# SDFIdk/malstroem

Measured on AMD Instinct MI355X. Metric: Mcells/s fill->D8->accum->label on 16384^2 f32 DEM, higher is better.
Workload: dtype f32 fill / f64 no-flats+D8+accum / u8 flowdir / i32 labels; 1 GPU; 16384x16384 float32 DEM (spectral fBm beta=2 seed 42 (SURVEY 8d recipe)): fill+depths -> no-flats fill -> D8 -> accumulation -> CCL+label_stats -> watersheds+label_count -> pour points; parallelism=1 GPU, one device context, fill_rounds=8, noflat_rounds=84, fill_tiles=70225, fill_visits=43613, fill_cycles=0, noflat_visits=409001, noflat_cycles=409001, nlabels=4637017, fill_algorithm=1, fill_launches=8, noflat_algorithm=2, pour_algorithm=1

## Files before the change

malstroem_amd/csrc/ccl.hip:

```cpp
#include <cstdlib>
#include <string>
#include <type_traits>
#include <utility>

#include "common.hpp"

namespace mh {
namespace {

constexpr int SCAN_BLOCK = 1024;
constexpr int SCAN_ITEMS = 4;
constexpr int SCAN_TILE = SCAN_BLOCK * SCAN_ITEMS;

template <typename T> __device__ __forceinline__ bool is_fg(T v) { return v != (T)0; }

template <typename T>
__global__ __launch_bounds__(256) void ccl_init_kernel(const T *__restrict__ data, int32_t *__restrict__ parent, int64_t n, int64_t W)
{
    const int64_t i = (int64_t)blockIdx.x * blockDim.x + threadIdx.x;
    const int lane = threadIdx.x & 63;
    const bool fg = i < n && is_fg(data[i]);
    const bool fg_left = __shfl_up((int)fg, 1) != 0;
    const bool start = fg && (lane == 0 || !fg_left || (i % W) == 0);
    const uint64_t brk = __ballot(start);
    if (i >= n) return;
    int32_t p = -1;
    if (fg) {
        const uint64_t below = brk & ((2ull << lane) - 1ull);
        p = (int32_t)(i - (lane - (63 - __builtin_clzll(below))));
    }
    parent[i] = p;
}

__device__ __forceinline__ int32_t find_root(const int32_t *parent, int32_t x)
{
    int32_t p = parent[x];
    while (p != x) {
        x = p;
        p = parent[x];
    }
    return x;
}

__device__ __forceinline__ void unite(int32_t *parent, int32_t a, int32_t b)
{
    for (;;) {
        a = find_root(parent, a);
        b = find_root(parent, b);
        if (a == b) return;
        if (a < b) {
            const int32_t t = a;
            a = b;
            b = t;
        }
        const int32_t old = atomicMin(&parent[a], b);
        if (old == a) return;
        a = old;
    }
}

__global__ __launch_bounds__(256) void ccl_merge_kernel(int32_t *parent, int64_t H, int64_t W)
{
    const int64_t i = (int64_t)blockIdx.x * blockDim.x + threadIdx.x;
    if (i >= H * W) return;
    if (parent[i] < 0) return;
    const int64_t r = i / W, c = i - r * W;
    const bool hasW = c > 0 && parent[i - 1] >= 0;
    if (hasW && (threadIdx.x & 63) == 0) unite(parent, (int32_t)i, (int32_t)(i - 1));
    if (r == 0) return;
    const bool hasN = parent[i - W] >= 0;
    const bool hasNW = c > 0 && parent[i - W - 1] >= 0;
    if (hasN) {
        if (!(hasW && hasNW)) unite(parent, (int32_t)i, (int32_t)(i - W));
        return;
    }
    const bool hasNE = c + 1 < W && parent[i - W + 1] >= 0;
    if (hasNW && !hasW) unite(parent, (int32_t)i, (int32_t)(i - W - 1));
    if (hasNE) unite(parent, (int32_t)i, (int32_t)(i - W + 1));
}

constexpr int CT = 64;
constexpr int MAXROOTS = CT * CT / 4;
constexpr uint32_t LBG = 0xffffffffu;

__device__ __forceinline__ uint32_t find_root_l(const uint32_t *par, uint32_t x)
{
    uint32_t p = par[x];
    while (p != x) {
        x = p;
        p = par[x];
    }
    return x;
}
__device__ __forceinline__ void unite_l(uint32_t *par, uint32_t a, uint32_t b)
{
    for (;;) {
        a = find_root_l(par, a);
        b = find_root_l(par, b);
        if (a == b) return;
        if (a < b) {
            const uint32_t t = a;
            a = b;
            b = t;
        }
        const uint32_t old = atomicMin(&par[a], b);
        if (old == a) return;
        a = old;
    }
}

#ifndef CCL_U2
#define CCL_U2 4
#endif
#ifndef CCL_U3
#define CCL_U3 4
#endif
template <typename T>
__global__ __launch_bounds__(256) void ccl_tile_kernel(const T *__restrict__ data, int32_t *__restrict__ parent, int64_t H, int64_t W, int ntc,
                                                       int32_t *__restrict__ rootlist, int32_t *__restrict__ rootcount, int32_t *__restrict__ colpar)
{
    __shared__ uint32_t par[CT * CT];
    __shared__ int s_nroots;
    if (threadIdx.x == 0) s_nroots = 0;
    const int lane = threadIdx.x & 63, wave = threadIdx.x >> 6;
    const int ti = blockIdx.x / ntc, tj = blockIdx.x - ti * ntc;
    const int64_t r0 = (int64_t)ti * CT, c0 = (int64_t)tj * CT;
    const int64_t cc = c0 + lane;
#pragma unroll
    for (int k = 0; k < CT / 4; ++k) {
        const int r = wave + 4 * k;
        const bool fg = (r0 + r) < H && cc < W && is_fg(data[(r0 + r) * W + cc]);
        const uint64_t m = __ballot(fg);
        const uint64_t starts = m & ~(m << 1);
        const uint64_t below = starts & ((2ull << lane) - 1ull);
        par[r * CT + lane] = fg ? (uint32_t)(r * CT + (63 - __builtin_clzll(below))) : LBG;
    }
    __syncthreads();
#pragma unroll CCL_U2
    for (int k = 0; k < CT / 4; ++k) {
        const int r = wave + 4 * k;
        if (r == 0) continue;
        const uint64_t m = __ballot(par[r * CT + lane] != LBG);
        const uint32_t pn = par[(r - 1) * CT + lane];
        const uint64_t up = __ballot(pn != LBG);
        if (!((m >> lane) & 1ull)) continue;
        const bool hasW = lane > 0 && ((m >> (lane - 1)) & 1ull), hasN = (up >> lane) & 1ull;
        const bool hasNW = lane > 0 && ((up >> (lane - 1)) & 1ull), hasNE = lane < 63 && ((up >> (lane + 1)) & 1ull);
        const uint32_t i = (uint32_t)(r * CT + lane);
        if (hasN) {
            if (!(hasW && hasNW)) unite_l(par, i, i - CT);
        } else {
            if (hasNW && !hasW) unite_l(par, i, i - CT - 1);
            if (hasNE) unite_l(par, i, i - CT + 1);
        }
    }
    __syncthreads();
#pragma unroll CCL_U3
    for (int k = 0; k < CT / 4; ++k) {
        const int r = wave + 4 * k;
        const bool inside = (r0 + r) < H && cc < W;
        const uint32_t p = inside ? par[r * CT + lane] : LBG;
        int32_t out = -1;
        if (lane == 0 || lane == CT - 1) {
            int32_t e = -1;
            if (p != LBG) {
                const uint32_t rt = find_root_l(par, p);
                e = (int32_t)((r0 + (rt >> 6)) * W + c0 + (rt & 63u));
            }
            colpar[((int64_t)blockIdx.x * 2 + (lane ? 1 : 0)) * CT + r] = e;
        }
        if (!inside) continue;
        if (p != LBG) {
            const uint32_t root = find_root_l(par, p);
            out = (int32_t)((r0 + (root >> 6)) * W + c0 + (root & 63u));
            if (root == (uint32_t)(r * CT + lane)) rootlist[(size_t)blockIdx.x * MAXROOTS + atomicAdd(&s_nroots, 1)] = out;
        }
        parent[(r0 + r) * W + cc] = out;
    }
    __syncthreads();
    if (threadIdx.x == 0) rootcount[blockIdx.x] = s_nroots;
}

__global__ __launch_bounds__(256) void ccl_flatten_roots_kernel(int32_t *parent, const int32_t *__restrict__ rootlist, const int32_t *__restrict__ rootcount,
                                                                int64_t ntiles, unsigned long long *rootbits)
{
    const int64_t tile = (int64_t)blockIdx.x * 4 + (threadIdx.x >> 6);
    if (tile >= ntiles) return;
    const int cnt = rootcount[tile];
    for (int j = threadIdx.x & 63; j < cnt; j += 64) {
        const int32_t r = rootlist[(size_t)tile * MAXROOTS + j];
        const int32_t root = find_root(parent, r);
        if (root != r) parent[r] = root;
        else atomicOr(&rootbits[r >> 6], 1ull << (r & 63));
    }
}

constexpr int WB = 1024;
__global__ __launch_bounds__(WB) void ccl_bits_count_kernel(const unsigned long long *__restrict__ rootbits, int64_t nwords, uint32_t *__restrict__ block_counts)
{
    __shared__ uint32_t wsum[WB / 64];
    const int64_t w = (int64_t)blockIdx.x * WB + threadIdx.x;
    uint32_t cnt = w < nwords ? (uint32_t)__popcll(rootbits[w]) : 0u;
#pragma unroll
    for (int o = 32; o > 0; o >>= 1) cnt += __shfl_xor(cnt, o);
    if ((threadIdx.x & 63) == 0) wsum[threadIdx.x >> 6] = cnt;
    __syncthreads();
    if (threadIdx.x == 0) {
        uint32_t t = 0;
        for (int k = 0; k < WB / 64; ++k) t += wsum[k];
        block_counts[blockIdx.x] = t;
    }
}
__global__ __launch_bounds__(WB) void ccl_bits_prefix_kernel(const unsigned long long *__restrict__ rootbits, int64_t nwords,
                                                              const uint32_t *__restrict__ block_offsets, uint32_t *__restrict__ wordprefix)
{
    __shared__ uint32_t wsum[WB / 64];
    const int lane = threadIdx.x & 63, wave = threadIdx.x >> 6;
    const int64_t w = (int64_t)blockIdx.x * WB + threadIdx.x;
    const uint32_t cnt = w < nwords ? (uint32_t)__popcll(rootbits[w]) : 0u;
    uint32_t incl = cnt;
#pragma unroll
    for (int o = 1; o < 64; o <<= 1) {
        const uint32_t v = __shfl_up(incl, o);
        if (lane >= o) incl += v;
    }
    if (lane == 63) wsum[wave] = incl;
    __syncthreads();
    uint32_t woff = 0;
    for (int k = 0; k < wave; ++k) woff += wsum[k];
    if (w < nwords) wordprefix[w] = block_offsets[blockIdx.x] + woff + incl - cnt;
}

__global__ __launch_bounds__(256) void ccl_emit_ranked_kernel(const int32_t *__restrict__ parent, const unsigned long long *__restrict__ rootbits,
                                                              const uint32_t *__restrict__ wordprefix, int32_t *__restrict__ labels, int64_t n)
{
    const int64_t i0 = ((int64_t)blockIdx.x * blockDim.x + threadIdx.x) * 4;
    if (i0 >= n) return;
    auto rank_of = [&](int32_t p) -> int32_t {
        if (p < 0) return 0;
        const int32_t g = parent[p];
        return (int32_t)(wordprefix[g >> 6] + (uint32_t)__popcll(rootbits[g >> 6] & ((1ull << (g & 63)) - 1ull))) + 1;
    };
    if (i0 + 4 <= n) {
        const int4 p = *reinterpret_cast<const int4 *>(parent + i0);
        int4 l;
        l.x = rank_of(p.x);
        l.y = rank_of(p.y);
        l.z = rank_of(p.z);
        l.w = rank_of(p.w);
        *reinterpret_cast<int4 *>(labels + i0) = l;
    } else {
        for (int64_t i = i0; i < n; ++i) labels[i] = rank_of(parent[i]);
    }
}

__global__ __launch_bounds__(256) void ccl_seam_kernel(int32_t *parent, int64_t H, int64_t W, int64_t nh, int64_t total, const int32_t *__restrict__ colpar,
                                                       int64_t ntc)
{
    const int64_t k = (int64_t)blockIdx.x * blockDim.x + threadIdx.x;
    if (k >= total) return;
    if (k < nh) {
        const int64_t r = (k / W + 1) * CT, c = k % W;
        const int64_t i = r * W + c;
        if (parent[i] < 0) return;
        const bool hasW = c > 0 && parent[i - 1] >= 0, hasN = parent[i - W] >= 0, hasNW = c > 0 && parent[i - W - 1] >= 0;
        if (hasN) {
            if (!(hasW && hasNW)) unite(parent, (int32_t)i, (int32_t)(i - W));
            return;
        }
        const bool hasNE = c + 1 < W && parent[i - W + 1] >= 0;
        if (hasNW && !hasW) unite(parent, (int32_t)i, (int32_t)(i - W - 1));
        if (hasNE) unite(parent, (int32_t)i, (int32_t)(i - W + 1));
    } else {
        const int64_t q = k - nh;
        const int64_t r = q % H, sj = q / H;
        const int64_t ti = r / CT, lr = r - ti * CT;
        const int32_t *left = colpar + ((ti * ntc + sj) * 2 + 1) * CT, *right = colpar + ((ti * ntc + sj + 1) * 2 + 0) * CT;
        const int32_t me = right[lr];
        if (me < 0) return;
        const int32_t w = left[lr];
        if (w >= 0) {
            unite(parent, me, w);
            return;
        }
        if (r > 0) {
            const int32_t nw = lr > 0 ? left[lr - 1] : colpar[(((ti - 1) * ntc + sj) * 2 + 1) * CT + CT - 1];
            if (nw >= 0) unite(parent, me, nw);
        }
        if (r + 1 < H) {
            const int32_t sw = lr < CT - 1 ? left[lr + 1] : colpar[(((ti + 1) * ntc + sj) * 2 + 1) * CT];
            if (sw >= 0) unite(parent, me, sw);
        }
    }
}

__global__ __launch_bounds__(256) void ccl_flatten_kernel(int32_t *parent, int64_t n)
{
    const int64_t i = (int64_t)blockIdx.x * blockDim.x + threadIdx.x;
    if (i >= n) return;
    const int32_t p = parent[i];
    if (p < 0 || p == (int32_t)i) return;
    parent[i] = find_root(parent, p);
}

__global__ __launch_bounds__(SCAN_BLOCK) void ccl_count_roots_kernel(const int32_t *__restrict__ parent, int64_t n,
                                                                    uint32_t *__restrict__ block_counts)
{
    __shared__ uint32_t wsum[SCAN_BLOCK / 64];
    const int64_t base = (int64_t)blockIdx.x * SCAN_TILE + (int64_t)threadIdx.x * SCAN_ITEMS;
    uint32_t cnt = 0;
#pragma unroll
    for (int k = 0; k < SCAN_ITEMS; ++k) {
        const int64_t i = base + k;
        if (i < n) cnt += parent[i] == (int32_t)i;
    }
#pragma unroll
    for (int o = 32; o > 0; o >>= 1) cnt += __shfl_xor(cnt, o);
    if ((threadIdx.x & 63) == 0) wsum[threadIdx.x >> 6] = cnt;
    __syncthreads();
    if (threadIdx.x == 0) {
        uint32_t t = 0;
        for (int w = 0; w < SCAN_BLOCK / 64; ++w) t += wsum[w];
        block_counts[blockIdx.x] = t;
    }
}

__global__ __launch_bounds__(1024) void scan_blocks_kernel(uint32_t *block_counts, int64_t nb, unsigned long long *total)
{
    __shared__ unsigned long long part[1024];
    const int64_t per = (nb + 1023) / 1024;
    const int64_t b0 = (int64_t)threadIdx.x * per, b1 = b0 + per < nb ? b0 + per : nb;
    unsigned long long s = 0;
    for (int64_t b = b0; b < b1; ++b) s += block_counts[b];
    part[threadIdx.x] = s;
    __syncthreads();
    if (threadIdx.x == 0) {
        unsigned long long run = 0;
        for (int t = 0; t < 1024; ++t) {
            const unsigned long long v = part[t];
            part[t] = run;
            run += v;
        }
        *total = run;
    }
    __syncthreads();
    unsigned long long run = part[threadIdx.x];
    for (int64_t b = b0; b < b1; ++b) {
        const uint32_t v = block_counts[b];
        block_counts[b] = (uint32_t)run;
        run += v;
    }
}

__global__ __launch_bounds__(SCAN_BLOCK) void ccl_rank_roots_kernel(int32_t *parent, int64_t n,
                                                                   const uint32_t *__restrict__ block_offsets)
{
    __shared__ uint32_t wsum[SCAN_BLOCK / 64];
    const int lane = threadIdx.x & 63, wave = threadIdx.x >> 6;
    const int64_t base = (int64_t)blockIdx.x * SCAN_TILE + (int64_t)threadIdx.x * SCAN_ITEMS;
    bool root[SCAN_ITEMS];
    uint32_t cnt = 0;
#pragma unroll
    for (int k = 0; k < SCAN_ITEMS; ++k) {
        const int64_t i = base + k;
        root[k] = i < n && parent[i] == (int32_t)i;
        cnt += root[k];
    }
    uint32_t incl = cnt;
#pragma unroll
    for (int o = 1; o < 64; o <<= 1) {
        const uint32_t v = __shfl_up(incl, o);
        if (lane >= o) incl += v;
    }
    if (lane == 63) wsum[wave] = incl;
    __syncthreads();
    uint32_t woff = 0;
    for (int w = 0; w < wave; ++w) woff += wsum[w];
    uint32_t rank = block_offsets[blockIdx.x] + woff + incl - cnt;
#pragma unroll
    for (int k = 0; k < SCAN_ITEMS; ++k)
        if (root[k]) {
            ++rank;
            parent[base + k] = -(int32_t)rank - 1;
        }
}

__global__ __launch_bounds__(256) void ccl_emit_kernel(const int32_t *__restrict__ parent, int32_t *__restrict__ labels,
                                                      int64_t n)
{
    const int64_t i = (int64_t)blockIdx.x * blockDim.x + threadIdx.x;
    if (i >= n) return;
    int32_t p = parent[i];
    if (p >= 0) p = parent[p];
    labels[i] = p == -1 ? 0 : -p - 1;
}

template <typename T>
int ccl8_dev(const T *d_data, int32_t *d_labels, int32_t *d_tmp, int64_t H, int64_t W, int64_t *nlabels, hipStream_t s, DevBuf *stats_out = nullptr,
             CclKeep *keep = nullptr)
{
    if (keep) keep->valid = false;
    const int64_t n = H * W;
    if (n >= (int64_t)INT32_MAX - 1) {
        set_error("connected components: %lld cells exceed the int32 index domain", (long long)n);
        return MHIP_ELIMIT;
    }
    const unsigned g256 = (unsigned)cdiv(n, 256);
    const int64_t nb = cdiv(n, SCAN_TILE);
    DevBuf counts, total;
    MH_TRY(counts.alloc(sizeof(uint32_t) * (size_t)nb));
    MH_TRY(total.alloc(sizeof(unsigned long long)));
    int32_t *parent = d_tmp;
    static const bool global_uf = [] { const char *e = dev_env("MHIP_CCL"); return e && std::string(e) == "global"; }();
    if (global_uf) {
        hipLaunchKernelGGL((ccl_init_kernel<T>), dim3(g256), dim3(256), 0, s, d_data, parent, n, W);
        hipLaunchKernelGGL(ccl_merge_kernel, dim3(g256), dim3(256), 0, s, parent, H, W);
        hipLaunchKernelGGL(ccl_flatten_kernel, dim3(g256), dim3(256), 0, s, parent, n);
        hipLaunchKernelGGL(ccl_count_roots_kernel, dim3((unsigned)nb), dim3(SCAN_BLOCK), 0, s, parent, n, counts.as<uint32_t>());
        hipLaunchKernelGGL(scan_blocks_kernel, dim3(1), dim3(1024), 0, s, counts.as<uint32_t>(), nb, total.as<unsigned long long>());
        hipLaunchKernelGGL(ccl_rank_roots_kernel, dim3((unsigned)nb), dim3(SCAN_BLOCK), 0, s, parent, n, counts.as<uint32_t>());
        hipLaunchKernelGGL(ccl_emit_kernel, dim3(g256), dim3(256), 0, s, parent, d_labels, n);
    } else {
        const int64_t ntr = cdiv(H, CT), ntc = cdiv(W, CT), ntiles = ntr * ntc;
        const int64_t nwords = cdiv(n, 64), nwb = cdiv(nwords, WB);
        DevBuf roots, rcount, bits, wprefix, bcounts, colpar;
        MH_TRY(colpar.alloc(4 * 2 * CT * (size_t)ntiles));
        MH_TRY(roots.alloc(4 * (size_t)ntiles * MAXROOTS));
        MH_TRY(rcount.alloc(4 * (size_t)ntiles));
        MH_TRY(bits.alloc(8 * (size_t)nwords));
        MH_TRY(wprefix.alloc(4 * (size_t)nwords));
        MH_TRY(bcounts.alloc(4 * (size_t)nwb));
        MH_HIP(hipMemsetAsync(bits.p, 0, 8 * (size_t)nwords, s));
        hipLaunchKernelGGL((ccl_tile_kernel<T>), dim3((unsigned)ntiles), dim3(256), 0, s, d_data, parent, H, W, (int)ntc, roots.as<int32_t>(),
                           rcount.as<int32_t>(), colpar.as<int32_t>());
        const int64_t nh = (ntr - 1) * W, nv = (ntc - 1) * H;
        if (nh + nv > 0)
            hipLaunchKernelGGL(ccl_seam_kernel, dim3((unsigned)cdiv(nh + nv, 256)), dim3(256), 0, s, parent, H, W, nh, nh + nv, colpar.as<int32_t>(), ntc);
        hipLaunchKernelGGL(ccl_flatten_roots_kernel, dim3((unsigned)cdiv(ntiles, 4)), dim3(256), 0, s, parent, roots.as<int32_t>(),
                           rcount.as<int32_t>(), ntiles, bits.as<unsigned long long>());
        hipLaunchKernelGGL(ccl_bits_count_kernel, dim3((unsigned)nwb), dim3(WB), 0, s, bits.as<unsigned long long>(), nwords, bcounts.as<uint32_t>());
        hipLaunchKernelGGL(scan_blocks_kernel, dim3(1), dim3(1024), 0, s, bcounts.as<uint32_t>(), nwb, total.as<unsigned long long>());
        hipLaunchKernelGGL(ccl_bits_prefix_kernel, dim3((unsigned)nwb), dim3(WB), 0, s, bits.as<unsigned long long>(), nwords, bcounts.as<uint32_t>(),
                           wprefix.as<uint32_t>());
        unsigned long long h_total = 0;
        if constexpr (std::is_same<T, float>::value) {
            if (stats_out) {
                MH_HIP(hipGetLastError());
                MH_HIP(hipMemcpyAsync(&h_total, total.p, sizeof(h_total), hipMemcpyDeviceToHost, s));
                MH_HIP(stream_sync(s));
                *nlabels = (int64_t)h_total;
                MH_TRY(stats_out->alloc(sizeof(mhip_stat_record) * (size_t)(h_total + 1)));
                return label_emit_stats_dev(parent, bits.as<unsigned long long>(), wprefix.as<uint32_t>(), d_data, d_labels, H, W, (int64_t)h_total,
                                            stats_out->as<mhip_stat_record>(), s);
            }
        }
        if (keep) {
            const int64_t top = (H < 4 ? H : 2) * W;
            MH_TRY(ccl_emit_rows_dev(parent, bits.as<unsigned long long>(), wprefix.as<uint32_t>(), d_labels, 0, top, s));
            if (H >= 4) MH_TRY(ccl_emit_rows_dev(parent, bits.as<unsigned long long>(), wprefix.as<uint32_t>(), d_labels, (H - 2) * W, 2 * W, s));
        } else {
            hipLaunchKernelGGL(ccl_emit_ranked_kernel, dim3((unsigned)cdiv(cdiv(n, 4), 256)), dim3(256), 0, s, parent, bits.as<unsigned long long>(), wprefix.as<uint32_t>(), d_labels, n);
        }
        MH_HIP(hipGetLastError());
        MH_HIP(hipMemcpyAsync(&h_total, total.p, sizeof(h_total), hipMemcpyDeviceToHost, s));
        MH_HIP(stream_sync(s));
        *nlabels = (int64_t)h_total;
        if (keep) {
            keep->bits.release();
            keep->wprefix.release();
            std::swap(keep->bits.p, bits.p);
            std::swap(keep->bits.bytes, bits.bytes);
            std::swap(keep->wprefix.p, wprefix.p);
            std::swap(keep->wprefix.bytes, wprefix.bytes);
            keep->H = H;
            keep->W = W;
            keep->nlocal = (int64_t)h_total;
            keep->valid = true;
        }
        return MHIP_OK;
    }
    MH_HIP(hipGetLastError());
    unsigned long long h_total = 0;
    MH_HIP(hipMemcpyAsync(&h_total, total.p, sizeof(h_total), hipMemcpyDeviceToHost, s));
    MH_HIP(stream_sync(s));
    *nlabels = (int64_t)h_total;
    if constexpr (std::is_same<T, float>::value) {
        if (stats_out) {
            MH_TRY(stats_out->alloc(sizeof(mhip_stat_record) * (size_t)(h_total + 1)));
            MH_TRY(label_stats_dev(d_data, d_labels, n, (int64_t)h_total, stats_out->as<mhip_stat_record>(), s, W, true));
        }
    }
    return MHIP_OK;
}

}

int ccl8_f32_dev(const float *d_data, int32_t *d_labels, int32_t *d_tmp, int64_t H, int64_t W, int64_t *nlabels,
                 hipStream_t s, DevBuf *stats_out)
{
    return ccl8_dev<float>(d_data, d_labels, d_tmp, H, W, nlabels, s, stats_out);
}
int ccl8_f32_begin_dev(const float *d_data, int32_t *d_labels, int32_t *d_tmp, int64_t H, int64_t W, int64_t *nlabels, hipStream_t s, CclKeep *keep)
{
    return ccl8_dev<float>(d_data, d_labels, d_tmp, H, W, nlabels, s, nullptr, keep);
}
int ccl8_u8_dev(const uint8_t *d_data, int32_t *d_labels, int32_t *d_tmp, int64_t H, int64_t W, int64_t *nlabels,
                hipStream_t s)
{
    return ccl8_dev<uint8_t>(d_data, d_labels, d_tmp, H, W, nlabels, s);
}

}
```

malstroem_amd/csrc/common.hpp:

```cpp
#pragma once
#include <hip/hip_runtime.h>
#include <cstdint>
#include <cstdio>
#include <cstring>
#include <string>
#include <vector>

#include "../../include/malstroem_hip.h"

struct mhip_polygons;
struct mhip_flowpaths;

namespace mh {

void set_error(const char *fmt, ...);
const char *get_error();
const char *dev_env(const char *name);
hipError_t stream_sync(hipStream_t s);
int require_device();

#define MH_HIP(expr)                                                                             \
    do {                                                                                         \
        hipError_t _e = (expr);                                                                  \
        if (_e != hipSuccess) {                                                                  \
// ... 24 lines not shown
    size_t bytes = 0;
    DevBuf() = default;
    DevBuf(const DevBuf &) = delete;
    DevBuf &operator=(const DevBuf &) = delete;
    ~DevBuf() { release(); }
    int alloc(size_t n)
    {
        if (n == 0) n = 16;
        if (p && bytes >= n && bytes <= 2 * n + 4096) return MHIP_OK;
        release();
        MH_TRY(pool_alloc(&p, n));
        bytes = n;
        return MHIP_OK;
    }
    void release()
    {
        if (p) pool_free(p, bytes);
        p = nullptr;
        bytes = 0;
    }
    template <typename T> T *as() const { return reinterpret_cast<T *>(p); }
};

int upload(DevBuf &b, const void *host, size_t bytes, hipStream_t s);
int download(void *host, const DevBuf &b, size_t bytes, hipStream_t s);
int64_t build_rank_lut(const uint8_t *keep, int64_t nlab, std::vector<int32_t> &lut);
inline bool hyps_res_ok(double res) { return res > 0.0 && res <= 1.7976931348623157e308; }
int trace_on_device(const uint8_t *d_fd, const int32_t *d_lab, int64_t H, int64_t W, const int64_t *cells_rc, int64_t n, int use_bg,
                    int32_t bg, int32_t *out_label, int32_t *out_found, int64_t *out_len, const int64_t *offsets, int64_t *out_cells,
                    hipStream_t s);

__host__ __device__ inline int dir_dr(int k) { return (k == 0 || k == 1 || k == 7) ? -1 : (k >= 3 && k <= 5) ? 1 : 0; }
__host__ __device__ inline int dir_dc(int k) { return (k >= 1 && k <= 3) ? 1 : (k >= 5 && k <= 7) ? -1 : 0; }

__device__ __forceinline__ unsigned d8_code(double z, double u, double ur, double r, double dr, double d, double dl,
                                            double l, double ul)
{
    const double INV_SQRT2 = 0.7071067811865475;
    unsigned i = 8;
    double dzmax = 0.0, dz;
#define MH_D8_STEP(expr, k)          \
    dz = (expr);                     \
    i = dz > dzmax ? (k) : i;        \
    dzmax = fmax(dzmax, dz);
    MH_D8_STEP(__dsub_rn(z, u), 0u)
    MH_D8_STEP(__dmul_rn(__dsub_rn(z, ur), INV_SQRT2), 1u)
    MH_D8_STEP(__dsub_rn(z, r), 2u)
    MH_D8_STEP(__dmul_rn(__dsub_rn(z, dr), INV_SQRT2), 3u)
    MH_D8_STEP(__dsub_rn(z, d), 4u)
    MH_D8_STEP(__dmul_rn(__dsub_rn(z, dl), INV_SQRT2), 5u)
    MH_D8_STEP(__dsub_rn(z, l), 6u)
    MH_D8_STEP(__dmul_rn(__dsub_rn(z, ul), INV_SQRT2), 7u)
#undef MH_D8_STEP
    return i;
}

__device__ __forceinline__ unsigned edge_code(int64_t r, int64_t c, int64_t maxr, int64_t maxc)
{
    unsigned code = 8;
    if (r == 0) code = 0;
    if (r == maxr) code = 4;
    if (c == 0) code = 6;
    if (c == maxc) code = 2;
    if (r == 0 && c == 0) code = 7;
    if (r == 0 && c == maxc) code = 1;
    if (r == maxr && c == 0) code = 5;
    if (r == maxr && c == maxc) code = 3;
    return code;
}

__host__ __device__ inline uint32_t f32_key(float f)
{
    uint32_t u;
    memcpy(&u, &f, 4);
    return (u & 0x80000000u) ? ~u : (u | 0x80000000u);
}
__host__ __device__ inline float key_f32(uint32_t k)
{
    uint32_t u = (k & 0x80000000u) ? (k & 0x7fffffffu) : ~k;
    float f;
    memcpy(&f, &u, 4);
    return f;
}
__device__ __forceinline__ uint32_t dem_key(float v)
{
    if (v != v) return f32_key(__builtin_inff());
    return f32_key(v + 0.0f);
}
__host__ __device__ inline uint64_t f64_key(double f)
{
    uint64_t u;
    memcpy(&u, &f, 8);
    return (u & 0x8000000000000000ull) ? ~u : (u | 0x8000000000000000ull);
}
__host__ __device__ inline double key_f64(uint64_t k)
{
    uint64_t u = (k & 0x8000000000000000ull) ? (k & 0x7fffffffffffffffull) : ~k;
    double f;
    memcpy(&f, &u, 8);
    return f;
}

struct FillStats {
    int32_t rounds = 0;
    int64_t visits = 0;
    int64_t cycles = 0;
    int64_t tiles = 0;
    float hot_ms = 0;
    int32_t hot_launches = 0;
    int32_t algorithm = 0;
    uint32_t overflow = 0;
    bool have_minmax = false, dem_nan = false;
    float dem_min = 0.0f, dem_max = 0.0f;
    int32_t geo_reject = 0;
    int64_t geo_irregular = 0, geo_unreached = 0, geo_mismatch = 0;
};

struct FillRun {
    bool noflat = false;
    const float *dem = nullptr;
    void *out = nullptr;
    int64_t H = 0, W = 0;
    double sh = 0, dg = 0;
    const float *seed = nullptr;
    double seed_add = 0;
    int fixed_top = 0, fixed_bot = 0;
    int rounds_per_batch = 8;
    bool attach_only = false;
    struct Impl;
    Impl *impl;
    FillRun();
    ~FillRun();
    FillRun(const FillRun &) = delete;
    FillRun &operator=(const FillRun &) = delete;
    int begin(hipStream_t s, bool *active);
    int batch(hipStream_t s, bool *active);
    int activate_row(int side, hipStream_t s);
    int attach(hipStream_t s);
    int certify(hipStream_t s, bool *changed);
    int finish(hipStream_t s, FillStats *st);
};
void noflat_seed(FillRun &f, const float *d_filled, double sh, double dg, int64_t ncells_global);
struct PfRun;
struct FillHandover {
    PfRun *run = nullptr;
    const float *dem = nullptr;
    float *filled = nullptr, *depths = nullptr;
    int64_t H = 0, W = 0;
    const uint16_t *bslot = nullptr;
    const uint32_t *tabV = nullptr;
    int ntr = 0, ntc = 0;
    bool pending = false, queued = false, violated = false, repaired = false;
    bool suspect = false;
    FillStats st_repair;
    FillHandover() = default;
    FillHandover(const FillHandover &) = delete;
    FillHandover &operator=(const FillHandover &) = delete;
    ~FillHandover();
    void release();
};
int fill_handover_complete(FillHandover *ho, hipStream_t s);
int fill_handover_repair(FillHandover *ho, hipStream_t s);
int fill_plain_dev(const float *d_dem, float *d_out, int64_t H, int64_t W, hipStream_t s, FillStats *st, float *d_depths = nullptr,
                   bool *depths_done = nullptr, FillHandover *ho = nullptr);
int fill_check_f32_dev(const float *d_dem, const float *d_filled, int64_t H, int64_t W, int fixed_top, int fixed_bot, hipStream_t s,
                       unsigned int *d_flag);
int fill_plain_pflood_dev(const float *d_dem, float *d_out, float *d_depths, int64_t H, int64_t W, hipStream_t s, FillStats *st, bool *violated = nullptr,
                          uint32_t *overflow = nullptr, FillHandover *ho = nullptr);
struct PfRun {
    const float *dem = nullptr;
    float *out = nullptr;
    int64_t H = 0, W = 0;
    int fixed_top = 0, fixed_bot = 0;
    uint32_t overflow = 0;
    struct Impl;
    Impl *impl;
    PfRun();
    ~PfRun();
    PfRun(const PfRun &) = delete;
    PfRun &operator=(const PfRun &) = delete;
    int begin(hipStream_t s);
    int halo_changed(int side, hipStream_t s);
    int batch(hipStream_t s);
    int finish(hipStream_t s, float *d_depths, FillStats *st, bool *violated = nullptr, FillHandover *ho = nullptr);
    int finish_late(hipStream_t s, float *d_depths, bool *violated);
    int proof_flag(hipStream_t s, unsigned int *h_flag);
    int solve(hipStream_t s);
    int pack(hipStream_t s, int row0, int nrows);
    int publish_edges(hipStream_t s);
};
struct StageHook {
    enum Point { FIRST_VISIT = 0, TAIL_ROUNDS = 1, FINISH = 3 };
    void (*fn)(void *, hipStream_t) = nullptr;
    void *arg = nullptr;
    bool fired = false;
    int at = TAIL_ROUNDS;
    void fire(hipStream_t s)
    {
        if (fn && !fired) {
            fired = true;
            fn(arg, s);
        }
    }
    void fire_at(int point, hipStream_t s)
    {
        if (point == at) fire(s);
    }
};

struct GeoRun {
    const float *dem = nullptr, *filled = nullptr;
    double *out = nullptr;
    uint32_t *dist = nullptr;
    int64_t H = 0, W = 0;
    double sh = 0, dg = 0;
    int fixed_top = 0, fixed_bot = 0;
    bool allow_partial = false;
    double seed_add = 0;
    bool partial = false;
    StageHook *tail_hook = nullptr;
    uint8_t *d8_out = nullptr;
    unsigned int *d8_nodir = nullptr;
    bool d8_done = false;
    bool defer_out = false;
    bool out_deferred = false;
    FillHandover *handover = nullptr;
    struct Impl;
    Impl *impl;
    GeoRun();
    ~GeoRun();
    GeoRun(const GeoRun &) = delete;
    GeoRun &operator=(const GeoRun &) = delete;
    int begin(hipStream_t s, bool *applicable, bool *active);
    int batch(hipStream_t s, bool *active);
    int halo_changed(int side, hipStream_t s);
    int end(hipStream_t s, bool *ok, FillStats *st);
    int launch_rounds(hipStream_t s, int nb);
};
struct D8Sink {
    uint8_t *flowdir = nullptr;
    unsigned int *nodir = nullptr;
    bool done = false;
    uint32_t *dist = nullptr;
    bool defer = false, deferred = false;
};
int noflat_assemble_dev(const float *d_filled, const uint32_t *d_dist, double *d_out, int64_t n, double seed_add, hipStream_t s);
int fill_noflat_geodesic_dev(const float *d_dem, const float *d_filled, double *d_out, int64_t H, int64_t W, double sh, double dg, double seed_add,
                             hipStream_t s, FillStats *st, bool *partial, StageHook *tail_hook = nullptr, D8Sink *d8 = nullptr, FillHandover *ho = nullptr);
int noflat_verify_dev(const float *d_dem, const double *d_out, int64_t H, int64_t W, double sh, double dg, hipStream_t s, bool *ok, int fixed_top = 0,
                      int fixed_bot = 0);
int fill_noflat_dev(const float *d_dem, double *d_out, int64_t H, int64_t W, double sh, double dg, hipStream_t s,
                    FillStats *st = nullptr, const float *d_filled = nullptr, StageHook *tail_hook = nullptr, D8Sink *d8 = nullptr,
                    FillHandover *ho = nullptr);
int short_diag_dev(const float *d_dem, int64_t n, double *sh, double *dg, hipStream_t s);
int depths_dev(const float *d_filled, const float *d_dem, float *d_out, int64_t n, hipStream_t s);
int d8_dev(const double *d_z, uint8_t *d_out, int64_t H, int64_t W, int edges_outward, hipStream_t s, int64_t row_off = 0,
           int64_t Hg = 0, unsigned int *d_interior_nodir = nullptr);
void short_diag_from_minmax(float mn, float mx, bool has_nan, double *sh, double *dg);
int minmax_dev(const float *d_x, int64_t n, float *mn, float *mx, int *has_nan, hipStream_t s);
int row_update_dev(void *d_dst, const void *d_src, int64_t nbytes, int *changed, hipStream_t s);
int copy_bandwidth_dev(size_t bytes, int reps, double *gbs, hipStream_t s);
int read_bandwidth_dev(size_t bytes, int reps, double *gbs, hipStream_t s);
int row_update_async(void *d_dst, const void *d_src, int64_t nbytes, int *d_changed, hipStream_t s);
int trace_downstream_dev(const uint8_t *d_fd, const int32_t *d_lab, int64_t H, int64_t W, const int64_t *d_cells, int64_t n, int use_bg,
                         int32_t bg, int32_t *d_label, int32_t *d_found, int64_t *d_len, const int64_t *d_offsets, int64_t *d_out_cells,
                         hipStream_t s);
int comm_unique_id(void *id128);
int comm_available();
int comm_create(void **comm, const void *id128, int rank, int nranks);
void comm_destroy(void *comm);
int comm_exchange_rows(void *comm, int rank, int nranks, const void *first_row, const void *last_row, void *stage, size_t rowbytes,
                       hipStream_t s);
int comm_allreduce_max(void *comm, double *d_value, hipStream_t s);
struct PourCandDev {
    uint16_t *mask0 = nullptr;
    uint2 *list = nullptr;
    uint32_t *tile_cnt = nullptr;
    unsigned long long *tile_key0 = nullptr;
    uint32_t *flags = nullptr;
    int components = 0;
    unsigned long long *key = nullptr;
    uint32_t nlab = 0;
};
constexpr uint32_t POUR_TILE_CAP = 512;
struct PourLink {
    PourCandDev dev;
    hipEvent_t ev = nullptr;
    void (*notify)(void *, int) = nullptr;
    int (*wait)(void *) = nullptr;
    void *arg = nullptr;
    bool consumed = false;
};
struct AccumKeep {
    DevBuf nodes;
    size_t o[9] = {};
    int64_t H = 0, W = 0;
    int fixed_top = 0, fixed_bot = 0;
    bool valid = false;
};
struct AccumPrep {
    DevBuf nodes;
    int64_t H = 0, W = 0;
    hipEvent_t ready = nullptr;
    bool valid = false;
    ~AccumPrep();
};
int accum_prepare_dev(AccumPrep *prep, int64_t H, int64_t W, hipStream_t s, hipEvent_t ready);
int accum_dev(const uint8_t *d_fd, double *d_out, int64_t H, int64_t W, hipStream_t s, int fixed_top = 0, int fixed_bot = 0, int halo_zero = 0,
              int32_t *d_exit_map = nullptr, PourLink *pour = nullptr, AccumKeep *keep = nullptr, AccumPrep *prep = nullptr);
int accum_band_delta_dev(const uint8_t *d_fd, double *d_out, int64_t H, int64_t W, hipStream_t s, int fixed_top, int fixed_bot, AccumKeep *keep, bool *done);
int ccl8_f32_dev(const float *d_data, int32_t *d_labels, int32_t *d_tmp, int64_t H, int64_t W, int64_t *nlabels,
                 hipStream_t s, DevBuf *stats_out = nullptr);
int label_emit_stats_dev(const int32_t *d_parent, const unsigned long long *d_rootbits, const uint32_t *d_wordprefix, const float *d_data,
                         int32_t *d_labels, int64_t H, int64_t W, int64_t nlab, mhip_stat_record *d_rec, hipStream_t s);
int ccl8_u8_dev(const uint8_t *d_data, int32_t *d_labels, int32_t *d_tmp, int64_t H, int64_t W, int64_t *nlabels,
                hipStream_t s);
struct CclKeep {
    DevBuf bits, wprefix;
    int64_t H = 0, W = 0, nlocal = 0;
    bool valid = false;
};
int ccl8_f32_begin_dev(const float *d_data, int32_t *d_labels, int32_t *d_tmp, int64_t H, int64_t W, int64_t *nlabels, hipStream_t s, CclKeep *keep);
int ccl_emit_rows_dev(const int32_t *d_parent, const unsigned long long *d_rootbits, const uint32_t *d_wordprefix, int32_t *d_labels, int64_t base,
                      int64_t count, hipStream_t s);
int label_emit_sparse_dev(const int32_t *d_parent, const unsigned long long *d_rootbits, const uint32_t *d_wordprefix, const float *d_data,
                          int32_t *d_labels, int64_t H, int64_t W, int ht, int64_t H_owned, int64_t nlocal, int32_t offset,
                          const int32_t *d_dropped, const int32_t *d_target, int32_t ndropped, int64_t nlab_global, mhip_stat_record *d_rec,
                          hipStream_t s);
int relabel_lut_dev(int32_t *d_labels, const int32_t *d_lut, int64_t nlab, int64_t n, hipStream_t s);
int relabel_range_dev(int32_t *d_labels, int64_t n, int32_t lo, int32_t hi, const int32_t *d_lut, const int32_t *d_fid, const int32_t *d_fnew, int32_t nf,
                      hipStream_t s);
int band_trace_dev(const uint8_t *d_fd, const int32_t *d_lab, int64_t Hl, int64_t W, int64_t row_lo, int64_t own0, int64_t own1, int64_t Hg,
                   const int64_t *d_cells, const int32_t *d_src, int64_t n, int use_bg, int32_t bg, int32_t *d_label, int32_t *d_status,
                   int32_t *d_src_out, int64_t *d_exit, int64_t *d_len, const int64_t *d_offsets, int64_t *d_out_cells, hipStream_t s);
int relabel_sparse_dev(int32_t *d_labels, int64_t n, int64_t nlocal, int32_t offset, const int32_t *d_dropped, const int32_t *d_target,
                       int32_t ndropped, hipStream_t s);
int keep_mask_dev(const int32_t *d_labels, const uint8_t *d_keep, int64_t nlab, int64_t n, uint8_t *d_mask,
                  hipStream_t s);
int label_stats_dev(const float *d_data, const int32_t *d_labels, int64_t n, int64_t nlab, mhip_stat_record *d_rec,
                    hipStream_t s, int64_t W = 0, bool components = false);
int label_stats64_dev(const double *d_data, const int32_t *d_labels, int64_t n, int64_t nlab, mhip_stat_record *d_rec, hipStream_t s);
int label_stats_zero_sign_dev(const float *d_data, const int32_t *d_labels, int64_t n, int64_t nlab, mhip_stat_record *d_rec, hipStream_t s);
int label_stats_zero_sign_dev(const double *d_data, const int32_t *d_labels, int64_t n, int64_t nlab, mhip_stat_record *d_rec, hipStream_t s);
int label_arg_dev(const double *d_data, const int32_t *d_labels, int64_t H, int64_t W, int64_t nlab, bool is_max,
                  mhip_index_record *d_rec, hipStream_t s, bool components = false);
int label_count_dev(const int32_t *d_labels, int64_t n, int64_t nlab, int64_t *d_counts, hipStream_t s, int64_t W = 0);
int label_max_dev(const int32_t *d_labels, int64_t n, int32_t *out_max, hipStream_t s);
constexpr int64_t HYPS_MAX_BINS = (int64_t)1 << 30;
int hyps_layout_dev(const double *d_dmax, int64_t stride, int64_t nlab, double res, int64_t *d_offsets, int64_t *total, hipStream_t s);
int hyps_table_dev(const float *d_data, const int32_t *d_labels, int64_t n, int64_t W, int64_t nlab, double res, const int64_t *d_offsets,
                   int64_t total, uint32_t *d_counts, double *d_sums, int64_t *lds_spills, hipStream_t s, hipEvent_t ev0 = nullptr,
                   hipEvent_t ev1 = nullptr);
int hyps_levels_dev(int64_t nlab, const int64_t *d_offsets, const uint32_t *d_counts, const double *d_sums, const double *d_dmax, int64_t stride,
                    const double *d_q, mhip_final_record *d_rec, hipStream_t s);
int final_depths_dev(const float *d_data, const int32_t *d_labels, int64_t n, int64_t W, int64_t nlab, mhip_final_record *d_rec, float *d_out,
                     hipStream_t s, hipEvent_t ev0 = nullptr, hipEvent_t ev1 = nullptr);
bool wet_at_events_ok(int64_t K, const float *values);
int wet_at_dev(const float *d_data, const int32_t *d_labels, int64_t n, int64_t W, int64_t nlab, int K, const double *d_drawdown, int64_t stride,
               const float *values, float *d_out, int64_t *d_wet, int64_t wet_stride, hipStream_t s, hipEvent_t ev0 = nullptr,
               hipEvent_t ev1 = nullptr);
bool flow_distance_scale_ok(double scale);
int flow_distance_dev(const uint8_t *d_fd, const int32_t *d_lab, int64_t H, int64_t W, double scale, int64_t nlab, float *d_out, mhip_index_record *d_rec,
                      int64_t *unresolved, hipStream_t s);
int fdist_jumps_dev(uint4 *&cur, uint4 *&nxt, int64_t W, int64_t ntc, int64_t ntiles, unsigned int *d_open, hipStream_t s);
int hand_check(double threshold, double scale);
int hand_dev(const uint8_t *d_fd, const double *d_acc, const float *d_elev, const int32_t *d_lab, int64_t H, int64_t W, double threshold, double scale,
             float nodata, float *d_hand, float *d_dist, int64_t *undrained, hipStream_t s);
int reach_catchments_dev(const uint8_t *d_fd, const double *d_acc, const int32_t *d_lab, int64_t H, int64_t W, double threshold, int32_t *d_catch,
                         mhip_flowpaths *p, int64_t *assigned, hipStream_t s);
int inundate_dev(const float *d_hand, const int32_t *d_catch, int64_t n, int64_t W, int64_t nreach, const float *d_stage, float nodata, float *d_depth,
                 mhip_zone_record *d_rec, hipStream_t s);
int burn_check(int64_t nseg, const mhip_burn_segment *segs, int64_t nline, const mhip_burn_line *lines, const mhip_burn_result *results);
int burn_lines_dev(float *d_dem, int64_t H, int64_t W, int64_t nseg, const mhip_burn_segment *segs, int64_t nline, const mhip_burn_line *lines,
                   double nodata, mhip_burn_result *results, hipStream_t s);
int zones_check(int64_t H, int64_t W, int64_t nvert, const double *xy, int64_t nring, const int64_t *ring_offsets, const int32_t *ring_zone,
                int64_t nzone, int grow);
int zones_rasterize_dev(int32_t *d_out, int64_t H, int64_t W, int64_t nvert, const double *xy, int64_t nring, const int64_t *ring_offsets,
                        const int32_t *ring_zone, int64_t nzone, int grow, hipStream_t s);
int zone_stats_dev(const float *d_data, const int32_t *d_zones, int64_t n, int64_t W, int64_t nzone, mhip_zone_record *d_rec, hipStream_t s);
int polygonize_check(int64_t H, int64_t W);
int polygons_fetch_dev(const mhip_polygons *p, int32_t *xy, int64_t *ring_offsets, int32_t *ring_label);
int polygonize_dev(const int32_t *d_lab, int64_t H, int64_t W, DevBuf &d_xy, DevBuf &d_off, DevBuf &d_rl, int64_t *nring, int64_t *nvert, hipStream_t s);
int flowpaths_check(int64_t H, int64_t W, double threshold);
int flowpaths_dev(const uint8_t *d_fd, const double *d_acc, const int32_t *d_lab, int64_t H, int64_t W, double threshold, mhip_flowpaths *p, hipStream_t s,
                  int32_t *d_rc = nullptr);
int flowpaths_fetch_dev(const mhip_flowpaths *p, int32_t *xy, int64_t *reach_offsets, mhip_reach_record *records);
int watersheds_dev(const uint8_t *d_fd, int32_t *d_labels, int64_t H, int64_t W, int32_t unassigned, hipStream_t s,
                   bool band_mode = false, const unsigned int *d_known_interior_nodir = nullptr, const int32_t *d_src = nullptr, PourLink *pour = nullptr);
int pour_finish_dev(unsigned long long *d_key, const unsigned long long *d_tile_key0, int64_t ntiles, int64_t nlab, int64_t W, mhip_index_record *d_rec,
                    hipStream_t s);
int band_pseudo_labels_dev(int32_t *d_ws, int64_t H, int64_t W, int top, int bottom, hipStream_t s);
int negative_lut_dev(int32_t *d_lab, int64_t n, const int32_t *d_lut, int64_t nlut, hipStream_t s);
constexpr int32_t BAND_ROOT = 1, BAND_ROOTLESS = 0x7fffffff;
int band_root_labels_dev(int32_t *d_out, int64_t H, int64_t W, int64_t row_off, int64_t Hg, hipStream_t s);
int band_hide_rootless_dev(const int32_t *d_lab, const int32_t *d_rooted, int32_t *d_out, int64_t n, hipStream_t s);
int band_show_rootless_dev(int32_t *d_ws, const int32_t *d_lab, int64_t n, hipStream_t s);

__host__ __device__ inline int64_t cdiv(int64_t a, int64_t b) { return (a + b - 1) / b; }

constexpr int TR = 32;
struct TileGeom {
    int64_t n, W;
    int64_t ntr, ntc;
};
__host__ __device__ inline TileGeom tile_geom(int64_t n, int64_t W)
{
    TileGeom g;
    g.n = n;
    g.W = (W > 0 && n % W == 0) ? W : 256;
    const int64_t H = cdiv(n, g.W);
    g.ntr = cdiv(H, TR);
    g.ntc = cdiv(g.W, 256);
    return g;
}
inline unsigned tile_grid(const TileGeom &g)
{
    const int64_t nt = g.ntr * g.ntc;
    return (unsigned)(nt < 2048 ? (nt > 0 ? nt : 1) : 2048);
}

#ifdef __HIPCC__
__device__ __forceinline__ int64_t downstream(const uint8_t *fd, int64_t i, int64_t H, int64_t W)
{
    const unsigned code = fd[i];
    if (code > 7u) return -1;
    const int64_t r = i / W, c = i - r * W;
    const int64_t nr = r + dir_dr((int)code), nc = c + dir_dc((int)code);
    if (nr < 0 || nr >= H || nc < 0 || nc >= W) return -1;
    return nr * W + nc;
}
constexpr int WS_TILE = 64;
__device__ __forceinline__ int ws_perim_slot(int lr, int lc)
{
    if (lr == 0) return lc;
    if (lr == WS_TILE - 1) return WS_TILE + lc;
    if (lc == 0) return 2 * WS_TILE + (lr - 1);
    if (lc == WS_TILE - 1) return 2 * WS_TILE + (WS_TILE - 2) + (lr - 1);
    return -1;
}
__device__ __forceinline__ int64_t ws_node_of(int32_t cell, uint32_t W, int ntc)
{
    const uint32_t r = (uint32_t)cell / W, c = (uint32_t)cell - r * W;
    const int slot = ws_perim_slot((int)(r & 63u), (int)(c & 63u));
    return slot < 0 ? -1 : (int64_t)((r >> 6) * (uint32_t)ntc + (c >> 6)) * 256 + slot;
}

constexpr int32_t FD_NONE = 0x7fffffff;
constexpr int32_t FD_DONE = (int32_t)0x80000000;
constexpr double FD_SQRT2 = 1.4142135623730951;
__device__ __forceinline__ uint32_t fd_step(unsigned code) { return (code & 1u) ? 0x10000u : 1u; }
__device__ __forceinline__ bool fd_resolve(uint2 s, const uint4 *__restrict__ Nn, uint32_t W, int ntc, uint32_t &no, uint32_t &nd, int32_t &T)
{
    int32_t t = (int32_t)s.x;
    no = s.y & 0xffffu;
    nd = s.y >> 16;
    if (t >= 0 && t != FD_NONE) {
        const int64_t node = ws_node_of(t, W, ntc);
        uint4 m = make_uint4((uint32_t)FD_NONE, 0u, 0u, 0u);
        if (node >= 0) m = Nn[node];
        t = (int32_t)m.x;
        no += m.y;
        nd += m.z;
    }
    T = t & ~FD_DONE;
    return t < 0;
// ... 55 lines not shown
```

malstroem_amd/csrc/ctx.hip:

```cpp
#include <mutex>
#include <new>
#include <string>
#include <vector>

#include "ctx.hpp"

namespace mh {

static void drop_hyps(mhip_ctx *c)
{
    c->hyps_total = -1;
    c->have[MHIP_R_FINALDEPTHS] = false;
    c->wetat_events = -1;
    c->wetat_out.release();
}

static void drop_flow_distance(mhip_ctx *c)
{
    std::lock_guard<std::mutex> lk(c->fdist_mu);
    c->fdist_unresolved = -1;
    c->fdist_out.release();
    c->fdist_rec.release();
}

// ... 257 lines not shown
}

int mhip_ctx_side_end(mhip_ctx *c)
{
    MH_ARG(c && t_side_ctx == c, "ctx_side_end without ctx_side_begin on this thread");
    MH_HIP(hipSetDevice(c->device));
    MH_HIP(stream_sync(c->stream_b));
    t_side_ctx = nullptr;
    return MHIP_OK;
}

int mhip_ctx_upload(mhip_ctx *c, int which, const void *host)
{
    MH_ARG(c && host && which >= 0 && which < MHIP_R_COUNT_, "ctx_upload(ctx, which, host)");
    return mhip_ctx_upload_rows(c, which, 0, c->H_owned, host);
}

int mhip_ctx_upload_dem(mhip_ctx *c, const float *dem) { return mhip_ctx_upload(c, MHIP_R_DEM, dem); }

int mhip_ctx_upload_rows(mhip_ctx *c, int which, int64_t row0, int64_t nrows, const void *host)
{
    MH_ARG(c && host && which >= 0 && which < MHIP_R_COUNT_ && row0 >= 0 && nrows >= 1 && row0 + nrows <= c->H_owned,
           "ctx_upload_rows(ctx, which, row0, nrows, host)");
    MH_HIP(hipSetDevice(c->device));
    MH_TRY(ctx_raster(c, which));
    MH_TRY(ctx_settle(c, which, true));
    ctx_wrote(c, which, true);
    c->have[which] = false;
    MH_TRY(ctx_copy_rows(c, c->r[which].p, raster_elem(which), row0, nrows, const_cast<void *>(host), hipMemcpyHostToDevice));
    if (row0 + nrows == c->H_owned) {
        c->have[which] = true;
        if (which == MHIP_R_LABELS) c->labels_filtered = true;
    }
    return MHIP_OK;
}

int mhip_ctx_download_rows(mhip_ctx *c, int which, int64_t row0, int64_t nrows, void *host)
{
    MH_ARG(c && host && which >= 0 && which < MHIP_R_COUNT_ && row0 >= 0 && nrows >= 1 && row0 + nrows <= c->H_owned,
           "ctx_download_rows(ctx, which, row0, nrows, host)");
    MH_ARG(c->have[which], "raster has not been computed or uploaded");
    MH_TRY(ctx_settle(c, which, false));
    return ctx_copy_rows(c, c->r[which].p, raster_elem(which), row0, nrows, host, hipMemcpyDeviceToHost);
}

int mhip_ctx_download(mhip_ctx *c, int which, void *host)
{
    MH_ARG(c && host && which >= 0 && which < MHIP_R_COUNT_, "ctx_download(ctx, which, host)");
    return mhip_ctx_download_rows(c, which, 0, c->H_owned, host);
}

int mhip_ctx_trace_downstream(mhip_ctx *c, const int64_t *cells_rc, int64_t n, int use_background, int32_t background, int32_t *out_label,
                              int32_t *out_found, int64_t *out_len, const int64_t *offsets, int64_t *out_cells)
{
    MH_ARG(c && n >= 0 && (n == 0 || cells_rc), "ctx_trace_downstream(ctx, cells, n, ...)");
    MH_ARG(c->have[MHIP_R_FLOWDIR] && c->have[MHIP_R_LABELS], "ctx_trace_downstream needs flow directions and labels");
    MH_ARG(!c->ht && !c->hb, "stream tracing runs on an undivided raster");
    if (n == 0) return MHIP_OK;
    MH_HIP(hipSetDevice(c->device));
    return trace_on_device(c->r[MHIP_R_FLOWDIR].as<uint8_t>(), c->r[MHIP_R_LABELS].as<int32_t>(), c->H, c->W, cells_rc, n, use_background,
                           background, out_label, out_found, out_len, offsets, out_cells, c->stream);
}

int mhip_ctx_sync(mhip_ctx *c)
{
    MH_ARG(c, "ctx");
    MH_HIP(stream_sync(c->stream));
    return MHIP_OK;
}

int mhip_ctx_stage_ms(mhip_ctx *c, int stage, float *ms)
{
    MH_ARG(c && ms, "ctx_stage_ms(ctx, stage, ms)");
    const int k = timer_slot(stage);
    MH_ARG(k >= 0 && c->timers[k].valid, "stage has not been run");
    MH_HIP(hipEventSynchronize(c->timers[k].b));
    MH_HIP(hipEventElapsedTime(ms, c->timers[k].a, c->timers[k].b));
    return MHIP_OK;
}

int mhip_ctx_kernel_ms(mhip_ctx *c, const char *kernel, float *ms_total, int32_t *launches)
{
    MH_ARG(c && kernel && ms_total && launches, "ctx_kernel_ms(ctx, kernel, ms, launches)");
    const std::string k(kernel);
    if (k == "d8") {
        *launches = 1;
        return mhip_ctx_stage_ms(c, MHIP_STAGE_FLOWDIR, ms_total);
    }
    if (k == "d8_steady") {
        MH_ARG(c->have[MHIP_R_NOFLAT] && !c->ht && !c->hb, "d8_steady needs the no-flats surface on an undivided context");
        MH_HIP(hipSetDevice(c->device));
        double *g = nullptr;
        MH_TRY(ctx_noflat(c, &g));
        MH_TRY(ctx_raster(c, MHIP_R_FLOWDIR));
        MH_TRY(c->nodir_cnt.alloc(4));
        constexpr int REPS = 16;
        StageTimer *t;
        MH_TRY(ctx_timer(c, D8_STEADY_SLOT, &t));
        hipStream_t s = c->stream;
        ctx_wrote(c, MHIP_R_FLOWDIR);
        MH_HIP(hipMemsetAsync(c->nodir_cnt.p, 0, 4, s));
        for (int i = 0; i < REPS + 2; ++i) {
            if (i == 2) MH_HIP(hipEventRecord(t->a, s));
            MH_TRY(d8_dev(g, c->r[MHIP_R_FLOWDIR].as<uint8_t>(), c->H, c->W, 1, s, 0, c->H_global, c->nodir_cnt.as<unsigned int>()));
        }
        MH_HIP(hipEventRecord(t->b, s));
        MH_HIP(hipEventSynchronize(t->b));
        MH_HIP(hipEventElapsedTime(ms_total, t->a, t->b));
        c->have[MHIP_R_FLOWDIR] = true;
        c->nodir_valid = true;
        c->flowdir_own = true;
        *launches = REPS;
        return MHIP_OK;
    }
    if (k == "hyps_table" || k == "final_depths") {
        *launches = 1;
        return mhip_ctx_stage_ms(c, k == "hyps_table" ? HYPS_KERNEL_SLOT : FINAL_KERNEL_SLOT, ms_total);
    }
    if (k == "wet_at") {
        *launches = 1;
        return mhip_ctx_stage_ms(c, WETAT_KERNEL_SLOT, ms_total);
    }
    if (k == "fill_round") {
        *launches = c->fill_rounds;
        return mhip_ctx_stage_ms(c, MHIP_STAGE_FILL, ms_total);
    }
    if (k == "noflat_round") {
        *launches = c->noflat_rounds;
        return mhip_ctx_stage_ms(c, MHIP_STAGE_NOFLAT, ms_total);
    }
    set_error("unknown kernel family '%s'", kernel);
    return MHIP_EINVAL;
}

int mhip_ctx_get_i64(mhip_ctx *c, const char *key, int64_t *value)
{
    MH_ARG(c && key && value, "ctx_get_i64(ctx, key, value)");
    const std::string k(key);
    if (k == "nlabels_raw") *value = c->nlabels_raw;
    else if (k == "nlabels") {
        if (c->nlabels < 0 && c->have[MHIP_R_LABELS]) {
            MH_HIP(hipSetDevice(c->device));
            MH_TRY(ctx_label_max(c, c->stream));
        }
        *value = c->nlabels;
    }
    else if (k == "fill_rounds") *value = c->fill_rounds;
    else if (k == "noflat_rounds") *value = c->noflat_rounds;
    else if (k == "fill_visits") *value = c->fill_st.visits;
    else if (k == "fill_cycles") *value = c->fill_st.cycles;
    else if (k == "fill_tiles") *value = c->fill_st.tiles;
    else if (k == "fill_algorithm") *value = c->fill_st.algorithm;
    else if (k == "fill_handover") *value = c->fill_handover;
    else if (k == "fill_handover_rechecks") *value = c->fill_handover_rechecks;
    else if (k == "fill_overflow") *value = c->fill_st.overflow;
    else if (k == "fill_launches") *value = c->fill_st.rounds;
    else if (k == "fill_hot_launches") *value = c->fill_st.hot_launches;
    else if (k == "noflat_hot_launches") *value = c->noflat_st.hot_launches;
    else if (k == "accum_algorithm") *value = c->accum_algorithm;
    else if (k == "flowdir_computed") *value = (c->have[MHIP_R_FLOWDIR] && c->flowdir_own) ? 1 : 0;
    else if (k == "pour_algorithm") *value = c->pour_algorithm;
    else if (k == "noflat_algorithm") *value = c->noflat_st.algorithm;
    else if (k == "noflat_pending") *value = c->noflat_pending ? 1 : 0;
    else if (k == "noflat_visits") *value = c->noflat_st.visits;
    else if (k == "noflat_reject") *value = c->noflat_st.geo_reject;
    else if (k == "noflat_reject_irregular") *value = c->noflat_st.geo_irregular;
    else if (k == "noflat_reject_unreached") *value = c->noflat_st.geo_unreached;
    else if (k == "noflat_reject_mismatch") *value = c->noflat_st.geo_mismatch;
    else if (k == "noflat_cycles") *value = c->noflat_st.cycles;
    else if (k == "hyps_bins") *value = c->hyps_total;
    else if (k == "hyps_lds_spills") *value = c->hyps_spills;
    else if (k == "wet_at_events") *value = c->wetat_events;
    else if (k == "flow_distance_unresolved") *value = c->fdist_unresolved;
    else if (k == "hand_undrained") *value = c->hand_undrained;
    else if (k == "reach_catchments") *value = c->rcatch_nreach;
    else if (k == "inundation") *value = c->inund_held;
    else if (k == "zones") *value = c->nzone;
    else if (k == "H") *value = c->H;
    else if (k == "W") *value = c->W;
    else {
        set_error("unknown key '%s'", key);
        return MHIP_EINVAL;
    }
    return MHIP_OK;
}

int mhip_ctx_get_f64(mhip_ctx *c, const char *key, double *value)
{
    MH_ARG(c && key && value, "ctx_get_f64(ctx, key, value)");
    const std::string k(key);
    if (k == "short") *value = c->sh;
    else if (k == "diag") *value = c->dg;
    else if (k == "fill_hot_ms") *value = c->fill_st.hot_ms;
    else if (k == "noflat_hot_ms") *value = c->noflat_st.hot_ms;
    else {
        set_error("unknown key '%s'", key);
        return MHIP_EINVAL;
    }
    return MHIP_OK;
}

int mhip_ctx_raw_stats(mhip_ctx *c, mhip_stat_record *records)
{
    MH_ARG(c && records && c->raw_stats.p && c->nlabels_raw >= 0, "ctx_raw_stats needs a LABEL run");
    return ctx_fetch(c, c->raw_stats, sizeof(mhip_stat_record) * (size_t)(c->nlabels_raw + 1), records);
}

int mhip_ctx_apply_keep(mhip_ctx *c, const uint8_t *keep)
{
    MH_ARG(c, "ctx");
    MH_HIP(hipSetDevice(c->device));
    return ctx_apply_keep_on(c, keep, c->stream);
}

int mhip_ctx_stats(mhip_ctx *c, mhip_stat_record *records)
{
    MH_ARG(c && records && c->stats_valid && c->labels_filtered, "ctx_stats needs LABEL + apply_keep (or mhip_ctx_hyps) on the resident depths and labels");
    return ctx_fetch(c, c->stats, sizeof(mhip_stat_record) * (size_t)(c->nlabels + 1), records);
}

int mhip_ctx_watershed_counts(mhip_ctx *c, int64_t *counts)
{
    MH_ARG(c && counts && c->ws_counts_valid, "ctx_watershed_counts needs a WATERSHED run on the resident labels");
    return ctx_fetch(c, c->ws_counts, 8 * (size_t)(c->nlabels + 1), counts);
}

int mhip_ctx_pourpoints(mhip_ctx *c, mhip_index_record *records)
{
    MH_ARG(c && records && c->pour_valid, "ctx_pourpoints needs a POURPOINTS run on the resident labels and accumulated flow");
    return ctx_fetch(c, c->pour, sizeof(mhip_index_record) * (size_t)(c->nlabels + 1), records);
}

int mhip_ctx_hyps(mhip_ctx *c, double res, int64_t *total)
{
    MH_ARG(c && total && hyps_res_ok(res), "ctx_hyps(ctx, 0 < res < inf, total)");
    MH_ARG(!(c->nranks > 1 || c->ht || c->hb), "hypsometry on a row band is not built (the tables of the bands add up: a later step); use an undivided context");
    MH_ARG(c->have[MHIP_R_DEPTHS] && c->have[MHIP_R_LABELS] && !c->ccl_pending, "ctx_hyps needs the DEPTHS and LABELS rasters");
    MH_ARG(c->labels_filtered, "ctx_hyps needs mhip_ctx_apply_keep after the LABEL run");
    MH_HIP(hipSetDevice(c->device));
    hipStream_t s = c->stream;
    const int64_t n = c->H * c->W;
    c->hyps_total = -1;
    if (!c->stats_valid) {
        MH_TRY(ctx_label_max(c, s));
        MH_TRY(c->stats.alloc(sizeof(mhip_stat_record) * (size_t)(c->nlabels + 1)));
        MH_TRY(label_stats_dev(c->r[MHIP_R_DEPTHS].as<float>(), c->r[MHIP_R_LABELS].as<int32_t>(), n, c->nlabels, c->stats.as<mhip_stat_record>(), s,
                               c->W, c->labels_components));
        c->stats_valid = true;
    }
    const int64_t nlab = c->nlabels;
    MH_TRY(c->hyps_off.alloc(8 * (size_t)(nlab + 2)));
    StageTimer *k;
    MH_TRY(ctx_timer(c, HYPS_KERNEL_SLOT, &k));
    MH_TRY(stage_begin(c, MHIP_STAGE_HYPS, s));
    int64_t tot = 0;
    MH_TRY(hyps_layout_dev(c->stats.as<double>() + 1, 4, nlab, res, c->hyps_off.as<int64_t>(), &tot, s));
    MH_TRY(c->hyps_cnt.alloc(4 * (size_t)tot));
    MH_TRY(c->hyps_sum.alloc(8 * (size_t)tot));
    MH_TRY(hyps_table_dev(c->r[MHIP_R_DEPTHS].as<float>(), c->r[MHIP_R_LABELS].as<int32_t>(), n, c->W, nlab, res, c->hyps_off.as<int64_t>(), tot,
                          c->hyps_cnt.as<uint32_t>(), c->hyps_sum.as<double>(), &c->hyps_spills, s, k->a, k->b));
    MH_TRY(stage_end(c, MHIP_STAGE_HYPS, s));
    k->valid = true;
    c->hyps_total = tot;
    *total = tot;
    return MHIP_OK;
}

int mhip_ctx_hyps_fetch(mhip_ctx *c, int64_t *offsets, int64_t *counts, double *sums)
{
    MH_ARG(c && offsets && counts && sums, "ctx_hyps_fetch(ctx, offsets, counts, sums)");
    MH_ARG(c->hyps_total >= 0, "ctx_hyps_fetch needs mhip_ctx_hyps on the resident depths and labels");
    MH_HIP(hipSetDevice(c->device));
    hipStream_t s = c->stream;
    const size_t tot = (size_t)c->hyps_total;
    std::vector<uint32_t> c32(tot + 1);
    MH_HIP(hipMemcpyAsync(offsets, c->hyps_off.p, 8 * (size_t)(c->nlabels + 2), hipMemcpyDeviceToHost, s));
    if (tot) {
        MH_HIP(hipMemcpyAsync(c32.data(), c->hyps_cnt.p, 4 * tot, hipMemcpyDeviceToHost, s));
        MH_HIP(hipMemcpyAsync(sums, c->hyps_sum.p, 8 * tot, hipMemcpyDeviceToHost, s));
    }
    MH_HIP(stream_sync(s));
    for (size_t k = 0; k < tot; ++k) counts[k] = (int64_t)c32[k];
    return MHIP_OK;
}

int mhip_ctx_final_depths(mhip_ctx *c, const double *q, mhip_final_record *records)
{
    MH_ARG(c && q && records, "ctx_final_depths(ctx, q, records)");
    MH_ARG(c->hyps_total >= 0 && c->stats_valid, "ctx_final_depths needs mhip_ctx_hyps on the resident depths and labels");
    MH_HIP(hipSetDevice(c->device));
    hipStream_t s = c->stream;
    const int64_t nlab = c->nlabels, n = c->H * c->W;
    DevBuf d_q;
    MH_TRY(upload(d_q, q, 8 * (size_t)(nlab + 1), s));
    MH_TRY(c->hyps_rec.alloc(sizeof(mhip_final_record) * (size_t)(nlab + 1)));
    MH_TRY(ctx_raster(c, MHIP_R_FINALDEPTHS));
    c->have[MHIP_R_FINALDEPTHS] = false;
    StageTimer *k;
    MH_TRY(ctx_timer(c, FINAL_KERNEL_SLOT, &k));
    MH_TRY(stage_begin(c, MHIP_STAGE_FINALDEPTHS, s));
    MH_TRY(hyps_levels_dev(nlab, c->hyps_off.as<int64_t>(), c->hyps_cnt.as<uint32_t>(), c->hyps_sum.as<double>(), c->stats.as<double>() + 1, 4,
                           d_q.as<double>(), c->hyps_rec.as<mhip_final_record>(), s));
    MH_TRY(final_depths_dev(c->r[MHIP_R_DEPTHS].as<float>(), c->r[MHIP_R_LABELS].as<int32_t>(), n, c->W, nlab, c->hyps_rec.as<mhip_final_record>(),
                            c->r[MHIP_R_FINALDEPTHS].as<float>(), s, k->a, k->b));
    MH_TRY(stage_end(c, MHIP_STAGE_FINALDEPTHS, s));
    k->valid = true;
// ... 321 lines not shown
```

malstroem_amd/csrc/ctx.hpp:

```cpp
#pragma once
#include <atomic>
#include <condition_variable>
#include <functional>
#include <mutex>
#include <thread>

#include "common.hpp"

namespace mh {

class SideThread {
    std::thread th_;
    std::mutex mu_;
    std::condition_variable cv_;
    std::function<void()> task_;
    bool busy_ = false, stop_ = false;

public:
    ~SideThread()
    {
        {
            std::lock_guard<std::mutex> lk(mu_);
            stop_ = true;
        }
        cv_.notify_all();
        if (th_.joinable()) th_.join();
    }
    void run(std::function<void()> f)
    {
        std::unique_lock<std::mutex> lk(mu_);
        if (!th_.joinable())
            th_ = std::thread([this] {
                std::unique_lock<std::mutex> l2(mu_);
                for (;;) {
                    cv_.wait(l2, [this] { return stop_ || (busy_ && task_); });
                    if (stop_) return;
                    std::function<void()> f2 = std::move(task_);
                    task_ = nullptr;
                    l2.unlock();
                    f2();
                    l2.lock();
                    busy_ = false;
                    cv_.notify_all();
                }
            });
        task_ = std::move(f);
        busy_ = true;
        cv_.notify_all();
    }
    void wait()
    {
        std::unique_lock<std::mutex> lk(mu_);
        cv_.wait(lk, [this] { return !busy_; });
    }
};

struct StageTimer {
    hipEvent_t a = nullptr, b = nullptr;
    bool valid = false;
};
constexpr int N_STAGE_BITS = 9;
constexpr int WETAT_KERNEL_SLOT = 1 << 27, FINAL_KERNEL_SLOT = 1 << 28, HYPS_KERNEL_SLOT = 1 << 29, D8_STEADY_SLOT = 1 << 30;
constexpr int N_TIMERS = N_STAGE_BITS + 4;

}

struct mhip_ctx {
    mh::SideThread side;
    int64_t H = 0, W = 0;
    int64_t H_global = 0, row0 = 0, H_owned = 0;
    int ht = 0, hb = 0;
    mh::FillRun *run[2] = {nullptr, nullptr};
    mh::GeoRun *geo = nullptr;
    uint32_t pf_overflow = 0;
    mh::PfRun *pf = nullptr;
    bool pf_done = false;
    mh::DevBuf nodir_cnt;
    bool nodir_valid = false;
    bool flowdir_own = false;
    int device = 0, rank = 0, nranks = 1;
    hipStream_t stream = nullptr;
    mh::DevBuf r[MHIP_R_COUNT_];
    bool have[MHIP_R_COUNT_] = {};
    bool noflat_pending = false;
    mh::DevBuf tmp_i32;
    mh::CclKeep ccl_keep;
    bool ccl_pending = false;
    bool pf_depths = false;
    mh::DevBuf raw_stats, stats, ws_counts, pour;
    mh::AccumKeep acc_keep;
    int accum_algorithm = 0;
    mh::DevBuf pp_mask0, pp_list, pp_tiles, pp_misc, pp_key;
    hipEvent_t ev_cand = nullptr;
    hipEvent_t ev_prep = nullptr;
    int pour_algorithm = 0;
    int64_t nlabels_raw = -1, nlabels = -1;
    bool labels_components = false;
    bool labels_filtered = false;
    std::atomic<bool> stats_valid{false};
    std::atomic<bool> ws_counts_valid{false};
    std::atomic<bool> pour_valid{false};
    mh::DevBuf hyps_off, hyps_cnt, hyps_sum, hyps_rec;
    int64_t hyps_total = -1, hyps_spills = 0;
    mh::DevBuf wetat_out;
    int wetat_events = -1;
    mh::DevBuf fdist_out, fdist_rec;
    std::atomic<int64_t> fdist_unresolved{-1};
    std::mutex fdist_mu;
    mh::DevBuf hand_out, hand_dist;
    std::atomic<int64_t> hand_undrained{-1};
    int hand_src = -1;
    bool hand_labels = false;
    double hand_thr = 0;
    float hand_nodata = 0;
    std::mutex hand_mu;
    mh::DevBuf rcatch_out, inund_out;
    std::atomic<int64_t> rcatch_nreach{-1};
    std::atomic<int> inund_held{-1};
    double rcatch_thr = 0;
    bool rcatch_labels = false;
    std::mutex rcatch_mu;
    mh::DevBuf zones;
    int64_t nzone = -1;
    double sh = 0, dg = 0;
    int32_t fill_rounds = 0, noflat_rounds = 0;
    int64_t fill_handover_rechecks = 0;
    int32_t fill_handover = 0;
    mh::FillStats fill_st, noflat_st;
    mh::StageTimer timers[mh::N_TIMERS];
    void *comm = nullptr;
    void *comm_b = nullptr;
    mh::DevBuf comm_stage, comm_word, comm_flags, comm_stage_b;
    hipStream_t stream_b = nullptr, stream_c = nullptr;
    hipEvent_t ev_fork = nullptr, ev_flowdir = nullptr, ev_join = nullptr, ev_label = nullptr, ev_tail = nullptr;
};

namespace mh {

inline size_t raster_elem(int which)
{
    switch (which) {
    case MHIP_R_DEM: case MHIP_R_FILLED: case MHIP_R_DEPTHS: case MHIP_R_LABELS: case MHIP_R_WATERSHEDS: case MHIP_R_NGDIST:
    case MHIP_R_FINALDEPTHS: return 4;
    case MHIP_R_NOFLAT: case MHIP_R_ACCUM: return 8;
    case MHIP_R_FLOWDIR: return 1;
    default: return 0;
    }
}

inline int ctx_raster(mhip_ctx *c, int which)
{
    if (!c->r[which].p) MH_TRY(c->r[which].alloc(raster_elem(which) * (size_t)(c->H * c->W)));
    return MHIP_OK;
}

inline int timer_slot(int stage)
{
    for (int b = 0; b < N_STAGE_BITS; ++b)
        if (stage == 1 << b) return b;
    return stage == FINAL_KERNEL_SLOT ? N_STAGE_BITS : stage == HYPS_KERNEL_SLOT ? N_STAGE_BITS + 1 : stage == D8_STEADY_SLOT ? N_STAGE_BITS + 2 :
           stage == WETAT_KERNEL_SLOT ? N_STAGE_BITS + 3 : -1;
}
inline int ctx_timer(mhip_ctx *c, int stage, StageTimer **t)
{
    const int k = timer_slot(stage);
    MH_ARG(k >= 0, "not a stage");
    *t = &c->timers[k];
    if (!(*t)->a) {
        hipEvent_t e0, e1;
        MH_HIP(hipEventCreate(&e0));
        MH_HIP(hipEventCreate(&e1));
        (*t)->a = e0;
        (*t)->b = e1;
    }
    return MHIP_OK;
}
inline int stage_begin(mhip_ctx *c, int stage, hipStream_t s)
{
    StageTimer *t;
    MH_TRY(ctx_timer(c, stage, &t));
    MH_HIP(hipEventRecord(t->a, s));
    return MHIP_OK;
}
inline int stage_end(mhip_ctx *c, int stage, hipStream_t s)
{
    StageTimer &t = c->timers[timer_slot(stage)];
    MH_HIP(hipEventRecord(t.b, s));
    t.valid = true;
    return MHIP_OK;
}

inline thread_local mhip_ctx *t_side_ctx = nullptr;
static inline hipStream_t cs(mhip_ctx *c) { return (t_side_ctx == c && c->stream_b) ? c->stream_b : c->stream; }
static inline bool on_side(mhip_ctx *c) { return t_side_ctx == c; }

void ctx_wrote(mhip_ctx *c, int which, bool uploaded = false);
int ctx_noflat(mhip_ctx *c, double **g = nullptr);
inline int ctx_settle(mhip_ctx *c, int which, bool write)
{
    if (which == MHIP_R_NOFLAT || (write && (which == MHIP_R_FILLED || which == MHIP_R_NGDIST))) return ctx_noflat(c);
    return MHIP_OK;
}
int ctx_copy_rows(mhip_ctx *c, void *dev_base, size_t elem_bytes, int64_t row0, int64_t nrows, void *host, hipMemcpyKind kind);
int ctx_fetch(mhip_ctx *c, const DevBuf &buf, size_t bytes, void *host);
int ctx_fork_join_events(mhip_ctx *c);
int ctx_apply_keep_on(mhip_ctx *c, const uint8_t *keep, hipStream_t s);
int ctx_ensure_labels_final(mhip_ctx *c, hipStream_t s);
int ctx_label_max(mhip_ctx *c, hipStream_t s);

}
```

malstroem_amd/csrc/ctx_run.hip:

```cpp
#include <atomic>
#include <future>
#include <string>

#include "ctx.hpp"

using namespace mh;

constexpr int LABEL_START_DEFAULT = 3;
constexpr int FILL_HANDOVER_DEFAULT = 1;
constexpr int NOFLAT_LAZY_DEFAULT = 1;

static bool fill_handover_env()
{
    const char *e = dev_env("MHIP_FILL_HANDOVER");
    return e ? e[0] != '0' : FILL_HANDOVER_DEFAULT != 0;
}

static bool noflat_lazy_env()
{
    const char *e = dev_env("MHIP_NOFLAT_LAZY");
    return e ? e[0] != '0' : NOFLAT_LAZY_DEFAULT != 0;
}

static int stage_depths(mhip_ctx *c, hipStream_t s)
{
    MH_ARG(c->have[MHIP_R_FILLED] && c->have[MHIP_R_DEM], "depths need the filled surface");
    MH_TRY(ctx_raster(c, MHIP_R_DEPTHS));
    MH_TRY(depths_dev(c->r[MHIP_R_FILLED].as<float>(), c->r[MHIP_R_DEM].as<float>(), c->r[MHIP_R_DEPTHS].as<float>(), c->H * c->W, s));
    ctx_wrote(c, MHIP_R_DEPTHS);
    c->have[MHIP_R_DEPTHS] = true;
    return MHIP_OK;
}

static int stage_fill(mhip_ctx *c, hipStream_t s, bool with_depths = true, FillHandover *ho = nullptr)
{
    const int64_t H = c->H, W = c->W;
    MH_ARG(c->have[MHIP_R_DEM], "FILL needs the DEM");
    MH_TRY(ctx_raster(c, MHIP_R_FILLED));
    MH_TRY(ctx_raster(c, MHIP_R_DEPTHS));
    MH_TRY(stage_begin(c, MHIP_STAGE_FILL, s));
    FillStats st;
    bool depths_done = false;
    MH_TRY(fill_plain_dev(c->r[MHIP_R_DEM].as<float>(), c->r[MHIP_R_FILLED].as<float>(), H, W, s, &st, c->r[MHIP_R_DEPTHS].as<float>(),
                          &depths_done, ho));
    ctx_wrote(c, MHIP_R_FILLED);
    ctx_wrote(c, MHIP_R_DEPTHS);
    const bool owed = ho && ho->pending;
    c->have[MHIP_R_FILLED] = !owed;
    c->have[MHIP_R_DEPTHS] = depths_done && !owed;
    if (with_depths && !depths_done) MH_TRY(stage_depths(c, s));
    MH_TRY(stage_end(c, MHIP_STAGE_FILL, s));
    c->fill_rounds = st.rounds;
    c->fill_st = st;
    return MHIP_OK;
}

static void ctx_handover_settled(mhip_ctx *c, FillHandover *ho)
{
    if (!ho || ho->pending || c->have[MHIP_R_FILLED]) return;
    c->have[MHIP_R_FILLED] = true;
    c->have[MHIP_R_DEPTHS] = true;
    c->fill_handover = ho->queued ? 1 : 0;
    if (ho->suspect) ++c->fill_handover_rechecks;
    if (ho->repaired) {
        c->fill_st.algorithm = 4;
        c->fill_st.rounds += ho->st_repair.rounds;
        c->fill_st.visits += ho->st_repair.visits;
        c->fill_st.cycles += ho->st_repair.cycles;
        c->fill_rounds = c->fill_st.rounds;
    }
}

static int stage_noflat(mhip_ctx *c, hipStream_t s, bool shdg_done = false, StageHook *tail_hook = nullptr, bool with_flowdir = false,
                        bool *flowdir_done = nullptr, FillHandover *ho = nullptr)
{
    const int64_t H = c->H, W = c->W, n = H * W;
    MH_ARG(c->have[MHIP_R_DEM], "NOFLAT needs the DEM");
    MH_TRY(ctx_raster(c, MHIP_R_NOFLAT));
    c->noflat_pending = false;
    MH_TRY(stage_begin(c, MHIP_STAGE_NOFLAT, s));
    if (!shdg_done) {
        if ((c->have[MHIP_R_FILLED] || (ho && ho->pending)) && c->fill_st.have_minmax) short_diag_from_minmax(c->fill_st.dem_min, c->fill_st.dem_max, c->fill_st.dem_nan, &c->sh, &c->dg);
        else MH_TRY(short_diag_dev(c->r[MHIP_R_DEM].as<float>(), n, &c->sh, &c->dg, s));
    }
    FillStats st;
    if (!c->have[MHIP_R_FILLED] && !(ho && ho->pending)) {
        MH_TRY(ctx_raster(c, MHIP_R_FILLED));
        FillStats st0;
        MH_TRY(fill_plain_dev(c->r[MHIP_R_DEM].as<float>(), c->r[MHIP_R_FILLED].as<float>(), H, W, s, &st0));
        ctx_wrote(c, MHIP_R_FILLED);
        c->have[MHIP_R_FILLED] = true;
    }
    D8Sink d8;
    static const bool fuse_d8 = [] { const char *e = dev_env("MHIP_D8_FUSE"); return !(e && e[0] == '0'); }();
    if (with_flowdir && fuse_d8 && !c->ht && !c->hb) {
        MH_TRY(ctx_raster(c, MHIP_R_FLOWDIR));
        MH_TRY(c->nodir_cnt.alloc(4));
        MH_HIP(hipMemsetAsync(c->nodir_cnt.p, 0, 4, s));
        d8.flowdir = c->r[MHIP_R_FLOWDIR].as<uint8_t>();
        d8.nodir = c->nodir_cnt.as<unsigned int>();
        if (c->nranks == 1 && noflat_lazy_env()) {
            MH_TRY(ctx_raster(c, MHIP_R_NGDIST));
            d8.dist = c->r[MHIP_R_NGDIST].as<uint32_t>();
            d8.defer = true;
        }
    }
    const int rc_nf = fill_noflat_dev(c->r[MHIP_R_DEM].as<float>(), c->r[MHIP_R_NOFLAT].as<double>(), H, W, c->sh, c->dg, s, &st,
                                      c->r[MHIP_R_FILLED].as<float>(), tail_hook, d8.flowdir ? &d8 : nullptr, ho);
    ctx_handover_settled(c, ho);
    MH_TRY(rc_nf);
    if (flowdir_done) *flowdir_done = d8.done;
    MH_TRY(stage_end(c, MHIP_STAGE_NOFLAT, s));
    c->noflat_rounds = st.rounds;
    c->noflat_st = st;
    ctx_wrote(c, MHIP_R_NOFLAT);
    c->have[MHIP_R_NOFLAT] = true;
    c->noflat_pending = d8.deferred;
    return MHIP_OK;
}

static int stage_flowdir(mhip_ctx *c, hipStream_t s)
{
    MH_ARG(c->have[MHIP_R_NOFLAT], "FLOWDIR needs the no-flats surface");
    double *g = nullptr;
    MH_TRY(ctx_noflat(c, &g));
    MH_TRY(ctx_raster(c, MHIP_R_FLOWDIR));
    MH_TRY(stage_begin(c, MHIP_STAGE_FLOWDIR, s));
    ctx_wrote(c, MHIP_R_FLOWDIR);
    MH_TRY(c->nodir_cnt.alloc(4));
    MH_HIP(hipMemsetAsync(c->nodir_cnt.p, 0, 4, s));
    MH_TRY(d8_dev(g, c->r[MHIP_R_FLOWDIR].as<uint8_t>(), c->H, c->W, 1, s, c->row0 - c->ht, c->H_global, c->nodir_cnt.as<unsigned int>()));
    MH_TRY(stage_end(c, MHIP_STAGE_FLOWDIR, s));
    c->have[MHIP_R_FLOWDIR] = true;
    c->flowdir_own = true;
    c->nodir_valid = !c->ht && !c->hb;
    return MHIP_OK;
}

static int stage_flowdir_fused(mhip_ctx *c, hipStream_t s)
{
    MH_TRY(stage_begin(c, MHIP_STAGE_FLOWDIR, s));
    MH_TRY(stage_end(c, MHIP_STAGE_FLOWDIR, s));
    ctx_wrote(c, MHIP_R_FLOWDIR);
    c->have[MHIP_R_FLOWDIR] = true;
    c->nodir_valid = true;
    c->flowdir_own = true;
    return MHIP_OK;
}

static int stage_accum(mhip_ctx *c, hipStream_t s, PourLink *pour = nullptr, AccumPrep *prep = nullptr)
{
    MH_ARG(c->have[MHIP_R_FLOWDIR], "ACCUM needs flow directions");
    MH_TRY(ctx_raster(c, MHIP_R_ACCUM));
    MH_TRY(stage_begin(c, MHIP_STAGE_ACCUM, s));
    bool delta_done = false;
    if ((c->ht || c->hb) && c->acc_keep.valid)
        MH_TRY(accum_band_delta_dev(c->r[MHIP_R_FLOWDIR].as<uint8_t>(), c->r[MHIP_R_ACCUM].as<double>(), c->H, c->W, s, c->ht, c->hb, &c->acc_keep, &delta_done));
    c->accum_algorithm = delta_done ? 1 : 0;
    ctx_wrote(c, MHIP_R_ACCUM);
    if (!delta_done)
        MH_TRY(accum_dev(c->r[MHIP_R_FLOWDIR].as<uint8_t>(), c->r[MHIP_R_ACCUM].as<double>(), c->H, c->W, s, c->ht, c->hb, 0, nullptr, pour, nullptr,
                         prep));
    MH_TRY(stage_end(c, MHIP_STAGE_ACCUM, s));
    c->have[MHIP_R_ACCUM] = true;
    return MHIP_OK;
}

static int stage_label(mhip_ctx *c, hipStream_t s)
{
    const int64_t H = c->H, W = c->W, n = H * W;
    MH_ARG(c->have[MHIP_R_DEPTHS] || c->have[MHIP_R_FILLED], "LABEL needs bluespot depths");
    MH_TRY(ctx_raster(c, MHIP_R_LABELS));
    if (!c->tmp_i32.p) MH_TRY(c->tmp_i32.alloc(4 * (size_t)n));
    MH_TRY(stage_begin(c, MHIP_STAGE_LABEL, s));
    if (!c->have[MHIP_R_DEPTHS]) MH_TRY(stage_depths(c, s));
    ctx_wrote(c, MHIP_R_LABELS);
    MH_TRY(ccl8_f32_dev(c->r[MHIP_R_DEPTHS].as<float>(), c->r[MHIP_R_LABELS].as<int32_t>(), c->tmp_i32.as<int32_t>(), H, W,
                        &c->nlabels_raw, s, &c->raw_stats));
    MH_TRY(stage_end(c, MHIP_STAGE_LABEL, s));
    c->have[MHIP_R_LABELS] = true;
    c->labels_components = true;
    c->labels_filtered = false;
    c->nlabels = c->nlabels_raw;
    return MHIP_OK;
}

static int pour_link_buffers(mhip_ctx *c, PourLink *pl, hipStream_t s)
{
    const int64_t H = c->H, W = c->W;
    const int64_t ntiles = cdiv(H, 64) * cdiv(W, 64);
    MH_TRY(c->pp_mask0.alloc(2 * 256 * (size_t)ntiles));
    MH_TRY(c->pp_list.alloc(8 * (size_t)POUR_TILE_CAP * (size_t)ntiles));
    MH_TRY(c->pp_tiles.alloc(12 * (size_t)ntiles));
    MH_TRY(c->pp_misc.alloc(16));
    MH_TRY(c->pp_key.alloc(8 * (size_t)(c->nlabels + 1)));
    MH_HIP(hipMemsetAsync(c->pp_misc.p, 0, 16, s));
    MH_HIP(hipMemsetAsync(c->pp_key.p, 0, 8 * (size_t)(c->nlabels + 1), s));
    pl->dev.mask0 = c->pp_mask0.as<uint16_t>();
    pl->dev.list = c->pp_list.as<uint2>();
    pl->dev.tile_key0 = c->pp_tiles.as<unsigned long long>();
    pl->dev.tile_cnt = reinterpret_cast<uint32_t *>(c->pp_tiles.as<unsigned long long>() + ntiles);
    pl->dev.flags = c->pp_misc.as<uint32_t>() + 1;
    pl->dev.components = c->labels_components ? 1 : 0;
    pl->dev.key = c->pp_key.as<unsigned long long>();
    pl->dev.nlab = (uint32_t)c->nlabels;
    pl->ev = c->ev_cand;
    return MHIP_OK;
}

static int stage_watershed(mhip_ctx *c, hipStream_t s, PourLink *pour = nullptr)
{
    const int64_t H = c->H, W = c->W, n = H * W;
    MH_ARG(c->have[MHIP_R_LABELS] && c->have[MHIP_R_FLOWDIR], "WATERSHED needs labels and flow directions");
    MH_TRY(ctx_ensure_labels_final(c, s));
    MH_TRY(ctx_label_max(c, s));
    MH_TRY(ctx_raster(c, MHIP_R_WATERSHEDS));
    MH_TRY(stage_begin(c, MHIP_STAGE_WATERSHED, s));
    ctx_wrote(c, MHIP_R_WATERSHEDS);
    if (pour) MH_TRY(pour_link_buffers(c, pour, s));
    MH_TRY(watersheds_dev(c->r[MHIP_R_FLOWDIR].as<uint8_t>(), c->r[MHIP_R_WATERSHEDS].as<int32_t>(), H, W, 0, s, false,
                          c->nodir_valid ? c->nodir_cnt.as<unsigned int>() : nullptr, c->r[MHIP_R_LABELS].as<int32_t>(), pour));
    MH_TRY(c->ws_counts.alloc(8 * (size_t)(c->nlabels + 1)));
    MH_TRY(label_count_dev(c->r[MHIP_R_WATERSHEDS].as<int32_t>(), n, c->nlabels, c->ws_counts.as<int64_t>(), s, W));
    MH_TRY(stage_end(c, MHIP_STAGE_WATERSHED, s));
    c->have[MHIP_R_WATERSHEDS] = true;
    c->ws_counts_valid = true;
    return MHIP_OK;
}

static int stage_pourpoints(mhip_ctx *c, hipStream_t s, PourLink *pour = nullptr)
{
    const int64_t H = c->H, W = c->W;
    MH_ARG(c->have[MHIP_R_LABELS] && (c->have[MHIP_R_ACCUM] || c->have[MHIP_R_NOFLAT]),
           "POURPOINTS needs labels and accumulated flow or the no-flats surface");
    MH_TRY(ctx_ensure_labels_final(c, s));
    MH_TRY(ctx_label_max(c, s));
    MH_TRY(c->pour.alloc(sizeof(mhip_index_record) * (size_t)(c->nlabels + 1)));
    double *g = nullptr;
    if (!c->have[MHIP_R_ACCUM]) MH_TRY(ctx_noflat(c, &g));
    MH_TRY(stage_begin(c, MHIP_STAGE_POURPOINTS, s));
    bool from_keys = false;
    if (pour && pour->consumed && c->have[MHIP_R_ACCUM]) {
        uint32_t h[3] = {0, 1, 1};
        MH_HIP(hipMemcpyAsync(h, c->pp_misc.p, 12, hipMemcpyDeviceToHost, s));
        MH_TRY(pour_finish_dev(c->pp_key.as<unsigned long long>(), c->pp_tiles.as<unsigned long long>(), cdiv(H, 64) * cdiv(W, 64), c->nlabels, W,
                               c->pour.as<mhip_index_record>(), s));
        MH_HIP(stream_sync(s));
        from_keys = !h[1] && !h[2];
    }
    c->pour_algorithm = from_keys ? 1 : 0;
    if (from_keys) {
    } else if (c->have[MHIP_R_ACCUM])
        MH_TRY(label_arg_dev(c->r[MHIP_R_ACCUM].as<double>(), c->r[MHIP_R_LABELS].as<int32_t>(), H, W, c->nlabels, true,
                             c->pour.as<mhip_index_record>(), s, c->labels_components));
    else
        MH_TRY(label_arg_dev(g, c->r[MHIP_R_LABELS].as<int32_t>(), H, W, c->nlabels, false, c->pour.as<mhip_index_record>(), s));
    MH_TRY(stage_end(c, MHIP_STAGE_POURPOINTS, s));
    c->pour_valid = true;
    return MHIP_OK;
}

static int label_start_env()
{
    const char *e = dev_env("MHIP_LABEL_START");
    const int v = e ? atoi(e) : LABEL_START_DEFAULT;
    return v >= 0 && v <= 3 ? v : LABEL_START_DEFAULT;
}

extern "C" int mhip_ctx_run(mhip_ctx *c, int mask)
{
    MH_ARG(c, "ctx");
    MH_HIP(hipSetDevice(c->device));
    hipStream_t s = c->stream;
    if (c->nranks > 1 || c->ht || c->hb) {
        MH_ARG((mask & ~(MHIP_STAGE_FLOWDIR | MHIP_STAGE_ACCUM)) == 0,
               "this stage runs through the band entry points on a row band (mhip_ctx_fill_*, mhip_ctx_band_*)");
    }
    const bool serial_env = [] { const char *e = dev_env("MHIP_SERIAL"); return e && e[0] == '1'; }();
    const int side_a = mask & (MHIP_STAGE_NOFLAT | MHIP_STAGE_FLOWDIR | MHIP_STAGE_ACCUM);
    const int side_b = mask & (MHIP_STAGE_LABEL | MHIP_STAGE_WATERSHED);
    const bool overlap = side_a && side_b && !serial_env;
    FillHandover handover;
    FillHandover *const ho =
        ((mask & MHIP_STAGE_FILL) && (mask & MHIP_STAGE_NOFLAT) && c->nranks == 1 && !c->ht && !c->hb && fill_handover_env()) ? &handover : nullptr;
    c->fill_handover = 0;

    if (!overlap) {
        if (mask & MHIP_STAGE_FILL) MH_TRY(stage_fill(c, s, true, ho));
        bool fd_done = false;
        if (mask & MHIP_STAGE_NOFLAT) MH_TRY(stage_noflat(c, s, false, nullptr, (mask & MHIP_STAGE_FLOWDIR) != 0, &fd_done, ho));
        if (mask & MHIP_STAGE_FLOWDIR) MH_TRY(fd_done ? stage_flowdir_fused(c, s) : stage_flowdir(c, s));
        if (mask & MHIP_STAGE_ACCUM) MH_TRY(stage_accum(c, s));
        if (mask & MHIP_STAGE_LABEL) MH_TRY(stage_label(c, s));
        if (mask & MHIP_STAGE_WATERSHED) MH_TRY(stage_watershed(c, s));
        if (mask & MHIP_STAGE_POURPOINTS) MH_TRY(stage_pourpoints(c, s));
        return MHIP_OK;
    }

    StageTimer *t;
    for (int st : {MHIP_STAGE_FILL, MHIP_STAGE_NOFLAT, MHIP_STAGE_FLOWDIR, MHIP_STAGE_ACCUM, MHIP_STAGE_LABEL, MHIP_STAGE_WATERSHED,
                   MHIP_STAGE_POURPOINTS})
        if (mask & st) MH_TRY(ctx_timer(c, st, &t));
    auto side_stream = [&](hipStream_t *st) -> int {
        int least = 0, greatest = 0;
        MH_HIP(hipDeviceGetStreamPriorityRange(&least, &greatest));
        MH_HIP(hipStreamCreateWithPriority(st, hipStreamNonBlocking, least));
        return MHIP_OK;
    };
    if (!c->stream_b) MH_TRY(side_stream(&c->stream_b));
    if (!c->stream_c) MH_TRY(side_stream(&c->stream_c));
    MH_TRY(ctx_fork_join_events(c));
    if (!c->ev_cand) MH_HIP(hipEventCreateWithFlags(&c->ev_cand, hipEventDisableTiming));
    if (!c->ev_prep) MH_HIP(hipEventCreateWithFlags(&c->ev_prep, hipEventDisableTiming));
    hipStream_t sb = c->stream_b;
    const bool do_fill = (mask & MHIP_STAGE_FILL) != 0;
    MH_ARG(c->have[MHIP_R_DEM] || !(mask & (MHIP_STAGE_FILL | MHIP_STAGE_NOFLAT)), "FILL / NOFLAT need the DEM");

    std::promise<int> fill_done, shdg_done, flowdir_ready, label_ready, tail_reached;
    std::future<int> fill_fut = fill_done.get_future(), shdg_fut = shdg_done.get_future(), tail_fut = tail_reached.get_future();
    struct TailCtx {
        mhip_ctx *c;
        std::promise<int> *p;
        FillHandover *ho;
    } tail_ctx{c, &tail_reached, ho};
    StageHook tail_hook;
    tail_hook.arg = &tail_ctx;
    tail_hook.fn = [](void *arg, hipStream_t st) {
        TailCtx *t = static_cast<TailCtx *>(arg);
        ctx_handover_settled(t->c, t->ho);
        t->p->set_value(hipEventRecord(t->c->ev_tail, st) == hipSuccess ? MHIP_OK : MHIP_EHIP);
    };
    std::future<int> flowdir_fut = flowdir_ready.get_future(), label_fut = label_ready.get_future();
    struct CandHand {
        std::promise<int> p;
        std::future<int> f;
        std::atomic<bool> set{false};
    } cand_hand;
    cand_hand.f = cand_hand.p.get_future();
    PourLink pour_link;
    pour_link.arg = &cand_hand;
    pour_link.notify = [](void *a, int v) {
        CandHand *h = static_cast<CandHand *>(a);
        if (!h->set.exchange(true)) h->p.set_value(v);
    };
    pour_link.wait = [](void *a) { return static_cast<CandHand *>(a)->f.get(); };
    static const bool pour_pass = [] { const char *e = dev_env("MHIP_POUR"); return e && std::string(e) == "pass"; }();
    PourLink *const pour = ((mask & MHIP_STAGE_ACCUM) && (mask & MHIP_STAGE_WATERSHED) && (mask & MHIP_STAGE_POURPOINTS) && !pour_pass) ? &pour_link : nullptr;
    AccumPrep acc_prep;
    const bool prep_accum = (mask & MHIP_STAGE_ACCUM) && (mask & (MHIP_STAGE_NOFLAT | MHIP_STAGE_FLOWDIR)) && !c->ht && !c->hb;
    const bool ws_needs_new_flowdir = (mask & MHIP_STAGE_WATERSHED) && (mask & MHIP_STAGE_FLOWDIR);
    int rc_b = MHIP_OK;
    char err_b[512] = "";
    bool shdg_set = false, label_set = false;
    c->side.run([&] {
        rc_b = [&]() -> int {
            MH_HIP(hipSetDevice(c->device));
            int rc_e = MHIP_OK;
            if ((mask & MHIP_STAGE_NOFLAT) && !do_fill) rc_e = short_diag_dev(c->r[MHIP_R_DEM].as<float>(), c->H * c->W, &c->sh, &c->dg, sb);
            if (rc_e != MHIP_OK) snprintf(err_b, sizeof(err_b), "%s", get_error());
            shdg_done.set_value(rc_e);
            shdg_set = true;
            int rc_l = rc_e == MHIP_OK ? fill_fut.get() : rc_e;
            if (rc_l == MHIP_OK) rc_l = tail_fut.get();
            if (rc_l == MHIP_OK && hipStreamWaitEvent(sb, c->ev_tail, 0) != hipSuccess) rc_l = MHIP_EHIP;
            if (rc_l == MHIP_OK && (mask & MHIP_STAGE_LABEL)) rc_l = stage_label(c, sb);
            else if (rc_l == MHIP_OK && do_fill && !c->have[MHIP_R_DEPTHS]) rc_l = stage_depths(c, sb);
            if (rc_l == MHIP_OK && (mask & (MHIP_STAGE_WATERSHED | MHIP_STAGE_POURPOINTS)) && c->have[MHIP_R_LABELS]) {
                rc_l = ctx_ensure_labels_final(c, sb);
                if (rc_l == MHIP_OK) rc_l = ctx_label_max(c, sb);
            }
            if (rc_l == MHIP_OK && hipEventRecord(c->ev_label, sb) != hipSuccess) rc_l = MHIP_EHIP;
            if (rc_l != MHIP_OK && !err_b[0]) snprintf(err_b, sizeof(err_b), "%s", get_error());
            label_ready.set_value(rc_l);
            label_set = true;
            MH_TRY(rc_l);
            hipStream_t sw = sb;
            if (mask & MHIP_STAGE_WATERSHED) {
                sw = c->stream_c;
                MH_HIP(hipStreamWaitEvent(sw, c->ev_label, 0));
                if (ws_needs_new_flowdir) {
                    MH_TRY(flowdir_fut.get());
                    MH_HIP(hipStreamWaitEvent(sw, c->ev_flowdir, 0));
                }
                MH_TRY(stage_watershed(c, sw, pour));
            }
            MH_HIP(hipEventRecord(c->ev_join, sw));
            return MHIP_OK;
        }();
        if (rc_b != MHIP_OK && !err_b[0]) snprintf(err_b, sizeof(err_b), "%s", get_error());
        if (!shdg_set) shdg_done.set_value(rc_b);
        if (!label_set) label_ready.set_value(rc_b);
        pour_link.notify(pour_link.arg, 0);
    });
    int rc_a = MHIP_OK;
    if (do_fill) rc_a = stage_fill(c, s, false, ho);
    if (rc_a == MHIP_OK && hipEventRecord(c->ev_fork, s) != hipSuccess) rc_a = MHIP_EHIP;
    fill_done.set_value(rc_a);
    const int rc_e = shdg_fut.get();
    if (rc_a == MHIP_OK) rc_a = [&]() -> int {
        MH_TRY(rc_e);
        if (do_fill && (mask & MHIP_STAGE_NOFLAT)) {
            if (c->fill_st.have_minmax) short_diag_from_minmax(c->fill_st.dem_min, c->fill_st.dem_max, c->fill_st.dem_nan, &c->sh, &c->dg);
            else MH_TRY(short_diag_dev(c->r[MHIP_R_DEM].as<float>(), c->H * c->W, &c->sh, &c->dg, s));
        }
        if (prep_accum) MH_TRY(accum_prepare_dev(&acc_prep, c->H, c->W, c->stream_c, c->ev_prep));
        const int label_start = label_start_env();
        const bool owed = ho && ho->pending;
        if (label_start == 0 && !owed) tail_hook.fire(s);
        tail_hook.at = label_start;
        const bool armed = label_start == StageHook::TAIL_ROUNDS || label_start == StageHook::FINISH || (label_start == StageHook::FIRST_VISIT && owed);
        bool fd_done = false;
        if (mask & MHIP_STAGE_NOFLAT)
            MH_TRY(stage_noflat(c, s, true, armed ? &tail_hook : nullptr, (mask & MHIP_STAGE_FLOWDIR) != 0, &fd_done, ho));
        if (mask & MHIP_STAGE_FLOWDIR) {
            MH_TRY(fd_done ? stage_flowdir_fused(c, s) : stage_flowdir(c, s));
            MH_HIP(hipEventRecord(c->ev_flowdir, s));
        }
        return MHIP_OK;
    }();
    tail_hook.fire(s);
    flowdir_ready.set_value(rc_a);
    if (rc_a == MHIP_OK && (mask & MHIP_STAGE_ACCUM)) rc_a = stage_accum(c, s, pour, &acc_prep);
    const int rc_l = label_fut.get();
    if (rc_a == MHIP_OK && rc_l == MHIP_OK && (mask & MHIP_STAGE_POURPOINTS)) {
        rc_a = hipStreamWaitEvent(s, c->ev_label, 0) == hipSuccess ? stage_pourpoints(c, s, pour) : MHIP_EHIP;
    }
    c->side.wait();
    if (rc_a != MHIP_OK) return rc_a;
    if (rc_b != MHIP_OK) {
        set_error("%s", err_b);
        return rc_b;
    }
    MH_HIP(hipStreamWaitEvent(s, c->ev_join, 0));
    return MHIP_OK;
}
```

malstroem_amd/csrc/handover_addr.hpp:

```cpp
#pragma once
#include <cstdint>

#if defined(__HIPCC__) || defined(__CUDACC__)
#define MH_HD __host__ __device__
#else
#define MH_HD
#endif

namespace mh {
namespace ho {

constexpr int WN = 64;
constexpr int TI = 62;
constexpr int NBMAX = 1024;

struct Win {
    int64_t H, W;
    int ntr, ntc, ti, tj;
    int64_t r0, c0;
    int last_row;
    int border_row;
    int tib, tjb;
};

MH_HD inline Win window(int64_t H, int64_t W, int ntr, int ntc, int ti, int tj)
{
    Win w;
    w.H = H; w.W = W; w.ntr = ntr; w.ntc = ntc; w.ti = ti; w.tj = tj;
    w.r0 = (int64_t)ti * TI;
    w.c0 = (int64_t)tj * TI;
    w.last_row = (int)(H - 1 - w.r0 < WN - 1 ? H - 1 - w.r0 : WN - 1);
    w.border_row = (int)(H - 1 - w.r0 < 2 * WN ? H - 1 - w.r0 : 2 * WN);
    w.tib = ti > 0 ? ti - 1 : 0;
    w.tjb = tj > 0 ? tj - 1 : 0;
    return w;
}

MH_HD inline int row_of(const Win &w, int r) { return r < w.last_row ? r : w.last_row; }
MH_HD inline int col_of(const Win &w, int lane) { return w.c0 + lane < w.W ? lane : (int)(w.W - 1 - w.c0); }
MH_HD inline int64_t cell_index(const Win &w, int r, int lane) { return (w.r0 + row_of(w, r)) * w.W + w.c0 + col_of(w, lane); }

MH_HD inline bool border_row(const Win &w, int r) { return ((w.ti == 0) & (r == 0)) | (r >= w.border_row); }
MH_HD inline bool border_col(const Win &w, int lane) { return ((w.tj == 0) & (lane == 0)) | (w.c0 + lane >= w.W - 1); }

MH_HD inline int tile_row(const Win &w, int r)
{
    const int t = w.ti + (r == WN - 1 ? 1 : 0) - (r == 0 ? 1 : 0);
    return t < 0 ? 0 : (t > w.ntr - 1 ? w.ntr - 1 : t);
}
MH_HD inline int tile_col(const Win &w, int lane)
{
    const int t = w.tj + (lane == WN - 1 ? 1 : 0) - (lane == 0 ? 1 : 0);
    return t < 0 ? 0 : (t > w.ntc - 1 ? w.ntc - 1 : t);
}
MH_HD inline int64_t tab_origin(const Win &w) { return ((int64_t)w.tib * w.ntc + w.tjb) * NBMAX; }
MH_HD inline uint32_t tab_row_words(const Win &w, int r) { return (uint32_t)(tile_row(w, r) - w.tib) * (uint32_t)w.ntc * (uint32_t)NBMAX; }
MH_HD inline uint32_t tab_lane_words(const Win &w, int lane) { return (uint32_t)(tile_col(w, lane) - w.tjb) * (uint32_t)NBMAX; }
MH_HD inline uint32_t tab_slot(uint32_t slot, bool border) { return border ? 0u : (slot < (uint32_t)NBMAX - 1u ? slot : (uint32_t)NBMAX - 1u); }
MH_HD inline int64_t tab_index(const Win &w, int r, int lane, uint32_t slot, bool border)
{
    return tab_origin(w) + tab_row_words(w, r) + tab_lane_words(w, lane) + tab_slot(slot, border);
}
MH_HD inline int64_t tab_words_behind_origin(const Win &w) { return (int64_t)w.ntr * w.ntc * NBMAX - tab_origin(w); }

MH_HD inline bool own_row(const Win &w, int r) { return ((r >= 1) & (r <= TI) & (r <= w.last_row)) | ((w.ti == 0) & (r == 0)) | (r == w.border_row); }
MH_HD inline bool own_col(const Win &w, int lane)
{
    const int64_t c = w.c0 + lane;
    return (c < w.W) & (((lane >= 1) & (lane <= TI)) | ((w.tj == 0) & (lane == 0)) | (c == w.W - 1));
}
MH_HD inline int64_t store_index(const Win &w, int r, int lane) { return (w.r0 + r) * w.W + w.c0 + lane; }

}
}
```

malstroem_amd/csrc/noflat_geo.hip:

```cpp
#include <algorithm>
#include <cmath>
#include <cstdlib>
#include <mutex>
#include <string>
#include <type_traits>
#include <vector>

#include "common.hpp"
#include "handover_addr.hpp"

namespace mh {

namespace {

constexpr int WN = 64;
constexpr int TI = 62;
constexpr uint32_t DINF = 0xE0000000u;
constexpr uint32_t WMAX = 1u << 28;
constexpr uint32_t D_IRR = 0xFFFFFFFFu;
constexpr uint32_t M_NOFLAT = 0xFF00u;
constexpr uint32_t M_IRR = 0xFD00u;
constexpr uint32_t M_WALL = 0xFE00u;
constexpr int DPP_WF_SL1 = 0x130;
constexpr int DPP_WF_SR1 = 0x138;
#ifndef NG_MAXCYC
#define NG_MAXCYC 1
#endif
enum { C_IRREGULAR = 0, C_UNREACHED = 1, C_MISMATCH = 2, C_FATAL = 3, C_PROOF = 4, C_STATS = 8 };
static_assert(WN == ho::WN && TI == ho::TI, "handover_addr.hpp cuts the raster like this file");

__device__ __forceinline__ uint32_t from_left(uint32_t v) { return (uint32_t)__builtin_amdgcn_update_dpp(0, (int)v, DPP_WF_SR1, 0xf, 0xf, true); }
__device__ __forceinline__ uint32_t from_right(uint32_t v) { return (uint32_t)__builtin_amdgcn_update_dpp(0, (int)v, DPP_WF_SL1, 0xf, 0xf, true); }

__device__ __forceinline__ float fleft(float v)
{
    return __int_as_float(__builtin_amdgcn_update_dpp(0x7f800000, __float_as_int(v), DPP_WF_SR1, 0xf, 0xf, false));
}
__device__ __forceinline__ float fright(float v)
{
    return __int_as_float(__builtin_amdgcn_update_dpp(0x7f800000, __float_as_int(v), DPP_WF_SL1, 0xf, 0xf, false));
}

__device__ __forceinline__ uint32_t class_above(float V)
{
    const uint32_t b = __float_as_uint(V), ex = (b >> 23) & 0xffu;
    const uint32_t e = ((b >> 31) && (b & 0x7fffffu) == 0u) ? ex - 1u : ex;
    return (ex == 0u || ex == 255u) ? 255u : e;
}
__device__ __forceinline__ double class_ulp(uint32_t e) { return __longlong_as_double((long long)(e + 1023u - 127u - 52u) << 52); }

struct GeoArgs {
    int64_t H, W;
    int ntr, ntc, nt;
    const float *F;
    uint32_t *d;
    uint32_t *blk;
    uint32_t *hdr;
    uint8_t *mark;
    const int *list;
    const uint32_t *count;
    const uint32_t *tab;
    unsigned long long *counters;
    int maxcyc;
    int append, round_next;
    int *amark;
    int *list_next;
    uint32_t *count_next;
    int fixed_top, fixed_bot;
    const float *ho_dem;
    const uint16_t *ho_bslot;
    const uint32_t *ho_tabV;
    float *ho_F, *ho_depths;
};

template <int R> __device__ __forceinline__ void lds_put(uint32_t addr, uint32_t v) { asm volatile("ds_write_b32 %0, %1 offset:%2" : : "v"(addr), "v"(v), "n"(R) : "memory"); }
template <int R> __device__ __forceinline__ uint32_t lds_get(uint32_t addr)
{
    uint32_t v;
    asm volatile("ds_read_b32 %0, %1 offset:%2" : "=v"(v) : "v"(addr), "n"(R) : "memory");
    return v;
}
__device__ __forceinline__ void lds_wait() { asm volatile("s_waitcnt lgkmcnt(0)" : : : "memory"); }
template <int R0, int N> __device__ __forceinline__ void lds_put_rows(uint32_t addr, const uint32_t (&x)[WN])
{
    if constexpr (N > 0) {
        lds_put<R0 * (WN + 1) * 4>(addr, x[R0]);
        lds_put_rows<R0 + 1, N - 1>(addr, x);
    }
}
template <int R0, int N> __device__ __forceinline__ void lds_get_rows(uint32_t addr, uint32_t (&x)[WN])
{
    if constexpr (N > 0) {
        x[R0] = lds_get<R0 * (WN + 1) * 4>(addr);
        lds_get_rows<R0 + 1, N - 1>(addr, x);
    }
}
template <int C0, int N> __device__ __forceinline__ void lds_get_cols(uint32_t addr, uint32_t (&x)[WN])
{
    if constexpr (N > 0) {
        x[C0] = lds_get<C0 * 4>(addr);
        lds_get_cols<C0 + 1, N - 1>(addr, x);
    }
}
__device__ __forceinline__ void transpose32(uint32_t (&x)[WN], uint32_t scr_b, int lane)
{
    lds_put_rows<0, WN>(scr_b + 4u * lane, x);
    lds_wait();
    lds_get_cols<0, WN>(scr_b + 4u * (WN + 1) * lane, x);
    lds_wait();
#pragma unroll
    for (int c = 0; c < WN; ++c) asm volatile("" : "+v"(x[c]));
}

struct LaneW {
    __device__ __forceinline__ void get(uint32_t mword, const uint32_t *tab_l, uint32_t &s, uint32_t &g) const
    {
        const uint32_t e = (mword >> 8) & 0xffu;
        s = tab_l[e];
        g = tab_l[256 + e];
    }
};

template <bool DOWN, typename WT>
__device__ __forceinline__ void pass(uint32_t (&d)[WN], uint32_t (&ni)[WN], const WT wt, const uint32_t *tab_l, uint32_t &acc_all,
                                     uint32_t &acc_first, uint32_t &acc_last)
{
    constexpr int first = DOWN ? 1 : TI, dir = DOWN ? 1 : -1;
    constexpr int bC = DOWN ? 0 : 4, bL = DOWN ? 7 : 5, bR = DOWN ? 1 : 3;
#pragma unroll
    for (int r = 0; r < WN; ++r) asm volatile("" : "+v"(d[r]), "+v"(ni[r]));
#pragma unroll
    for (int i = 0; i < TI; ++i) {
        const int r = first + dir * i;
        const uint32_t behind = d[r - dir];
        const uint32_t bl = from_left(behind), br = from_right(behind);
        const uint32_t w = ni[r];
        uint32_t S, G;
        wt.get(w, tab_l, S, G);
        const uint32_t c0 = (behind + S) | (uint32_t)__builtin_amdgcn_sbfe((int)w, bC, 1);
        const uint32_t c1 = (bl + G) | (uint32_t)__builtin_amdgcn_sbfe((int)w, bL, 1);
        const uint32_t c2 = (br + G) | (uint32_t)__builtin_amdgcn_sbfe((int)w, bR, 1);
        const uint32_t cu = d[r];
        const uint32_t nv = min(min(c0, c1), min(c2, cu));
        const uint32_t x = nv ^ cu;
        acc_all |= x;
        asm volatile("" : "+v"(acc_all));
        if (r == 1) acc_first |= (w & 0x83u) != 0x83u ? x : 0u;
        if (r == TI) acc_last |= (w & 0x38u) != 0x38u ? x : 0u;
        d[r] = nv;
        __builtin_amdgcn_sched_barrier(0);
    }
}

template <typename WT>
__device__ __forceinline__ void relax(uint32_t (&d)[WN], uint32_t (&ni)[WN], const WT wt, const uint32_t *tab_l, uint32_t scr_b, int lane, int maxcyc,
                                      unsigned &wake, bool &changed, bool &capped, unsigned &cycles)
{
    const uint64_t INNER = ((1ull << TI) - 1) << 1, B1 = 2ull, B62 = 1ull << TI;
    capped = true;
#pragma nounroll
    for (int cyc = 0; cyc < maxcyc; ++cyc) {
        uint64_t chg = 0;
        ++cycles;
#pragma nounroll
        for (int half = 0; half < 2; ++half) {
            uint32_t acc_all = 0, acc_first = 0, acc_last = 0;
            pass<true>(d, ni, wt, tab_l, acc_all, acc_first, acc_last);
            pass<false>(d, ni, wt, tab_l, acc_all, acc_first, acc_last);
            const uint64_t all = __ballot(acc_all != 0), fst = __ballot(acc_first != 0), lst = __ballot(acc_last != 0);
            chg |= all;
            const unsigned e_first = (fst & INNER) ? 1u : 0u, e_last = (lst & INNER) ? 1u : 0u;
            const unsigned l1 = (all & B1) ? 1u : 0u, l62 = (all & B62) ? 1u : 0u;
            const unsigned f1 = (fst & B1) ? 1u : 0u, f62 = (fst & B62) ? 1u : 0u, g1 = (lst & B1) ? 1u : 0u, g62 = (lst & B62) ? 1u : 0u;
            if (half == 0)
                wake |= (e_first << 1) | (e_last << 7) | (l1 << 3) | (l62 << 5) | (f1 << 0) | (f62 << 2) | (g1 << 6) | (g62 << 8);
            else
                wake |= (e_first << 3) | (e_last << 5) | (l1 << 1) | (l62 << 7) | (f1 << 0) | (f62 << 6) | (g1 << 2) | (g62 << 8);
            transpose32(d, scr_b, lane);
#pragma unroll
            for (int r = 0; r < WN; ++r) ni[r] = __builtin_amdgcn_alignbit(ni[r], ni[r], 16);
        }
        changed |= chg != 0;
        if (!chg) {
            capped = false;
            break;
        }
    }
}

constexpr int NMK = 9;
#define NG_DPP " row_mask:0xf bank_mask:0xf bound_ctrl:1\n\t"
#define NG_ROW(O, I, B, BIT)                                                                                                                 \
    "v_add_u32 %[u], %[" B "], %[S]\n\t"                                                                                                    \
    "v_add_u32_dpp %[t], %[" B "], %[G] wave_shr:1" NG_DPP                                                                                   \
    "v_add_u32_dpp %[k], %[" B "], %[G] wave_shl:1" NG_DPP                                                                                   \
    "v_min3_u32 %[t], %[u], %[t], %[k]\n\t"                                                                                                 \
    "v_bfe_i32 %[k], %[m], " BIT ", 1\n\t"                                                                                                  \
    "v_min_u32 %[" O "], %[t], %[" I "]\n\t"                                                                                                \
    "v_bfi_b32 %[" O "], %[k], %[" I "], %[" O "]\n\t"                                                                                      \
    "v_bitop3_b32 %[acc], %[" O "], %[acc], %[" I "] bitop3:0xde\n\t"
template <int R, int DIR>
__device__ __forceinline__ void rows6_wl(uint32_t (&d)[WN], const uint32_t m, const uint32_t S, const uint32_t G, uint32_t &acc)
{
    static_assert((R >> 5) == ((R + 5 * DIR) >> 5), "one mask word a block");
    uint32_t o0, o1, o2, o3, o4, o5, u, t, k;
    if constexpr (DIR > 0)
        asm volatile(NG_ROW("o0", "i0", "b", "%[bit]") NG_ROW("o1", "i1", "o0", "%[bit]+1") NG_ROW("o2", "i2", "o1", "%[bit]+2")
                     NG_ROW("o3", "i3", "o2", "%[bit]+3") NG_ROW("o4", "i4", "o3", "%[bit]+4") NG_ROW("o5", "i5", "o4", "%[bit]+5")
                     : [o0] "=&v"(o0), [o1] "=&v"(o1), [o2] "=&v"(o2), [o3] "=&v"(o3), [o4] "=&v"(o4), [o5] "=&v"(o5), [u] "=&v"(u), [t] "=&v"(t),
                       [k] "=&v"(k), [acc] "+v"(acc)
                     : [b] "v"(d[R - DIR]), [i0] "v"(d[R]), [i1] "v"(d[R + DIR]), [i2] "v"(d[R + 2 * DIR]), [i3] "v"(d[R + 3 * DIR]),
                       [i4] "v"(d[R + 4 * DIR]), [i5] "v"(d[R + 5 * DIR]), [S] "v"(S), [G] "v"(G), [m] "v"(m), [bit] "n"(R & 31));
    else
        asm volatile(NG_ROW("o0", "i0", "b", "%[bit]") NG_ROW("o1", "i1", "o0", "%[bit]-1") NG_ROW("o2", "i2", "o1", "%[bit]-2")
                     NG_ROW("o3", "i3", "o2", "%[bit]-3") NG_ROW("o4", "i4", "o3", "%[bit]-4") NG_ROW("o5", "i5", "o4", "%[bit]-5")
                     : [o0] "=&v"(o0), [o1] "=&v"(o1), [o2] "=&v"(o2), [o3] "=&v"(o3), [o4] "=&v"(o4), [o5] "=&v"(o5), [u] "=&v"(u), [t] "=&v"(t),
                       [k] "=&v"(k), [acc] "+v"(acc)
                     : [b] "v"(d[R - DIR]), [i0] "v"(d[R]), [i1] "v"(d[R + DIR]), [i2] "v"(d[R + 2 * DIR]), [i3] "v"(d[R + 3 * DIR]),
                       [i4] "v"(d[R + 4 * DIR]), [i5] "v"(d[R + 5 * DIR]), [S] "v"(S), [G] "v"(G), [m] "v"(m), [bit] "n"(R & 31));
    d[R] = o0; d[R + DIR] = o1; d[R + 2 * DIR] = o2; d[R + 3 * DIR] = o3; d[R + 4 * DIR] = o4; d[R + 5 * DIR] = o5;
}
template <int R, int DIR>
__device__ __forceinline__ uint32_t row1_wl(uint32_t (&d)[WN], const uint32_t m, const uint32_t S, const uint32_t G, uint32_t &acc)
{
    uint32_t o0, u, t, k;
// ... 264 lines not shown
        acc_last |= row1_open<TI, -1>(d, ring, S, G, acc_all);
        __builtin_amdgcn_sched_barrier(0);
        blocks_open<TI - 1, -1, 10>(d, ring, S, G, acc_all);
        acc_first |= row1_open<1, -1>(d, ring, S, G, acc_all);
    }
    __builtin_amdgcn_sched_barrier(0);
}

__device__ __forceinline__ void relax_open(uint32_t (&d)[WN], const uint32_t S, const uint32_t G, uint32_t scr_b, int lane, int maxcyc, unsigned &wake,
                                           bool &changed, bool &capped, unsigned &cycles)
{
    const uint64_t INNER = ((1ull << TI) - 1) << 1, B1 = 2ull, B62 = 1ull << TI;
    const bool ring_lane = (lane == 0) | (lane == WN - 1);
    capped = true;
#pragma nounroll
    for (int cyc = 0; cyc < maxcyc; ++cyc) {
        uint64_t chg = 0;
        ++cycles;
#pragma nounroll
        for (int half = 0; half < 2; ++half) {
            uint32_t acc_all = 0, acc_first = 0, acc_last = 0;
            pass_open<true>(d, S, G, ring_lane, acc_all, acc_first, acc_last);
            pass_open<false>(d, S, G, ring_lane, acc_all, acc_first, acc_last);
            const uint64_t all = __ballot(acc_all != 0), fst = __ballot(acc_first != 0), lst = __ballot(acc_last != 0);
            chg |= all;
            const unsigned e_first = (fst & INNER) ? 1u : 0u, e_last = (lst & INNER) ? 1u : 0u;
            const unsigned l1 = (all & B1) ? 1u : 0u, l62 = (all & B62) ? 1u : 0u;
            const unsigned f1 = (fst & B1) ? 1u : 0u, f62 = (fst & B62) ? 1u : 0u, g1 = (lst & B1) ? 1u : 0u, g62 = (lst & B62) ? 1u : 0u;
            if (half == 0) wake |= (e_first << 1) | (e_last << 7) | (l1 << 3) | (l62 << 5) | (f1 << 0) | (f62 << 2) | (g1 << 6) | (g62 << 8);
            else wake |= (e_first << 3) | (e_last << 5) | (l1 << 1) | (l62 << 7) | (f1 << 0) | (f62 << 6) | (g1 << 2) | (g62 << 8);
            transpose32(d, scr_b, lane);
        }
        changed |= chg != 0;
        if (!chg) {
            capped = false;
            break;
        }
    }
}

constexpr uint32_t HDR_ACTIVE = 1u << 31, HDR_UNIFORM = 1u << 9, HDR_OPEN = 1u << 10, HDR_TWO = 1u << 11;
template <bool FIRST, bool HANDOVER = false>
__device__ __forceinline__ void visit(const GeoArgs &a, int t, const uint32_t *tab_l, uint32_t scr_b, int lane, unsigned &visits, unsigned &cycles)
{
#ifdef NG_PROFILE
    const long long tp0 = __builtin_amdgcn_s_memtime();
#endif
    const int64_t H = a.H, W = a.W;
    const int ti = t / a.ntc, tj = t - ti * a.ntc;
    const int64_t r0 = (int64_t)ti * TI, c0 = (int64_t)tj * TI;
    const int64_t cc = c0 + lane;
    const bool col_in = cc < W;
    const uint32_t lane_c = (uint32_t)(col_in ? lane : W - 1 - c0);

    const int64_t org = r0 * W + c0;
    const __amdgpu_buffer_rsrc_t rd = __builtin_amdgcn_make_buffer_rsrc((void *)(a.d + org), 0, 0x7fffffff, 0x00020000);
    const __amdgpu_buffer_rsrc_t rb = __builtin_amdgcn_make_buffer_rsrc((void *)(a.blk + (int64_t)t * (WN * WN)), 0, WN * WN * 4, 0x00020000);
    int Wi = (int)W;
    asm volatile("" : "+s"(Wi));
    const int last_row = (int)(H - 1 - r0 < WN - 1 ? H - 1 - r0 : WN - 1);
    uint32_t ni[WN], d[WN], mk[NMK2];
    uint32_t hdr;
    if constexpr (FIRST) {
        const __amdgpu_buffer_rsrc_t rf = __builtin_amdgcn_make_buffer_rsrc((void *)(a.F + org), 0, 0x7fffffff, 0x00020000);
        const bool ring_lane = (lane == 0) | (lane == WN - 1);
        const bool lane_in = (lane >= 1) & (lane <= TI) & (cc < W - 1);
        const bool lane_border = (tj == 0 && lane == 0) | (cc >= W - 1);
        const float PINF = __builtin_inff();
        const int border_row = (int)(H - 1 - r0 < 2 * WN ? H - 1 - r0 : 2 * WN);
        uint32_t lake_any = 0, nirr = 0, nfatal = 0;
        uint32_t proof_bad = 0;
        auto classify = [&](auto inner_tag) {
            constexpr bool INNER = decltype(inner_tag)::value;
            const bool lane_in_c = INNER ? ((lane >= 1) & (lane <= TI)) : lane_in;
            float f[WN];
            uint32_t raised[2] = {0u, 0u};
            if constexpr (!HANDOVER) {
                int so = 0;
#pragma unroll
                for (int r = 0; r < WN; ++r) {
                    f[r] = __uint_as_float(__builtin_amdgcn_raw_buffer_load_b32(rf, (int)((INNER ? (uint32_t)lane : lane_c) * 4u), INNER ? r * Wi * 4 : so * 4, 0));
                    so = r < last_row ? so + Wi : so;
                }
            } else {
                const ho::Win w = ho::window(H, W, a.ntr, a.ntc, ti, tj);
                const int64_t tab0 = ho::tab_origin(w), tab_left = ho::tab_words_behind_origin(w) * 4;
                const __amdgpu_buffer_rsrc_t re = __builtin_amdgcn_make_buffer_rsrc((void *)(a.ho_dem + org), 0, 0x7fffffff, 0x00020000);
                const __amdgpu_buffer_rsrc_t rs = __builtin_amdgcn_make_buffer_rsrc((void *)(a.ho_bslot + org), 0, 0x7fffffff, 0x00020000);
                const __amdgpu_buffer_rsrc_t rt =
                    __builtin_amdgcn_make_buffer_rsrc((void *)(a.ho_tabV + tab0), 0, (int)(tab_left < 0x7fffffff ? tab_left : 0x7fffffff), 0x00020000);
                const __amdgpu_buffer_rsrc_t rF = __builtin_amdgcn_make_buffer_rsrc((void *)(a.ho_F + org), 0, 0x7fffffff, 0x00020000);
                const __amdgpu_buffer_rsrc_t rD =
                    __builtin_amdgcn_make_buffer_rsrc((void *)(a.ho_depths ? a.ho_depths + org : a.ho_F), 0, a.ho_depths ? 0x7fffffff : 0, 0x00020000);
                const uint32_t col_read = INNER ? (uint32_t)lane : (uint32_t)ho::col_of(w, lane);
                const bool bcol = INNER ? false : ho::border_col(w, lane);
                const uint32_t lane_bytes = ho::tab_lane_words(w, lane) * 4u;
                const int row_bytes_top = (int)(ho::tab_row_words(w, 0) * 4u), row_bytes_mid = (int)(ho::tab_row_words(w, 1) * 4u),
                          row_bytes_bot = (int)(ho::tab_row_words(w, WN - 1) * 4u);
                const bool ocol = INNER ? lane_in_c : ho::own_col(w, lane);
                volatile __attribute__((address_space(3))) uint32_t *const scr_p = (volatile __attribute__((address_space(3))) uint32_t *)(uintptr_t)scr_b + lane;
                uint32_t below = 0u;
                constexpr int QR = 16;
                uint32_t sl[WN];
                auto load_q = [&](int q) {
#pragma unroll
                    for (int r = q * QR; r < (q + 1) * QR; ++r) {
                        const int so = INNER ? r * Wi : (r < last_row ? r : last_row) * Wi;
                        f[r] = __uint_as_float(__builtin_amdgcn_raw_buffer_load_b32(re, (int)(col_read * 4u), so * 4, 0));
                        sl[r] = (uint32_t)(uint16_t)__builtin_amdgcn_raw_buffer_load_b16(rs, (int)(col_read * 2u), so * 2, 0);
                    }
                    __builtin_amdgcn_sched_barrier(0);
                };
                auto gather_q = [&](int q) {
#pragma unroll
                    for (int r = q * QR; r < (q + 1) * QR; ++r) {
                        const bool border = INNER ? false : (bcol | ho::border_row(w, r));
                        sl[r] = __builtin_amdgcn_raw_buffer_load_b32(rt, (int)(lane_bytes + ho::tab_slot(sl[r], border) * 4u),
                                                                     r == 0 ? row_bytes_top : (r == WN - 1 ? row_bytes_bot : row_bytes_mid), 0);
                    }
                    __builtin_amdgcn_sched_barrier(0);
                };
                auto finish_q = [&](int q) {
#pragma unroll
                    for (int r = q * QR; r < (q + 1) * QR; ++r) {
                        const bool border = INNER ? false : (bcol | ho::border_row(w, r));
                        const float e = f[r];
                        const float lev = key_f32(max(dem_key(e), sl[r]));
                        const float v = border ? e : lev;
                        raised[r >> 5] |= v > e ? 1u << (r & 31) : 0u;
                        below |= v < e ? 1u : 0u;
                        asm volatile("" : "+v"(below), "+v"(raised[r >> 5]));
                        if ((INNER ? (r >= 1 && r <= TI) : ho::own_row(w, r)) && ocol) {
                            __builtin_amdgcn_raw_buffer_store_b32(__float_as_uint(v), rF, lane * 4, r * Wi * 4, 0);
                            __builtin_amdgcn_raw_buffer_store_b32(__float_as_uint(v - e), rD, lane * 4, r * Wi * 4, 0);
                        }
                        scr_p[r * (WN + 1)] = __float_as_uint(v);
                        __builtin_amdgcn_sched_barrier(0);
                    }
                };
                load_q(0);
                load_q(1);
                gather_q(0);
                load_q(2);
                gather_q(1);
                finish_q(0);
                load_q(3);
                gather_q(2);
                finish_q(1);
                gather_q(3);
                finish_q(2);
                finish_q(3);
                proof_bad |= below;
                asm volatile("" : "+v"(raised[0]), "+v"(raised[1]));
                lds_wait();
                __builtin_amdgcn_sched_barrier(0);
                lds_get_rows<0, WN>(scr_b + 4u * lane, sl);
                lds_wait();
#pragma unroll
                for (int r = 0; r < WN; ++r) {
                    asm volatile("" : "+v"(sl[r]));
                    f[r] = __uint_as_float(sl[r]);
                }
                __builtin_amdgcn_sched_barrier(0);
            }
            float upl = PINF, up = PINF, upr = PINF, cul = fleft(f[0]), cur = fright(f[0]);
            float h_up = PINF, h_cu = fminf(fminf(cul, f[0]), cur);
            uint32_t e_cu = class_above(f[0]), tv_cu = tab_l[e_cu & 0xffu];
#pragma unroll
            for (int r = 0; r < WN; ++r) {
                const float V = f[r], dn = r + 1 < WN ? f[r + 1] : PINF;
                const float dnl = r + 1 < WN ? fleft(dn) : PINF, dnr = r + 1 < WN ? fright(dn) : PINF;
                const float h_dn = fminf(fminf(dnl, dn), dnr);
                const bool lower = fminf(fminf(h_up, h_dn), fminf(cul, cur)) < V;
                h_up = h_cu;
                h_cu = h_dn;
                const bool border = INNER ? false : (lane_border | (ti == 0 && r == 0 && !a.fixed_top) | (r == border_row && !a.fixed_bot) | (r > border_row));
                const bool src = lower | border;
                const bool ring = (r == 0) | (r == WN - 1) | ring_lane | (INNER ? false : (r >= border_row));
                const uint32_t adj = (up == V ? 1u : 0u) | (upr == V ? 2u : 0u) | (cur == V ? 4u : 0u) | (dnr == V ? 8u : 0u) |
                                     (dn == V ? 16u : 0u) | (dnl == V ? 32u : 0u) | (cul == V ? 64u : 0u) | (upl == V ? 128u : 0u);
                const uint32_t e = e_cu, tv = tv_cu;
                e_cu = r + 1 < WN ? class_above(dn) : 255u;
                tv_cu = tab_l[e_cu & 0xffu];
                const bool cell = lane_in_c & !border & !ring;
                const bool flat = cell & !src;
                const bool regular = flat & (adj != 0u) & (e < 253u) & (tv != 0u);
                const bool nan = cell & (V != V);
                const bool irregular = flat & !regular & !nan;
                nirr += irregular ? 1u : 0u;
                nfatal += nan ? 1u : 0u;
                if constexpr (HANDOVER) proof_bad |= (cell & lower) ? raised[r >> 5] & (1u << (r & 31)) : 0u;
                const uint32_t w = regular ? (adj | (e << 8)) : (irregular ? M_IRR : M_NOFLAT);
                lake_any |= w;
                ni[r] = w;
                upl = cul; up = V; upr = cur;
                cul = dnl; cur = dnr;
                __builtin_amdgcn_sched_barrier(0);
            }
            {
                auto arow = [&](int r) -> uint32_t {
                    if (r < 0 || r >= WN) return 0u;
                    const uint32_t q = (ni[r] & 0xffu) != 0u ? (~ni[r] & 0xffu) : 0u;
                    return (q & 0x11u) | (from_left(q) & 0x0eu) | (from_right(q) & 0xe0u);
                };
                uint32_t Ap = 0u, Ac = arow(0);
#pragma unroll
                for (int r = 0; r < WN; ++r) {
                    const uint32_t An = arow(r + 1);
                    const uint32_t hit = (An & 0x83u) | (Ap & 0x38u) | (Ac & 0x44u);
                    ni[r] = (hit != 0u && (ni[r] & 0xffu) == 0u) ? M_WALL : ni[r];
                    Ap = Ac; Ac = An;
                    asm volatile("" : "+v"(ni[r]), "+v"(Ap), "+v"(Ac));
                    __builtin_amdgcn_sched_barrier(0);
                }
            }
            {
                auto trow = [&](int r) -> uint32_t {
                    const uint32_t c = (ni[r] & 0xff00u) == M_WALL ? 1u : 0u;
                    return c | (from_left(c) << 1) | (from_right(c) << 2);
                };
                uint32_t P = trow(0), C = trow(1);
#pragma unroll
                for (int r = 1; r <= TI; ++r) {
                    const uint32_t N = trow(r + 1);
                    const uint32_t nb = (P & 1u) | ((P & 4u) >> 1) | (C & 4u) | ((N & 4u) << 1) | ((N & 1u) << 4) | ((N & 2u) << 4) | ((C & 2u) << 5) | ((P & 2u) << 6);
                    const uint32_t w = ni[r], sb = w & nb;
                    const uint32_t e = (w >> 8) & 0xffu;
                    uint32_t seeded = DINF;
                    if (__any(sb != 0u)) {
                        const uint32_t S = tab_l[e], G = tab_l[256 + e];
                        seeded = min((sb & 0x55u) ? S : DINF, (sb & 0xaau) ? G : DINF);
                    }
                    const uint32_t d0 = (w & 0xffu) != 0u ? seeded : ((w & 0xff00u) == M_IRR ? D_IRR : 0u);
                    if ((INNER || r < last_row) && lane_in_c) __builtin_amdgcn_raw_buffer_store_b32(d0, rd, lane * 4, r * Wi * 4, 0);
                    P = C; C = N;
                    asm volatile("" : "+v"(P), "+v"(C));
                    __builtin_amdgcn_sched_barrier(0);
                }
            }
        };
        if (ti > 0 && tj > 0 && H - 1 - r0 > WN - 1 && c0 + WN - 1 < W - 1) classify(std::true_type{});
        else classify(std::false_type{});
        {
            uint32_t tot = nirr | (nfatal << 16);
#pragma unroll
            for (int o = 32; o >= 1; o >>= 1) tot += (uint32_t)__shfl_xor((int)tot, o);
            if ((tot & 0xffffu) && lane == 0) atomicAdd(&a.counters[C_IRREGULAR], (unsigned long long)(tot & 0xffffu));
            if ((tot >> 16) && lane == 0) atomicAdd(&a.counters[C_FATAL], (unsigned long long)(tot >> 16));
        }
        if constexpr (HANDOVER) {
            if (__any(proof_bad != 0u) && lane == 0) a.counters[C_PROOF] = 1ull;
        }
        if (ti == 0 || tj == 0 || H - 1 - r0 <= WN - 1 || c0 + WN - 1 >= W - 1) {
#pragma unroll
            for (int r = 0; r < WN; ++r) {
                const bool brow = (ti == 0 && r == 0 && !a.fixed_top) | (r == last_row && last_row == (int)(H - 1 - r0) && !a.fixed_bot);
                const bool halo = (ti == 0 && r == 0 && a.fixed_top) | (r == last_row && last_row == (int)(H - 1 - r0) && a.fixed_bot);
                const bool bcell = r <= last_row && col_in && !halo && (brow | (tj == 0 && lane == 0) | (cc == W - 1));
                if (bcell) __builtin_amdgcn_raw_buffer_store_b32(0u, rd, lane * 4, r * Wi * 4, 0);
            }
        }
        if (!__any((lake_any & 0xffu) != 0u)) {
            if (lane == 0) a.hdr[t] = 0u;
            return;
        }
        __builtin_amdgcn_sched_barrier(0);
        {
            uint32_t tw[WN];
#pragma unroll
            for (int r = 0; r < WN; ++r) {
                const uint32_t adj = ni[r] & 0xffu;
                tw[r] = (__builtin_bitreverse32(adj << 25) | (adj & 0x80u)) | (ni[r] & 0xff00u);
            }
            lds_put_rows<0, WN>(scr_b + 4u * lane, tw);
            lds_wait();
            lds_get_cols<0, 32>(scr_b + 4u * (WN + 1) * lane, tw);
            lds_wait();
#pragma unroll
            for (int r = 0; r < 32; ++r) {
                asm volatile("" : "+v"(tw[r]));
                ni[r] = (ni[r] | (tw[r] << 16)) ^ 0x00ff00ffu;
            }
            lds_get_cols<32, 32>(scr_b + 4u * (WN + 1) * lane, tw);
            lds_wait();
#pragma unroll
            for (int r = 32; r < WN; ++r) {
                asm volatile("" : "+v"(tw[r]));
                ni[r] = (ni[r] | (tw[r] << 16)) ^ 0x00ff00ffu;
            }
        }
        __builtin_amdgcn_sched_barrier(0);
        auto fresh = [&]() {
#pragma unroll
            for (int r = 0; r < WN; ++r) asm volatile("" : "+v"(ni[r]));
        };
        uint32_t esel = 255u;
        fresh();
#pragma unroll
        for (int r = 1; r <= TI; ++r) esel = (ni[r] & 0xffu) != 0xffu ? (ni[r] >> 8) & 0xffu : esel;
        const uint64_t has = __ballot(esel != 255u);
        const uint32_t eref = (uint32_t)__builtin_amdgcn_readlane((int)esel, (int)__builtin_ctzll(has));
        uint32_t mism = 0;
        fresh();
#pragma unroll
        for (int r = 1; r <= TI; ++r) mism |= (ni[r] & 0xffu) != 0xffu ? ((ni[r] >> 8) & 0xffu) ^ eref : 0u;
        unsigned seams = 1u << 4;
// ... 190 lines not shown
#endif
}

template <bool FIRST, int WPB = 4, bool HANDOVER = false>
__device__ __forceinline__ void round_body(const GeoArgs &a)
{
    extern __shared__ __attribute__((aligned(16))) uint32_t lds[];
    const int lane = threadIdx.x & 63;
    const int wave = __builtin_amdgcn_readfirstlane(threadIdx.x >> 6);
    const uint32_t scr_b = (uint32_t)(uintptr_t)(__attribute__((address_space(3))) uint32_t *)(lds + wave * (WN * (WN + 1)));
    uint32_t *tab_l = lds + WPB * (WN * (WN + 1));
    const int nwaves = (int)gridDim.x * WPB, gw = (int)blockIdx.x * WPB + wave;
    uint32_t tw[512 / (64 * WPB)];
#pragma unroll
    for (int k = 0; k < 512 / (64 * WPB); ++k) tw[k] = a.tab[threadIdx.x + k * 64 * WPB];
    const int n = FIRST ? a.nt : (int)__builtin_amdgcn_readfirstlane((int)*a.count);
    const int t_first = FIRST ? 0 : a.list[gw < a.nt ? gw : a.nt - 1];
#pragma unroll
    for (int k = 0; k < 512 / (64 * WPB); ++k) tab_l[threadIdx.x + k * 64 * WPB] = tw[k];
    __syncthreads();
    unsigned visits = 0, cycles = 0;
    for (int i = gw; i < n; i += nwaves) {
        const int t = FIRST ? i : __builtin_amdgcn_readfirstlane(i == gw ? t_first : a.list[i]);
        visit<FIRST, HANDOVER>(a, t, tab_l, scr_b, lane, visits, cycles);
    }
    if (lane == 0 && visits) {
        unsigned long long *st = a.counters + C_STATS + 2 * (gw & 63);
        atomicAdd(&st[0], (unsigned long long)visits);
        atomicAdd(&st[1], (unsigned long long)cycles);
    }
}
__global__ __launch_bounds__(256, 2) void ng_first_kernel(GeoArgs a) { round_body<true>(a); }
__global__ __launch_bounds__(256, 2) void ng_round_kernel(GeoArgs a) { round_body<false>(a); }
__global__ __launch_bounds__(64, 2) void ng_round_w1_kernel(GeoArgs a) { round_body<false, 1>(a); }
__global__ __launch_bounds__(256, 2) void ng_handover_kernel(GeoArgs a) { round_body<true, 4, true>(a); }

__global__ __launch_bounds__(256) void ng_compact_kernel(unsigned long long *mark8, int nwords, int *list, uint32_t *count)
{
    __shared__ uint32_t n_l, base_l;
    if (threadIdx.x == 0) n_l = 0;
    __syncthreads();
    const int w = (int)blockIdx.x * 256 + (int)threadIdx.x;
    const unsigned long long v = w < nwords ? mark8[w] : 0ull;
    unsigned k = 0;
    uint32_t o = 0;
    if (v) {
        mark8[w] = 0;
#pragma unroll
        for (int j = 0; j < 8; ++j) k += ((v >> (8 * j)) & 0xffull) ? 1u : 0u;
        o = atomicAdd(&n_l, k);
    }
    __syncthreads();
    if (threadIdx.x == 0) base_l = n_l ? atomicAdd(count, n_l) : 0u;
    __syncthreads();
    if (v) {
        o += base_l;
#pragma unroll
        for (int j = 0; j < 8; ++j)
            if ((v >> (8 * j)) & 0xffull) list[o++] = 8 * w + j;
    }
}

__device__ __forceinline__ double ng_value(float f, uint32_t dd, double seed_add, bool *beyond)
{
    *beyond = false;
    if (dd == D_IRR) return (double)f + seed_add;
    if (dd >= 0x80000000u) {
        *beyond = true;
        return (double)f + seed_add;
    }
    return dd ? (double)f + (double)dd * class_ulp(class_above(f)) : (double)f;
}

__global__ __launch_bounds__(256) void ng_assemble_kernel(const float *__restrict__ F, const uint32_t *__restrict__ d, double *__restrict__ G, int64_t n,
                                                          double seed_add, unsigned long long *counters)
{
    const int64_t i0 = ((int64_t)blockIdx.x * 256 + threadIdx.x) * 4;
    if (i0 >= n) return;
    unsigned bad = 0;
    auto value = [&](float f, uint32_t dd) {
        bool beyond;
        const double v = ng_value(f, dd, seed_add, &beyond);
        bad += beyond ? 1u : 0u;
        return v;
    };
    if (i0 + 4 <= n) {
        const float4 f = *reinterpret_cast<const float4 *>(F + i0);
        const uint4 dv = *reinterpret_cast<const uint4 *>(d + i0);
        typedef double __attribute__((ext_vector_type(2))) v2d;
        *reinterpret_cast<v2d *>(G + i0) = v2d{value(f.x, dv.x), value(f.y, dv.y)};
        *reinterpret_cast<v2d *>(G + i0 + 2) = v2d{value(f.z, dv.z), value(f.w, dv.w)};
    } else {
        for (int64_t i = i0; i < n; ++i) G[i] = value(F[i], d[i]);
    }
    if (bad && counters) atomicAdd(&counters[C_UNREACHED], (unsigned long long)bad);
}

constexpr int VRB = 16;
__global__ __launch_bounds__(256) void ng_verify_kernel(const float *__restrict__ dem, const double *__restrict__ G, int64_t H, int64_t W, double sh,
                                                        double dg, int fixed_top, int fixed_bot, unsigned long long *counters)
{
    const int64_t c = (int64_t)blockIdx.x * 256 + threadIdx.x;
    const int64_t rb = (int64_t)blockIdx.y * VRB;
    if (c >= W) return;
    const double PINF = __builtin_inf();
    const bool cl = c > 0, cr = c + 1 < W;
    auto row = [&](int64_t r, double (&v)[3]) {
        const bool in = r >= 0 && r < H;
        const double *p = G + (in ? r : 0) * W + c;
        v[0] = (in && cl) ? p[-1] : PINF;
        v[1] = in ? p[0] : PINF;
        v[2] = (in && cr) ? p[1] : PINF;
    };
    double a[3], b[3], n[3];
    row(rb - 1, a);
    row(rb, b);
    unsigned bad = 0;
#pragma unroll 4
    for (int i = 0; i < VRB; ++i) {
        const int64_t r = rb + i;
        if (r >= H) break;
        row(r + 1, n);
        const double own = b[1], dv = (double)dem[r * W + c];
        double want = dv;
        if (r > 0 && r < H - 1 && cl && cr) {
            const double md = fmin(fmin(a[0], a[2]), fmin(n[0], n[2])) + dg;
            const double me = fmin(fmin(a[1], b[0]), fmin(b[2], n[1])) + sh;
            want = fmax(fmin(md, me), dv);
        }
        const bool halo = (r == 0 && fixed_top) || (r == H - 1 && fixed_bot);
        bad += (own == want || halo) ? 0u : 1u;
#pragma unroll
        for (int k = 0; k < 3; ++k) {
            a[k] = b[k];
            b[k] = n[k];
        }
    }
    if (bad) atomicAdd(&counters[C_MISMATCH], (unsigned long long)bad);
}

constexpr int FRB = 32;
__device__ __forceinline__ double dleft(double v)
{
    const uint64_t b = (uint64_t)__double_as_longlong(v);
    const uint32_t lo = from_left((uint32_t)b), hi = from_left((uint32_t)(b >> 32));
    return __longlong_as_double((long long)(((uint64_t)hi << 32) | lo));
}
__device__ __forceinline__ double dright(double v)
{
    const uint64_t b = (uint64_t)__double_as_longlong(v);
    const uint32_t lo = from_right((uint32_t)b), hi = from_right((uint32_t)(b >> 32));
    return __longlong_as_double((long long)(((uint64_t)hi << 32) | lo));
}
template <bool D8, bool STORE = true>
__global__ __launch_bounds__(256) void ng_finish_kernel(const float *__restrict__ F, const uint32_t *__restrict__ d, const float *__restrict__ dem,
                                                        double *__restrict__ G, int64_t H, int64_t W, double sh, double dg, double seed_add, int fixed_top,
                                                        int fixed_bot, unsigned long long *counters, uint8_t *__restrict__ flowdir, unsigned int *nodir)
{
    const int lane = threadIdx.x & 63, wave = threadIdx.x >> 6;
    const int64_t c = ((int64_t)blockIdx.x * 4 + wave) * TI + lane - 1;
    const int64_t rb = (int64_t)blockIdx.y * FRB;
    const bool col_in = c >= 0 && c < W;
    const int64_t cc = c < 0 ? 0 : (c < W ? c : W - 1);
    const bool mine = lane >= 1 && lane <= TI && col_in;
    const bool inner_col = c > 0 && c + 1 < W;
    const double PINF = __builtin_inf();
    unsigned unreached = 0, bad = 0, anynodir = 0;
    auto value = [&](int64_t r) -> double {
        if (!(r >= 0 && r < H && col_in)) return PINF;
        bool beyond;
        const double v = ng_value(F[r * W + cc], d[r * W + cc], seed_add, &beyond);
        unreached += beyond && mine && r >= rb && r < rb + FRB ? 1u : 0u;
        return v;
    };
    double a = value(rb - 1), b = value(rb);
    for (int i = 0; i < FRB; ++i) {
        const int64_t r = rb + i;
        if (r >= H) break;
        const double n = value(r + 1);
        const double al = dleft(a), ar = dright(a), bl = dleft(b), br = dright(b), nl = dleft(n), nr = dright(n);
        if (mine) {
            const double dv = (double)dem[r * W + c];
            double want = dv;
            if (r > 0 && r < H - 1 && inner_col) {
                const double md = fmin(fmin(al, ar), fmin(nl, nr)) + dg;
                const double me = fmin(fmin(a, bl), fmin(br, n)) + sh;
                want = fmax(fmin(md, me), dv);
            }
            const bool halo = (r == 0 && fixed_top) || (r == H - 1 && fixed_bot);
            bad += (b == want || halo) ? 0u : 1u;
            if (STORE) G[r * W + c] = b;
            if (D8) {
                unsigned code;
                if (r == 0 || r == H - 1 || c == 0 || c == W - 1) code = edge_code(r, c, H - 1, W - 1);
                else {
                    code = d8_code(b, a, ar, br, nr, n, nl, bl, al);
                    anynodir |= code == 8u ? 1u : 0u;
                }
                flowdir[r * W + c] = (uint8_t)code;
            }
        }
        a = b;
        b = n;
    }
    if (unreached) atomicAdd(&counters[C_UNREACHED], (unsigned long long)unreached);
    if (bad) atomicAdd(&counters[C_MISMATCH], (unsigned long long)bad);
    if (D8 && __any(anynodir != 0u) && lane == 0) *nodir = 1u;
}

#ifndef NG_FINISH_AHEAD
#define NG_FINISH_AHEAD 1
#endif
#ifndef NG_FINISH_WAVES
#define NG_FINISH_WAVES 8
#endif
#if NG_FINISH_WAVES < 8
#define NG_FINISH_RESIDENCY __attribute__((amdgpu_waves_per_eu(1, NG_FINISH_WAVES)))
#else
#define NG_FINISH_RESIDENCY
#endif
#if NG_FINISH_AHEAD
template <bool STORE>
__device__ __forceinline__ void ng_finish_ahead(const float *__restrict__ F, const uint32_t *__restrict__ d, const float *__restrict__ dem,
                                                double *__restrict__ G, int64_t H, int64_t W, double sh, double dg, double seed_add, int fixed_top,
                                                int fixed_bot, unsigned long long *counters, uint8_t *__restrict__ flowdir, unsigned int *nodir)
{
    const int lane = threadIdx.x & 63, wave = threadIdx.x >> 6;
    const int64_t c = ((int64_t)blockIdx.x * 4 + wave) * TI + lane - 1;
    const int64_t rb = (int64_t)blockIdx.y * FRB;
    const bool col_in = c >= 0 && c < W;
    const int64_t cc = c < 0 ? 0 : (c < W ? c : W - 1);
    const bool mine = lane >= 1 && lane <= TI && col_in;
    const bool inner_col = c > 0 && c + 1 < W;
    const double PINF = __builtin_inf();
    unsigned unreached = 0, bad = 0, anynodir = 0;
    struct Row {
        float f, z;
        uint32_t dd;
    };
    auto load = [&](int64_t r) -> Row {
        const int64_t at = (r < 0 ? 0 : (r < H ? r : H - 1)) * W + cc;
        return Row{F[at], dem[at], d[at]};
    };
    auto value = [&](int64_t r, const Row &x) -> double {
        if (!(r >= 0 && r < H && col_in)) return PINF;
        bool beyond;
        const double v = ng_value(x.f, x.dd, seed_add, &beyond);
        unreached += beyond && mine && r >= rb && r < rb + FRB ? 1u : 0u;
        return v;
    };
    const Row xa = load(rb - 1), xb = load(rb);
    Row x0 = load(rb + 1), x1{0.0f, 0.0f, 0u};
    double a = value(rb - 1, xa), b = value(rb, xb);
    double dvb = (double)xb.z;
    auto row = [&](int i, const Row &xn, Row &xnn, auto more) {
        const int64_t r = rb + i;
        const double dv = dvb;
        if (decltype(more)::value) xnn = load(r + 2);
        const double n = value(r + 1, xn);
        dvb = (double)xn.z;
        asm volatile("" : "+v"(dvb));
        const double al = dleft(a), ar = dright(a), bl = dleft(b), br = dright(b), nl = dleft(n), nr = dright(n);
        if (mine && r < H) {
            double want = dv;
            if (r > 0 && r < H - 1 && inner_col) {
                const double md = fmin(fmin(al, ar), fmin(nl, nr)) + dg;
                const double me = fmin(fmin(a, bl), fmin(br, n)) + sh;
                want = fmax(fmin(md, me), dv);
            }
            const bool halo = (r == 0 && fixed_top) || (r == H - 1 && fixed_bot);
            bad += (b == want || halo) ? 0u : 1u;
            if (STORE) G[r * W + c] = b;
            unsigned code;
            if (r == 0 || r == H - 1 || c == 0 || c == W - 1) code = edge_code(r, c, H - 1, W - 1);
            else {
                code = d8_code(b, a, ar, br, nr, n, nl, bl, al);
                anynodir |= code == 8u ? 1u : 0u;
            }
            flowdir[r * W + c] = (uint8_t)code;
        }
        a = b;
        b = n;
    };
    static_assert(FRB % 2 == 0, "rows in pairs");
    int i = 0;
    for (; i < FRB - 2 && rb + i < H; i += 2) {
        row(i, x0, x1, std::true_type());
        row(i + 1, x1, x0, std::true_type());
    }
    if (i == FRB - 2 && rb + i < H) {
        row(i, x0, x1, std::true_type());
        row(i + 1, x1, x0, std::false_type());
    }
    if (unreached) atomicAdd(&counters[C_UNREACHED], (unsigned long long)unreached);
    if (bad) atomicAdd(&counters[C_MISMATCH], (unsigned long long)bad);
    if (__any(anynodir != 0u) && lane == 0) *nodir = 1u;
}
#define NG_FINISH_AHEAD_KERNEL(STORE)                                                                                                                  \
    template <>                                                                                                                                        \
    __global__ __launch_bounds__(256) NG_FINISH_RESIDENCY void ng_finish_kernel<true, STORE>(                                                          \
        const float *__restrict__ F, const uint32_t *__restrict__ d, const float *__restrict__ dem, double *__restrict__ G, int64_t H, int64_t W,      \
        double sh, double dg, double seed_add, int fixed_top, int fixed_bot, unsigned long long *counters, uint8_t *__restrict__ flowdir,              \
        unsigned int *nodir)                                                                                                                           \
    {                                                                                                                                                  \
        ng_finish_ahead<STORE>(F, d, dem, G, H, W, sh, dg, seed_add, fixed_top, fixed_bot, counters, flowdir, nodir);                                  \
    }
NG_FINISH_AHEAD_KERNEL(true)
NG_FINISH_AHEAD_KERNEL(false)
#undef NG_FINISH_AHEAD_KERNEL
#endif

uint32_t class_weight(double eps, int e)
{
    if (!(eps > 0.0) || std::isinf(eps)) return 0;
    int q;
    const double fr = std::frexp(eps, &q);
    const uint64_t M = (uint64_t)std::ldexp(fr, 53);
    const int k = (e - 127 - 52) - (q - 53);
    if (k <= 24 || k > 52) return 0;
    const uint64_t half = 1ull << (k - 1), rem = M & ((1ull << k) - 1);
    if (rem == half) return 0;
    const uint64_t w = (M >> k) + (rem > half ? 1 : 0);
    return (w >= 1 && w < WMAX) ? (uint32_t)w : 0;
}

}

struct GeoRun::Impl {
    DevBuf ws;
    uint32_t *d_tab = nullptr, *d_any = nullptr, *d_hdr = nullptr, *d_blk = nullptr;
    unsigned long long *d_cnt = nullptr;
    uint8_t *d_mark = nullptr;
    int *d_list = nullptr, *d_list2 = nullptr, *d_amark = nullptr;
    int ntr = 0, ntc = 0, round = 0, used = 0;
    std::vector<std::pair<hipEvent_t, hipEvent_t>> span;
    int span_rounds = 0;
    uint32_t last_count = 0xffffffffu;
    bool light = false;
    int light_from = 0;
    int64_t nt = 0;
    size_t lds = 0;
    int maxcyc = NG_MAXCYC;
    bool debug = false;
    unsigned long long irregular = 0;
};
namespace {
constexpr int MAXR = 8192, BATCH = 32, BATCH_HEAD = 16;
constexpr uint32_t LIGHT_TILES = 6144;
__global__ void ng_mark_row_kernel(uint8_t *mark, int ti, int ntc)
{
    const int tj = blockIdx.x * blockDim.x + threadIdx.x;
    if (tj < ntc) mark[(int64_t)ti * ntc + tj] = 1;
}
}

GeoRun::GeoRun() : impl(new Impl) {}
GeoRun::~GeoRun()
{
    for (auto &e : impl->span) {
        (void)hipEventDestroy(e.first);
        (void)hipEventDestroy(e.second);
    }
    delete impl;
}

int GeoRun::launch_rounds(hipStream_t s, int nb)
{
    {
        Impl &mm = *impl;
        hipEvent_t e0, e1;
        MH_HIP(hipEventCreate(&e0));
        MH_HIP(hipEventCreate(&e1));
        mm.span.emplace_back(e0, e1);
        MH_HIP(hipEventRecord(e0, s));
    }
    struct CloseSpan {
        Impl &m;
        hipStream_t s;
        ~CloseSpan() { (void)hipEventRecord(m.span.back().second, s); }
    } close_span{*impl, s};
    Impl &m = *impl;
    GeoArgs a;
    a.H = H; a.W = W; a.ntr = m.ntr; a.ntc = m.ntc; a.nt = (int)m.nt; a.F = filled; a.d = dist; a.tab = m.d_tab; a.counters = m.d_cnt;
    a.blk = m.d_blk; a.hdr = m.d_hdr; a.mark = m.d_mark; a.list = m.d_list; a.fixed_top = fixed_top; a.fixed_bot = fixed_bot;
    a.append = 0; a.round_next = 0; a.amark = m.d_amark; a.list_next = nullptr; a.count_next = nullptr;
    a.ho_dem = nullptr; a.ho_bslot = nullptr; a.ho_tabV = nullptr; a.ho_F = nullptr; a.ho_depths = nullptr;
    const unsigned grid = (unsigned)std::min<int64_t>((m.nt + 3) / 4, 512);
    for (int k = 0; k < nb; ++k, ++m.round) {
        a.maxcyc = m.maxcyc;
        a.count = m.d_any + m.round;
        if (!m.round && handover && handover->pending) {
            a.ho_dem = handover->dem; a.ho_bslot = handover->bslot; a.ho_tabV = handover->tabV;
            a.ho_F = handover->filled; a.ho_depths = handover->depths;
            hipLaunchKernelGGL(ng_handover_kernel, dim3(grid), dim3(256), m.lds, s, a);
            handover->queued = true;
            (void)hipEventRecord(m.span.back().first, s);
            continue;
        }
        if (!m.round) {
            hipLaunchKernelGGL(ng_first_kernel, dim3(grid), dim3(256), m.lds, s, a);
            (void)hipEventRecord(m.span.back().first, s);
            continue;
        }
        if (!m.light || m.round == m.light_from)
            hipLaunchKernelGGL(ng_compact_kernel, dim3((unsigned)(((m.nt + 7) / 8 + 255) / 256)), dim3(256), 0, s, reinterpret_cast<unsigned long long *>(m.d_mark),
                               (int)((m.nt + 7) / 8), m.d_list, m.d_any + m.round);
        if (m.light) {
            const bool odd = ((m.round - m.light_from) & 1) != 0;
            a.append = 1;
            a.round_next = m.round + 1;
            a.list = odd ? m.d_list2 : m.d_list;
            a.list_next = odd ? m.d_list : m.d_list2;
            a.count_next = m.d_any + m.round + 1;
        }
        if (m.light && tail_hook && tail_hook->at == StageHook::TAIL_ROUNDS)
            hipLaunchKernelGGL(ng_round_w1_kernel, dim3((unsigned)std::min<int64_t>(m.nt, 2048)), dim3(64), (WN * (WN + 1) + 512) * sizeof(uint32_t), s, a);
        else
            hipLaunchKernelGGL(ng_round_kernel, dim3(grid), dim3(256), m.lds, s, a);
    }
    MH_HIP(hipGetLastError());
    return MHIP_OK;
}

int GeoRun::begin(hipStream_t s, bool *applicable, bool *active)
{
    Impl &m = *impl;
    static const bool off = [] { const char *e = dev_env("MHIP_NOFLAT"); return e && std::string(e) == "iterative"; }();
    m.debug = dev_env("MHIP_NG_DEBUG") != nullptr;
    *applicable = false;
    *active = false;
    if (off || !filled || H < 3 || W < 3) return MHIP_OK;
    if (!(sh > 0.0) || !(dg > 0.0) || std::isinf(sh) || std::isinf(dg)) return MHIP_OK;
    std::vector<uint32_t> tab(512, 0u);
    bool any_class = false;
    for (int e = 0; e < 255; ++e) {
        const uint32_t S = class_weight(sh, e), G = class_weight(dg, e);
        if (S && G) {
            tab[e] = S;
            tab[256 + e] = G;
            any_class = true;
        }
    }
    if (!any_class) return MHIP_OK;

    const int64_t n = H * W;
    m.ntr = (int)((H - 2 + TI - 1) / TI);
    m.ntc = (int)((W - 2 + TI - 1) / TI);
    m.nt = (int64_t)m.ntr * m.ntc;
    auto align = [](size_t x) { return (x + 255) & ~size_t(255); };
    const size_t o_d = 0, o_tab = align(o_d + (dist ? 0 : 4 * (size_t)n)), o_cnt = align(o_tab + 2048);
    const size_t o_any = align(o_cnt + 8 * (C_STATS + 128 + 16)), o_mark = align(o_any + 4 * (size_t)(MAXR + BATCH));
    const size_t o_amark = align(o_mark + (size_t)m.nt + 8), o_list = align(o_amark + 4 * (size_t)m.nt), o_list2 = align(o_list + 4 * (size_t)m.nt);
    const size_t o_hdr = align(o_list2 + 4 * (size_t)m.nt), o_blk = align(o_hdr + 4 * (size_t)m.nt);
    MH_TRY(m.ws.alloc(o_blk + 4 * (size_t)m.nt * WN * WN + 256));
    char *b = m.ws.as<char>();
    if (!dist) dist = reinterpret_cast<uint32_t *>(b + o_d);
    m.d_tab = reinterpret_cast<uint32_t *>(b + o_tab);
    m.d_cnt = reinterpret_cast<unsigned long long *>(b + o_cnt);
    m.d_any = reinterpret_cast<uint32_t *>(b + o_any);
    m.d_mark = reinterpret_cast<uint8_t *>(b + o_mark);
    m.d_list = reinterpret_cast<int *>(b + o_list);
    m.d_list2 = reinterpret_cast<int *>(b + o_list2);
    m.d_amark = reinterpret_cast<int *>(b + o_amark);
    m.d_hdr = reinterpret_cast<uint32_t *>(b + o_hdr);
    m.d_blk = reinterpret_cast<uint32_t *>(b + o_blk);
    MH_HIP(hipMemsetAsync(b + o_cnt, 0, o_list - o_cnt, s));
    MH_HIP(hipMemcpyAsync(m.d_tab, tab.data(), 2048, hipMemcpyHostToDevice, s));
    if (fixed_top) MH_HIP(hipMemsetAsync(dist, 0xE0, 4 * (size_t)W, s));
    if (fixed_bot) MH_HIP(hipMemsetAsync(dist + (H - 1) * W, 0xE0, 4 * (size_t)W, s));

    m.lds = (4 * WN * (WN + 1) + 512) * sizeof(uint32_t);
    {
        static std::mutex mu;
        static bool attr_done[64] = {};
        int dev = 0;
        MH_HIP(hipGetDevice(&dev));
        std::lock_guard<std::mutex> lk(mu);
        if (dev < 0 || dev >= 64 || !attr_done[dev]) {
            MH_HIP(hipFuncSetAttribute((const void *)ng_round_kernel, hipFuncAttributeMaxDynamicSharedMemorySize, (int)m.lds));
            MH_HIP(hipFuncSetAttribute((const void *)ng_first_kernel, hipFuncAttributeMaxDynamicSharedMemorySize, (int)m.lds));
            MH_HIP(hipFuncSetAttribute((const void *)ng_handover_kernel, hipFuncAttributeMaxDynamicSharedMemorySize, (int)m.lds));
            if (dev >= 0 && dev < 64) attr_done[dev] = true;
        }
    }
    m.round = 0;
    m.last_count = 0xffffffffu;
    m.used = 0;
    if (handover && handover->pending &&
        !(handover->ntr == m.ntr && handover->ntc == m.ntc && handover->H == H && handover->W == W && handover->filled == filled && handover->dem == dem &&
          !fixed_top && !fixed_bot))
        MH_TRY(fill_handover_complete(handover, s));
    const bool took = handover && handover->pending;
    MH_TRY(launch_rounds(s, 1));
    unsigned long long h_c[5] = {0, 0, 0, 0, 0};
    MH_HIP(hipMemcpyAsync(h_c, m.d_cnt, sizeof(h_c), hipMemcpyDeviceToHost, s));
    MH_HIP(stream_sync(s));
    if (took) {
        if (h_c[C_PROOF] != 0 || dev_env("MHIP_HO_RECHECK") != nullptr) {
            handover->suspect = true;
            m.ws.release();
            return MHIP_OK;
        }
        handover->release();
    }
    m.used = 1;
    m.irregular = h_c[C_IRREGULAR];
    if (h_c[C_FATAL] || (m.irregular && !allow_partial)) {
        if (m.debug) fprintf(stderr, "[noflat geodesic] %llu irregular flat cells, %llu NaN cells: float64 relaxation\n", m.irregular, h_c[C_FATAL]);
        return MHIP_OK;
    }
    *applicable = true;
    *active = true;
    return MHIP_OK;
}

int GeoRun::batch(hipStream_t s, bool *active)
{
    Impl &m = *impl;
    const char *eb = dev_env("MHIP_NG_BATCH");
    const int nb_env = eb && atoi(eb) >= 1 && atoi(eb) <= BATCH ? atoi(eb) : 0;
    for (;;) {
        const int nb = nb_env ? nb_env : (!m.light ? BATCH_HEAD : (m.last_count <= 64 ? 8 : (m.last_count <= 512 ? 16 : BATCH)));
        if (m.round + BATCH > MAXR) {
            set_error("no-flats fill (geodesic) did not converge within %d rounds", MAXR);
            return MHIP_ENOTCONV;
        }
        MH_TRY(launch_rounds(s, nb));
        if (tail_hook) tail_hook->fire_at(StageHook::TAIL_ROUNDS, s);
        uint32_t h_any[BATCH];
        MH_HIP(hipMemcpyAsync(h_any, m.d_any + (m.round - nb), sizeof(uint32_t) * nb, hipMemcpyDeviceToHost, s));
        MH_HIP(stream_sync(s));
        for (int k = 0; k < nb; ++k) {
            if (!h_any[k]) {
                *active = false;
                m.light = false;
                return MHIP_OK;
            }
            ++m.used;
        }
        m.last_count = h_any[nb - 1];
        if (!m.light && h_any[nb - 1] <= LIGHT_TILES) {
            m.light = true;
            m.light_from = m.round;
        }
    }
}

int GeoRun::halo_changed(int side, hipStream_t s)
{
    Impl &m = *impl;
    hipLaunchKernelGGL(ng_mark_row_kernel, dim3((unsigned)((m.ntc + 255) / 256)), dim3(256), 0, s, m.d_mark, side == 0 ? 0 : m.ntr - 1, m.ntc);
    MH_HIP(hipGetLastError());
    return MHIP_OK;
}

int GeoRun::end(hipStream_t s, bool *ok, FillStats *st)
{
    Impl &m = *impl;
    const int64_t n = H * W;
    partial = m.irregular != 0 && allow_partial;
    if (dev_env("MHIP_NG_CORRUPT") && W > 8)
        MH_HIP(hipMemsetAsync(dist + (H / 2) * W + 1, 0x01, 4 * (size_t)(W - 2), s));
    d8_done = false;
    const bool with_d8 = !partial && d8_out && d8_nodir && !fixed_top && !fixed_bot;
    if (tail_hook) tail_hook->fire_at(StageHook::FINISH, s);
    const bool no_store = with_d8 && defer_out;
    out_deferred = false;
    if (no_store)
        hipLaunchKernelGGL((ng_finish_kernel<true, false>), dim3((unsigned)((W + 4 * TI - 1) / (4 * TI)), (unsigned)((H + FRB - 1) / FRB)), dim3(256), 0, s, filled, dist,
                           dem, out, H, W, sh, dg, seed_add, fixed_top, fixed_bot, m.d_cnt, d8_out, d8_nodir);
    else if (with_d8)
        hipLaunchKernelGGL(ng_finish_kernel<true>, dim3((unsigned)((W + 4 * TI - 1) / (4 * TI)), (unsigned)((H + FRB - 1) / FRB)), dim3(256), 0, s, filled, dist, dem,
                           out, H, W, sh, dg, seed_add, fixed_top, fixed_bot, m.d_cnt, d8_out, d8_nodir);
    else if (!partial)
        hipLaunchKernelGGL(ng_finish_kernel<false>, dim3((unsigned)((W + 4 * TI - 1) / (4 * TI)), (unsigned)((H + FRB - 1) / FRB)), dim3(256), 0, s, filled, dist, dem,
                           out, H, W, sh, dg, seed_add, fixed_top, fixed_bot, m.d_cnt, (uint8_t *)nullptr, (unsigned int *)nullptr);
    else
        hipLaunchKernelGGL(ng_assemble_kernel, dim3((unsigned)((n + 1023) / 1024)), dim3(256), 0, s, filled, dist, out, n, seed_add, m.d_cnt);
    MH_HIP(hipGetLastError());
    unsigned long long h_all[C_STATS + 128 + 16];
    MH_HIP(hipMemcpyAsync(h_all, m.d_cnt, sizeof(h_all), hipMemcpyDeviceToHost, s));
    MH_HIP(stream_sync(s));
    if (allow_partial && h_all[C_UNREACHED]) partial = true;
    if (st) {
        *st = FillStats();
        st->geo_irregular = (int64_t)m.irregular;
        st->geo_unreached = (int64_t)h_all[C_UNREACHED];
        st->geo_mismatch = (int64_t)h_all[C_MISMATCH];
        st->rounds = m.used;
        st->tiles = m.nt;
        st->algorithm = partial ? 3 : 2;
        for (auto &e : m.span) {
            float ms = 0;
            if (hipEventElapsedTime(&ms, e.first, e.second) == hipSuccess) st->hot_ms += ms;
            else (void)hipGetLastError();
        }
        st->hot_launches = m.used > 0 ? m.used - 1 : 0;
        for (int k = 0; k < 64; ++k) {
            st->visits += (int64_t)h_all[C_STATS + 2 * k];
            st->cycles += (int64_t)h_all[C_STATS + 2 * k + 1];
        }
    }
    if (m.debug) {
        std::vector<uint32_t> cnt((size_t)m.round);
        MH_HIP(hipMemcpy(cnt.data(), m.d_any, 4 * (size_t)m.round, hipMemcpyDeviceToHost));
        unsigned long long v = 0, cy = 0;
        for (int k = 0; k < 64; ++k) {
            v += h_all[C_STATS + 2 * k];
            cy += h_all[C_STATS + 2 * k + 1];
        }
        fprintf(stderr, "[noflat geodesic] tiles %lld, visits %llu, cycles %llu; tiles per round:", (long long)m.nt, v, cy);
        for (int k = 1; k < m.round && k < 200; ++k) fprintf(stderr, " %u", cnt[k]);
#ifdef NG_PROFILE
        for (int o = 0; o < 2; ++o) {
            const unsigned long long *q = h_all + C_STATS + 128 + 8 * o;
            if (q[0]) fprintf(stderr, "\n[noflat visits, %s] %llu: ticks per visit: setup+issue %.0f, wait for loads %.0f, relax %.0f, store %.0f", o ? "open" : "masked", q[0],
                              (double)q[1] / q[0], (double)q[2] / q[0], (double)q[3] / q[0], (double)q[4] / q[0]);
        }
#endif
        fprintf(stderr, "\n[noflat geodesic] %lld x %lld: rounds %d, unreached %llu, mismatches %llu\n", (long long)H, (long long)W, m.used, h_all[C_UNREACHED],
                h_all[C_MISMATCH]);
    }
    *ok = partial ? true : !(h_all[C_UNREACHED] || h_all[C_MISMATCH]);
    d8_done = with_d8 && !partial && *ok;
    if (no_store) {
        if (d8_done) out_deferred = true;
        else MH_TRY(noflat_assemble_dev(filled, dist, out, n, seed_add, s));
    }
    m.ws.release();
    return MHIP_OK;
}

int noflat_assemble_dev(const float *d_filled, const uint32_t *d_dist, double *d_out, int64_t n, double seed_add, hipStream_t s)
{
    hipLaunchKernelGGL(ng_assemble_kernel, dim3((unsigned)((n + 1023) / 1024)), dim3(256), 0, s, d_filled, d_dist, d_out, n, seed_add,
                       (unsigned long long *)nullptr);
    MH_HIP(hipGetLastError());
    return MHIP_OK;
}

int noflat_verify_dev(const float *d_dem, const double *d_out, int64_t H, int64_t W, double sh, double dg, hipStream_t s, bool *ok, int fixed_top,
                      int fixed_bot)
{
    DevBuf cnt;
    MH_TRY(cnt.alloc(8 * (C_STATS + 128 + 16)));
    MH_HIP(hipMemsetAsync(cnt.p, 0, 8 * (C_STATS + 128), s));
    hipLaunchKernelGGL(ng_verify_kernel, dim3((unsigned)((W + 255) / 256), (unsigned)((H + VRB - 1) / VRB)), dim3(256), 0, s, d_dem, d_out, H, W, sh, dg, fixed_top,
                       fixed_bot, cnt.as<unsigned long long>());
    MH_HIP(hipGetLastError());
    unsigned long long bad = 0;
    MH_HIP(hipMemcpyAsync(&bad, cnt.as<unsigned long long>() + C_MISMATCH, 8, hipMemcpyDeviceToHost, s));
    MH_HIP(stream_sync(s));
    *ok = bad == 0;
    return MHIP_OK;
}

int fill_noflat_geodesic_dev(const float *d_dem, const float *d_filled, double *d_out, int64_t H, int64_t W, double sh, double dg, double seed_add,
                             hipStream_t s, FillStats *st, bool *partial, StageHook *tail_hook, D8Sink *d8, FillHandover *ho)
{
    GeoRun g;
    g.handover = ho;
    g.tail_hook = tail_hook;
    if (d8) {
        g.d8_out = d8->flowdir; g.d8_nodir = d8->nodir; d8->done = false; d8->deferred = false;
        if (d8->dist) g.dist = d8->dist;
        g.defer_out = d8->defer && d8->dist;
    }
    g.dem = d_dem; g.filled = d_filled; g.out = d_out; g.H = H; g.W = W; g.sh = sh; g.dg = dg;
    g.allow_partial = partial != nullptr && seed_add == seed_add && seed_add < 1e300;
    g.seed_add = seed_add;
    bool applicable = false, active = false, ok = false;
    MH_TRY(g.begin(s, &applicable, &active));
    if (ho && ho->pending) {
        const bool again = ho->suspect;
        MH_TRY(fill_handover_complete(ho, s));
        if (again) {
            g.handover = nullptr;
            MH_TRY(g.begin(s, &applicable, &active));
        }
    }
    if (tail_hook) tail_hook->fire_at(StageHook::FIRST_VISIT, s);
    if (!applicable) {
        if (st) st->geo_reject = 1;
        return MHIP_ELIMIT;
    }
    while (active) MH_TRY(g.batch(s, &active));
    MH_TRY(g.end(s, &ok, st));
    if (partial) *partial = g.partial;
    if (d8) { d8->done = g.d8_done; d8->deferred = g.out_deferred; }
    if (!ok && st) st->geo_reject = 2;
    return ok ? MHIP_OK : MHIP_ELIMIT;
}

}
```

Measured before the change: 12900 Mcells/s.

## Emit per-column wet bitmasks in handover and reuse them in finish and CCL

The handover kernel now writes a 64-bit per-column bitmask of raised (wet) rows per tile row into a new buffer. The no-flat finish kernel uses these bits instead of reading the f32 DEM, and the CCL tile kernel derives foreground from the bits instead of reading the f32 depths raster. This is meant to replace two full-raster float reads with reads of a bitmask about 1/64 the size per row-tile. The cost is an extra buffer, an extra store in the handover kernel, and new indexing logic whose correctness relies on the wet bits exactly matching depth>0 and the DEM comparison.

```diff
diff --git a/malstroem_amd/csrc/ccl.hip b/malstroem_amd/csrc/ccl.hip
--- a/malstroem_amd/csrc/ccl.hip
+++ b/malstroem_amd/csrc/ccl.hip
@@ -4,6 +4,7 @@
 #include <utility>
 
 #include "common.hpp"
+#include "handover_addr.hpp"
 
 namespace mh {
 namespace {
@@ -115,9 +116,10 @@
 #ifndef CCL_U3
 #define CCL_U3 4
 #endif
-template <typename T>
+template <typename T, bool WET = false>
 __global__ __launch_bounds__(256) void ccl_tile_kernel(const T *__restrict__ data, int32_t *__restrict__ parent, int64_t H, int64_t W, int ntc,
-                                                       int32_t *__restrict__ rootlist, int32_t *__restrict__ rootcount, int32_t *__restrict__ colpar)
+                                                       int32_t *__restrict__ rootlist, int32_t *__restrict__ rootcount, int32_t *__restrict__ colpar,
+                                                       const unsigned long long *__restrict__ wet = nullptr, int wet_ntr = 0)
 {
     __shared__ uint32_t par[CT * CT];
     __shared__ int s_nroots;
@@ -126,10 +128,19 @@
     const int ti = blockIdx.x / ntc, tj = blockIdx.x - ti * ntc;
     const int64_t r0 = (int64_t)ti * CT, c0 = (int64_t)tj * CT;
     const int64_t cc = c0 + lane;
+    uint64_t wrows = 0ull;
+    if constexpr (WET) {
+        const int t0 = ho::wet_tile_row(r0, wet_ntr), t1 = t0 + 1 < wet_ntr ? t0 + 1 : wet_ntr - 1, t2 = t0 + 2 < wet_ntr ? t0 + 2 : wet_ntr - 1;
+        const int64_t cw = cc < W ? cc : W - 1;
+        const uint64_t w0 = wet[(int64_t)t0 * W + cw], w1 = wet[(int64_t)t1 * W + cw], w2 = wet[(int64_t)t2 * W + cw];
+        wrows = (cc > 0 && cc < W - 1) ? ho::wet_rows64(w0, w1, w2, r0, H, wet_ntr) : 0ull;
+    }
 #pragma unroll
     for (int k = 0; k < CT / 4; ++k) {
         const int r = wave + 4 * k;
-        const bool fg = (r0 + r) < H && cc < W && is_fg(data[(r0 + r) * W + cc]);
+        bool fg;
+        if constexpr (WET) fg = (wrows >> r) & 1ull;
+        else fg = (r0 + r) < H && cc < W && is_fg(data[(r0 + r) * W + cc]);
         const uint64_t m = __ballot(fg);
         const uint64_t starts = m & ~(m << 1);
         const uint64_t below = starts & ((2ull << lane) - 1ull);
@@ -397,7 +408,7 @@
 
 template <typename T>
 int ccl8_dev(const T *d_data, int32_t *d_labels, int32_t *d_tmp, int64_t H, int64_t W, int64_t *nlabels, hipStream_t s, DevBuf *stats_out = nullptr,
-             CclKeep *keep = nullptr)
+             CclKeep *keep = nullptr, const unsigned long long *wet = nullptr, bool *wet_used = nullptr)
 {
     if (keep) keep->valid = false;
     const int64_t n = H * W;
@@ -431,8 +442,17 @@
         MH_TRY(wprefix.alloc(4 * (size_t)nwords));
         MH_TRY(bcounts.alloc(4 * (size_t)nwb));
         MH_HIP(hipMemsetAsync(bits.p, 0, 8 * (size_t)nwords, s));
-        hipLaunchKernelGGL((ccl_tile_kernel<T>), dim3((unsigned)ntiles), dim3(256), 0, s, d_data, parent, H, W, (int)ntc, roots.as<int32_t>(),
-                           rcount.as<int32_t>(), colpar.as<int32_t>());
+        bool from_bits = false;
+        if constexpr (std::is_same<T, float>::value) from_bits = wet && H >= 3 && W >= 3;
+        if constexpr (std::is_same<T, float>::value) {
+            if (from_bits)
+                hipLaunchKernelGGL((ccl_tile_kernel<T, true>), dim3((unsigned)ntiles), dim3(256), 0, s, d_data, parent, H, W, (int)ntc, roots.as<int32_t>(),
+                                   rcount.as<int32_t>(), colpar.as<int32_t>(), wet, (int)((H - 2 + ho::TI - 1) / ho::TI));
+            if (from_bits && wet_used) *wet_used = true;
+        }
+        if (!from_bits)
+            hipLaunchKernelGGL((ccl_tile_kernel<T, false>), dim3((unsigned)ntiles), dim3(256), 0, s, d_data, parent, H, W, (int)ntc, roots.as<int32_t>(),
+                               rcount.as<int32_t>(), colpar.as<int32_t>(), (const unsigned long long *)nullptr, 0);
         const int64_t nh = (ntr - 1) * W, nv = (ntc - 1) * H;
         if (nh + nv > 0)
             hipLaunchKernelGGL(ccl_seam_kernel, dim3((unsigned)cdiv(nh + nv, 256)), dim3(256), 0, s, parent, H, W, nh, nh + nv, colpar.as<int32_t>(), ntc);
@@ -496,9 +516,10 @@
 }
 
 int ccl8_f32_dev(const float *d_data, int32_t *d_labels, int32_t *d_tmp, int64_t H, int64_t W, int64_t *nlabels,
-                 hipStream_t s, DevBuf *stats_out)
-{
-    return ccl8_dev<float>(d_data, d_labels, d_tmp, H, W, nlabels, s, stats_out);
+                 hipStream_t s, DevBuf *stats_out, const unsigned long long *wet, bool *wet_used)
+{
+    if (wet_used) *wet_used = false;
+    return ccl8_dev<float>(d_data, d_labels, d_tmp, H, W, nlabels, s, stats_out, nullptr, wet, wet_used);
 }
 int ccl8_f32_begin_dev(const float *d_data, int32_t *d_labels, int32_t *d_tmp, int64_t H, int64_t W, int64_t *nlabels, hipStream_t s, CclKeep *keep)
 {
diff --git a/malstroem_amd/csrc/common.hpp b/malstroem_amd/csrc/common.hpp
--- a/malstroem_amd/csrc/common.hpp
+++ b/malstroem_amd/csrc/common.hpp
@@ -200,6 +200,9 @@
     int ntr = 0, ntc = 0;
     bool pending = false, queued = false, violated = false, repaired = false;
     bool suspect = false;
+    unsigned long long *wet = nullptr;
+    bool wet_ok = false;
+    bool wet_pass = false;
     FillStats st_repair;
     FillHandover() = default;
     FillHandover(const FillHandover &) = delete;
@@ -273,6 +276,7 @@
     bool defer_out = false;
     bool out_deferred = false;
     FillHandover *handover = nullptr;
+    bool wet_used = false;
     struct Impl;
     Impl *impl;
     GeoRun();
@@ -358,7 +362,7 @@
               int32_t *d_exit_map = nullptr, PourLink *pour = nullptr, AccumKeep *keep = nullptr, AccumPrep *prep = nullptr);
 int accum_band_delta_dev(const uint8_t *d_fd, double *d_out, int64_t H, int64_t W, hipStream_t s, int fixed_top, int fixed_bot, AccumKeep *keep, bool *done);
 int ccl8_f32_dev(const float *d_data, int32_t *d_labels, int32_t *d_tmp, int64_t H, int64_t W, int64_t *nlabels,
-                 hipStream_t s, DevBuf *stats_out = nullptr);
+                 hipStream_t s, DevBuf *stats_out = nullptr, const unsigned long long *wet = nullptr, bool *wet_used = nullptr);
 int label_emit_stats_dev(const int32_t *d_parent, const unsigned long long *d_rootbits, const uint32_t *d_wordprefix, const float *d_data,
                          int32_t *d_labels, int64_t H, int64_t W, int64_t nlab, mhip_stat_record *d_rec, hipStream_t s);
 int ccl8_u8_dev(const uint8_t *d_data, int32_t *d_labels, int32_t *d_tmp, int64_t H, int64_t W, int64_t *nlabels,
diff --git a/malstroem_amd/csrc/ctx.hip b/malstroem_amd/csrc/ctx.hip
--- a/malstroem_amd/csrc/ctx.hip
+++ b/malstroem_amd/csrc/ctx.hip
@@ -433,6 +433,7 @@
     else if (k == "fill_tiles") *value = c->fill_st.tiles;
     else if (k == "fill_algorithm") *value = c->fill_st.algorithm;
     else if (k == "fill_handover") *value = c->fill_handover;
+    else if (k == "wetbits_used") *value = (c->wet_pass_used ? 1 : 0) | (c->wet_label_used ? 2 : 0);
     else if (k == "fill_handover_rechecks") *value = c->fill_handover_rechecks;
     else if (k == "fill_overflow") *value = c->fill_st.overflow;
     else if (k == "fill_launches") *value = c->fill_st.rounds;
diff --git a/malstroem_amd/csrc/ctx.hpp b/malstroem_amd/csrc/ctx.hpp
--- a/malstroem_amd/csrc/ctx.hpp
+++ b/malstroem_amd/csrc/ctx.hpp
@@ -126,6 +126,7 @@
     int32_t fill_rounds = 0, noflat_rounds = 0;
     int64_t fill_handover_rechecks = 0;
     int32_t fill_handover = 0;
+    int32_t wet_pass_used = 0, wet_label_used = 0;
     mh::FillStats fill_st, noflat_st;
     mh::StageTimer timers[mh::N_TIMERS];
     void *comm = nullptr;
diff --git a/malstroem_amd/csrc/ctx_run.hip b/malstroem_amd/csrc/ctx_run.hip
--- a/malstroem_amd/csrc/ctx_run.hip
+++ b/malstroem_amd/csrc/ctx_run.hip
@@ -1,14 +1,17 @@
 #include <atomic>
+#include <cmath>
 #include <future>
 #include <string>
 
 #include "ctx.hpp"
+#include "handover_addr.hpp"
 
 using namespace mh;
 
 constexpr int LABEL_START_DEFAULT = 3;
 constexpr int FILL_HANDOVER_DEFAULT = 1;
 constexpr int NOFLAT_LAZY_DEFAULT = 1;
+constexpr int WETBITS_DEFAULT = 1;
 
 static bool fill_handover_env()
 {
@@ -20,6 +23,12 @@
 {
     const char *e = dev_env("MHIP_NOFLAT_LAZY");
     return e ? e[0] != '0' : NOFLAT_LAZY_DEFAULT != 0;
+}
+
+static bool wetbits_env()
+{
+    const char *e = dev_env("MHIP_WETBITS");
+    return e ? e[0] != '0' : WETBITS_DEFAULT != 0;
 }
 
 static int stage_depths(mhip_ctx *c, hipStream_t s)
@@ -91,6 +100,8 @@
         ctx_wrote(c, MHIP_R_FILLED);
         c->have[MHIP_R_FILLED] = true;
     }
+    if (ho && ho->wet && !(c->fill_st.have_minmax && !c->fill_st.dem_nan && std::isfinite(c->fill_st.dem_min) && std::isfinite(c->fill_st.dem_max)))
+        ho->wet = nullptr;
     D8Sink d8;
     static const bool fuse_d8 = [] { const char *e = dev_env("MHIP_D8_FUSE"); return !(e && e[0] == '0'); }();
     if (with_flowdir && fuse_d8 && !c->ht && !c->hb) {
@@ -108,6 +119,7 @@
     const int rc_nf = fill_noflat_dev(c->r[MHIP_R_DEM].as<float>(), c->r[MHIP_R_NOFLAT].as<double>(), H, W, c->sh, c->dg, s, &st,
                                       c->r[MHIP_R_FILLED].as<float>(), tail_hook, d8.flowdir ? &d8 : nullptr, ho);
     ctx_handover_settled(c, ho);
+    if (ho && ho->wet_pass) c->wet_pass_used = 1;
     MH_TRY(rc_nf);
     if (flowdir_done) *flowdir_done = d8.done;
     MH_TRY(stage_end(c, MHIP_STAGE_NOFLAT, s));
@@ -166,7 +178,7 @@
     return MHIP_OK;
 }
 
-static int stage_label(mhip_ctx *c, hipStream_t s)
+static int stage_label(mhip_ctx *c, hipStream_t s, const FillHandover *ho = nullptr)
 {
     const int64_t H = c->H, W = c->W, n = H * W;
     MH_ARG(c->have[MHIP_R_DEPTHS] || c->have[MHIP_R_FILLED], "LABEL needs bluespot depths");
@@ -175,8 +187,11 @@
     MH_TRY(stage_begin(c, MHIP_STAGE_LABEL, s));
     if (!c->have[MHIP_R_DEPTHS]) MH_TRY(stage_depths(c, s));
     ctx_wrote(c, MHIP_R_LABELS);
+    const unsigned long long *wet = ho && ho->wet_ok && c->have[MHIP_R_DEPTHS] ? ho->wet : nullptr;
+    bool wet_used = false;
     MH_TRY(ccl8_f32_dev(c->r[MHIP_R_DEPTHS].as<float>(), c->r[MHIP_R_LABELS].as<int32_t>(), c->tmp_i32.as<int32_t>(), H, W,
-                        &c->nlabels_raw, s, &c->raw_stats));
+                        &c->nlabels_raw, s, &c->raw_stats, wet, &wet_used));
+    if (wet_used) c->wet_label_used = 1;
     MH_TRY(stage_end(c, MHIP_STAGE_LABEL, s));
     c->have[MHIP_R_LABELS] = true;
     c->labels_components = true;
@@ -284,6 +299,12 @@
     FillHandover *const ho =
         ((mask & MHIP_STAGE_FILL) && (mask & MHIP_STAGE_NOFLAT) && c->nranks == 1 && !c->ht && !c->hb && fill_handover_env()) ? &handover : nullptr;
     c->fill_handover = 0;
+    c->wet_pass_used = c->wet_label_used = 0;
+    DevBuf wetbuf;
+    if (ho && wetbits_env() && c->H >= 3 && c->W >= 3) {
+        MH_TRY(wetbuf.alloc(8 * (size_t)ho::wet_words(c->W, (int)((c->H - 2 + ho::TI - 1) / ho::TI))));
+        handover.wet = wetbuf.as<unsigned long long>();
+    }
 
     if (!overlap) {
         if (mask & MHIP_STAGE_FILL) MH_TRY(stage_fill(c, s, true, ho));
@@ -291,7 +312,7 @@
         if (mask & MHIP_STAGE_NOFLAT) MH_TRY(stage_noflat(c, s, false, nullptr, (mask & MHIP_STAGE_FLOWDIR) != 0, &fd_done, ho));
         if (mask & MHIP_STAGE_FLOWDIR) MH_TRY(fd_done ? stage_flowdir_fused(c, s) : stage_flowdir(c, s));
         if (mask & MHIP_STAGE_ACCUM) MH_TRY(stage_accum(c, s));
-        if (mask & MHIP_STAGE_LABEL) MH_TRY(stage_label(c, s));
+        if (mask & MHIP_STAGE_LABEL) MH_TRY(stage_label(c, s, ho));
         if (mask & MHIP_STAGE_WATERSHED) MH_TRY(stage_watershed(c, s));
         if (mask & MHIP_STAGE_POURPOINTS) MH_TRY(stage_pourpoints(c, s));
         return MHIP_OK;
@@ -363,7 +384,7 @@
             int rc_l = rc_e == MHIP_OK ? fill_fut.get() : rc_e;
             if (rc_l == MHIP_OK) rc_l = tail_fut.get();
             if (rc_l == MHIP_OK && hipStreamWaitEvent(sb, c->ev_tail, 0) != hipSuccess) rc_l = MHIP_EHIP;
-            if (rc_l == MHIP_OK && (mask & MHIP_STAGE_LABEL)) rc_l = stage_label(c, sb);
+            if (rc_l == MHIP_OK && (mask & MHIP_STAGE_LABEL)) rc_l = stage_label(c, sb, ho);
             else if (rc_l == MHIP_OK && do_fill && !c->have[MHIP_R_DEPTHS]) rc_l = stage_depths(c, sb);
             if (rc_l == MHIP_OK && (mask & (MHIP_STAGE_WATERSHED | MHIP_STAGE_POURPOINTS)) && c->have[MHIP_R_LABELS]) {
                 rc_l = ctx_ensure_labels_final(c, sb);
diff --git a/malstroem_amd/csrc/handover_addr.hpp b/malstroem_amd/csrc/handover_addr.hpp
--- a/malstroem_amd/csrc/handover_addr.hpp
+++ b/malstroem_amd/csrc/handover_addr.hpp
@@ -71,5 +71,27 @@
 }
 MH_HD inline int64_t store_index(const Win &w, int r, int lane) { return (w.r0 + r) * w.W + w.c0 + lane; }
 
+MH_HD inline int64_t wet_words(int64_t W, int ntr) { return (int64_t)ntr * W; }
+MH_HD inline int64_t wet_index(const Win &w, int lane) { return (int64_t)w.ti * w.W + w.c0 + lane; }
+MH_HD inline int64_t wet_bytes_behind(const Win &w) { return (w.W - w.c0) * 8; }
+MH_HD inline int wet_tile_row(int64_t R, int ntr)
+{
+    const int64_t t = (R < 1 ? 0 : R - 1) / TI;
+    return (int)(t < ntr - 1 ? t : ntr - 1);
+}
+MH_HD inline uint64_t wet_rows64(uint64_t w0, uint64_t w1, uint64_t w2, int64_t R0, int64_t H, int ntr)
+{
+    const int t0 = wet_tile_row(R0, ntr);
+    const int s = (int)(R0 - (int64_t)t0 * TI);
+    const int n0 = TI - s;
+    const uint64_t lo0 = (2ull << n0) - 1ull;
+    const uint64_t lo1 = n0 + TI >= 63 ? ~0ull : (2ull << (n0 + TI)) - 1ull;
+    const uint64_t p2 = n0 + TI < 64 ? w2 << ((n0 + TI) & 63) : 0ull;
+    uint64_t m = ((w0 >> s) & lo0) | ((w1 << n0) & ~lo0 & lo1) | (p2 & ~lo1);
+    const int64_t inner = H - 1 - R0;
+    m &= inner >= 64 ? ~0ull : (inner <= 0 ? 0ull : (1ull << inner) - 1ull);
+    return R0 == 0 ? m & ~1ull : m;
+}
+
 }
 }
diff --git a/malstroem_amd/csrc/noflat_geo.hip b/malstroem_amd/csrc/noflat_geo.hip
--- a/malstroem_amd/csrc/noflat_geo.hip
+++ b/malstroem_amd/csrc/noflat_geo.hip
@@ -71,6 +71,7 @@
     const uint16_t *ho_bslot;
     const uint32_t *ho_tabV;
     float *ho_F, *ho_depths;
+    unsigned long long *ho_wet;
 };
 
 template <int R> __device__ __forceinline__ void lds_put(uint32_t addr, uint32_t v) { asm volatile("ds_write_b32 %0, %1 offset:%2" : : "v"(addr), "v"(v), "n"(R) : "memory"); }
@@ -641,6 +642,15 @@
                 finish_q(3);
                 proof_bad |= below;
                 asm volatile("" : "+v"(raised[0]), "+v"(raised[1]));
+                {
+                    const int64_t wet_left = ho::wet_bytes_behind(w);
+                    const __amdgpu_buffer_rsrc_t rW = __builtin_amdgcn_make_buffer_rsrc(
+                        (void *)(a.ho_wet ? a.ho_wet + ho::wet_index(w, 0) : (unsigned long long *)a.ho_F), 0,
+                        a.ho_wet ? (int)(wet_left < 0x7fffffff ? wet_left : 0x7fffffff) : 0, 0x00020000);
+                    typedef uint32_t u32x2 __attribute__((ext_vector_type(2)));
+                    const u32x2 word = {raised[0], raised[1]};
+                    if (ocol) __builtin_amdgcn_raw_buffer_store_b64(word, rW, lane * 8, 0, 0);
+                }
                 lds_wait();
                 __builtin_amdgcn_sched_barrier(0);
                 lds_get_rows<0, WN>(scr_b + 4u * lane, sl);
@@ -1137,10 +1147,17 @@
     const uint32_t lo = from_right((uint32_t)b), hi = from_right((uint32_t)(b >> 32));
     return __longlong_as_double((long long)(((uint64_t)hi << 32) | lo));
 }
-template <bool D8, bool STORE = true>
+__device__ __forceinline__ uint32_t ng_wet_rows(const unsigned long long *__restrict__ wet, int64_t rb, int64_t cc, int64_t H, int64_t W, int ntr, bool inner_col)
+{
+    const int t0 = ho::wet_tile_row(rb, ntr), t1 = t0 + 1 < ntr ? t0 + 1 : ntr - 1;
+    const uint64_t w0 = wet[(int64_t)t0 * W + cc], w1 = wet[(int64_t)t1 * W + cc];
+    return inner_col ? (uint32_t)ho::wet_rows64(w0, w1, 0ull, rb, H, ntr) : 0u;
+}
+template <bool D8, bool STORE = true, bool WET = false>
 __global__ __launch_bounds__(256) void ng_finish_kernel(const float *__restrict__ F, const uint32_t *__restrict__ d, const float *__restrict__ dem,
                                                         double *__restrict__ G, int64_t H, int64_t W, double sh, double dg, double seed_add, int fixed_top,
-                                                        int fixed_bot, unsigned long long *counters, uint8_t *__restrict__ flowdir, unsigned int *nodir)
+                                                        int fixed_bot, unsigned long long *counters, uint8_t *__restrict__ flowdir, unsigned int *nodir,
+                                                        const unsigned long long *__restrict__ wet, int ntr)
 {
     const int lane = threadIdx.x & 63, wave = threadIdx.x >> 6;
     const int64_t c = ((int64_t)blockIdx.x * 4 + wave) * TI + lane - 1;
@@ -1151,21 +1168,28 @@
     const bool inner_col = c > 0 && c + 1 < W;
     const double PINF = __builtin_inf();
     unsigned unreached = 0, bad = 0, anynodir = 0;
+    float fb = 0.0f, fn = 0.0f;
     auto value = [&](int64_t r) -> double {
         if (!(r >= 0 && r < H && col_in)) return PINF;
         bool beyond;
-        const double v = ng_value(F[r * W + cc], d[r * W + cc], seed_add, &beyond);
+        fn = F[r * W + cc];
+        const double v = ng_value(fn, d[r * W + cc], seed_add, &beyond);
         unreached += beyond && mine && r >= rb && r < rb + FRB ? 1u : 0u;
         return v;
     };
+    uint32_t wrows = 0u;
+    if constexpr (WET) wrows = ng_wet_rows(wet, rb, cc, H, W, ntr, inner_col);
     double a = value(rb - 1), b = value(rb);
+    fb = fn;
     for (int i = 0; i < FRB; ++i) {
         const int64_t r = rb + i;
         if (r >= H) break;
         const double n = value(r + 1);
         const double al = dleft(a), ar = dright(a), bl = dleft(b), br = dright(b), nl = dleft(n), nr = dright(n);
         if (mine) {
-            const double dv = (double)dem[r * W + c];
+            double dv;
+            if constexpr (WET) dv = (wrows >> i) & 1u ? -PINF : (double)fb;
+            else dv = (double)dem[r * W + c];
             double want = dv;
             if (r > 0 && r < H - 1 && inner_col) {
                 const double md = fmin(fmin(al, ar), fmin(nl, nr)) + dg;
@@ -1187,6 +1211,7 @@
         }
         a = b;
         b = n;
+        fb = fn;
     }
     if (unreached) atomicAdd(&counters[C_UNREACHED], (unsigned long long)unreached);
     if (bad) atomicAdd(&counters[C_MISMATCH], (unsigned long long)bad);
@@ -1205,10 +1230,11 @@
 #define NG_FINISH_RESIDENCY
 #endif
 #if NG_FINISH_AHEAD
-template <bool STORE>
+template <bool STORE, bool WET>
 __device__ __forceinline__ void ng_finish_ahead(const float *__restrict__ F, const uint32_t *__restrict__ d, const float *__restrict__ dem,
                                                 double *__restrict__ G, int64_t H, int64_t W, double sh, double dg, double seed_add, int fixed_top,
-                                                int fixed_bot, unsigned long long *counters, uint8_t *__restrict__ flowdir, unsigned int *nodir)
+                                                int fixed_bot, unsigned long long *counters, uint8_t *__restrict__ flowdir, unsigned int *nodir,
+                                                const unsigned long long *__restrict__ wet, int ntr)
 {
     const int lane = threadIdx.x & 63, wave = threadIdx.x >> 6;
     const int64_t c = ((int64_t)blockIdx.x * 4 + wave) * TI + lane - 1;
@@ -1219,13 +1245,29 @@
     const bool inner_col = c > 0 && c + 1 < W;
     const double PINF = __builtin_inf();
     unsigned unreached = 0, bad = 0, anynodir = 0;
-    struct Row {
+    struct RowZ {
         float f, z;
         uint32_t dd;
     };
+    struct RowW {
+        float f;
+        uint32_t dd;
+    };
+    typedef typename std::conditional<WET, RowW, RowZ>::type Row;
     auto load = [&](int64_t r) -> Row {
         const int64_t at = (r < 0 ? 0 : (r < H ? r : H - 1)) * W + cc;
-        return Row{F[at], dem[at], d[at]};
+        if constexpr (WET) return Row{F[at], d[at]};
+        else return Row{F[at], dem[at], d[at]};
+    };
+    uint32_t wrows = 0u;
+    if constexpr (WET) wrows = ng_wet_rows(wet, rb, cc, H, W, ntr, inner_col);
+    auto dem_of = [&](const Row &x) -> double {
+        if constexpr (WET) {
+            const double v = wrows & 1u ? -PINF : (double)x.f;
+            wrows >>= 1;
+            return v;
+        } else
+            return (double)x.z;
     };
     auto value = [&](int64_t r, const Row &x) -> double {
         if (!(r >= 0 && r < H && col_in)) return PINF;
@@ -1235,15 +1277,15 @@
         return v;
     };
     const Row xa = load(rb - 1), xb = load(rb);
-    Row x0 = load(rb + 1), x1{0.0f, 0.0f, 0u};
+    Row x0 = load(rb + 1), x1{};
     double a = value(rb - 1, xa), b = value(rb, xb);
-    double dvb = (double)xb.z;
+    double dvb = dem_of(xb);
     auto row = [&](int i, const Row &xn, Row &xnn, auto more) {
         const int64_t r = rb + i;
         const double dv = dvb;
         if (decltype(more)::value) xnn = load(r + 2);
         const double n = value(r + 1, xn);
-        dvb = (double)xn.z;
+        dvb = dem_of(xn);
         asm volatile("" : "+v"(dvb));
         const double al = dleft(a), ar = dright(a), bl = dleft(b), br = dright(b), nl = dleft(n), nr = dright(n);
         if (mine && r < H) {
@@ -1281,17 +1323,19 @@
     if (bad) atomicAdd(&counters[C_MISMATCH], (unsigned long long)bad);
     if (__any(anynodir != 0u) && lane == 0) *nodir = 1u;
 }
-#define NG_FINISH_AHEAD_KERNEL(STORE)                                                                                                                  \
+#define NG_FINISH_AHEAD_KERNEL(STORE, WET)                                                                                                             \
     template <>                                                                                                                                        \
-    __global__ __launch_bounds__(256) NG_FINISH_RESIDENCY void ng_finish_kernel<true, STORE>(                                                          \
+    __global__ __launch_bounds__(256) NG_FINISH_RESIDENCY void ng_finish_kernel<true, STORE, WET>(                                                     \
         const float *__restrict__ F, const uint32_t *__restrict__ d, const float *__restrict__ dem, double *__restrict__ G, int64_t H, int64_t W,      \
         double sh, double dg, double seed_add, int fixed_top, int fixed_bot, unsigned long long *counters, uint8_t *__restrict__ flowdir,              \
-        unsigned int *nodir)                                                                                                                           \
+        unsigned int *nodir, const unsigned long long *__restrict__ wet, int ntr)                                                                      \
     {                                                                                                                                                  \
-        ng_finish_ahead<STORE>(F, d, dem, G, H, W, sh, dg, seed_add, fixed_top, fixed_bot, counters, flowdir, nodir);                                  \
-    }
-NG_FINISH_AHEAD_KERNEL(true)
-NG_FINISH_AHEAD_KERNEL(false)
+        ng_finish_ahead<STORE, WET>(F, d, dem, G, H, W, sh, dg, seed_add, fixed_top, fixed_bot, counters, flowdir, nodir, wet, ntr);                   \
+    }
+NG_FINISH_AHEAD_KERNEL(true, false)
+NG_FINISH_AHEAD_KERNEL(false, false)
+NG_FINISH_AHEAD_KERNEL(true, true)
+NG_FINISH_AHEAD_KERNEL(false, true)
 #undef NG_FINISH_AHEAD_KERNEL
 #endif
 
@@ -1369,14 +1413,14 @@
     a.H = H; a.W = W; a.ntr = m.ntr; a.ntc = m.ntc; a.nt = (int)m.nt; a.F = filled; a.d = dist; a.tab = m.d_tab; a.counters = m.d_cnt;
     a.blk = m.d_blk; a.hdr = m.d_hdr; a.mark = m.d_mark; a.list = m.d_list; a.fixed_top = fixed_top; a.fixed_bot = fixed_bot;
     a.append = 0; a.round_next = 0; a.amark = m.d_amark; a.list_next = nullptr; a.count_next = nullptr;
-    a.ho_dem = nullptr; a.ho_bslot = nullptr; a.ho_tabV = nullptr; a.ho_F = nullptr; a.ho_depths = nullptr;
+    a.ho_dem = nullptr; a.ho_bslot = nullptr; a.ho_tabV = nullptr; a.ho_F = nullptr; a.ho_depths = nullptr; a.ho_wet = nullptr;
     const unsigned grid = (unsigned)std::min<int64_t>((m.nt + 3) / 4, 512);
     for (int k = 0; k < nb; ++k, ++m.round) {
         a.maxcyc = m.maxcyc;
         a.count = m.d_any + m.round;
         if (!m.round && handover && handover->pending) {
             a.ho_dem = handover->dem; a.ho_bslot = handover->bslot; a.ho_tabV = handover->tabV;
-            a.ho_F = handover->filled; a.ho_depths = handover->depths;
+            a.ho_F = handover->filled; a.ho_depths = handover->depths; a.ho_wet = handover->wet;
             hipLaunchKernelGGL(ng_handover_kernel, dim3(grid), dim3(256), m.lds, s, a);
             handover->queued = true;
             (void)hipEventRecord(m.span.back().first, s);
@@ -1487,6 +1531,7 @@
             return MHIP_OK;
         }
         handover->release();
+        handover->wet_ok = handover->wet != nullptr;
     }
     m.used = 1;
     m.irregular = h_c[C_IRREGULAR];
@@ -1551,15 +1596,22 @@
     if (tail_hook) tail_hook->fire_at(StageHook::FINISH, s);
     const bool no_store = with_d8 && defer_out;
     out_deferred = false;
-    if (no_store)
-        hipLaunchKernelGGL((ng_finish_kernel<true, false>), dim3((unsigned)((W + 4 * TI - 1) / (4 * TI)), (unsigned)((H + FRB - 1) / FRB)), dim3(256), 0, s, filled, dist,
-                           dem, out, H, W, sh, dg, seed_add, fixed_top, fixed_bot, m.d_cnt, d8_out, d8_nodir);
-    else if (with_d8)
-        hipLaunchKernelGGL(ng_finish_kernel<true>, dim3((unsigned)((W + 4 * TI - 1) / (4 * TI)), (unsigned)((H + FRB - 1) / FRB)), dim3(256), 0, s, filled, dist, dem,
-                           out, H, W, sh, dg, seed_add, fixed_top, fixed_bot, m.d_cnt, d8_out, d8_nodir);
-    else if (!partial)
-        hipLaunchKernelGGL(ng_finish_kernel<false>, dim3((unsigned)((W + 4 * TI - 1) / (4 * TI)), (unsigned)((H + FRB - 1) / FRB)), dim3(256), 0, s, filled, dist, dem,
-                           out, H, W, sh, dg, seed_add, fixed_top, fixed_bot, m.d_cnt, (uint8_t *)nullptr, (unsigned int *)nullptr);
+    const unsigned long long *wet = handover && handover->wet_ok && !fixed_top && !fixed_bot ? handover->wet : nullptr;
+    wet_used = false;
+    const dim3 fgrid((unsigned)((W + 4 * TI - 1) / (4 * TI)), (unsigned)((H + FRB - 1) / FRB));
+    auto finish = [&](auto d8_tag, auto store_tag, auto wet_tag, uint8_t *fd, unsigned int *nd) {
+        hipLaunchKernelGGL((ng_finish_kernel<decltype(d8_tag)::value, decltype(store_tag)::value, decltype(wet_tag)::value>), fgrid, dim3(256), 0, s, filled, dist, dem,
+                           out, H, W, sh, dg, seed_add, fixed_top, fixed_bot, m.d_cnt, fd, nd, wet, m.ntr);
+        wet_used = decltype(wet_tag)::value;
+    };
+    const std::true_type yes;
+    const std::false_type no;
+    if (no_store && wet) finish(yes, no, yes, d8_out, d8_nodir);
+    else if (no_store) finish(yes, no, no, d8_out, d8_nodir);
+    else if (with_d8 && wet) finish(yes, yes, yes, d8_out, d8_nodir);
+    else if (with_d8) finish(yes, yes, no, d8_out, d8_nodir);
+    else if (!partial && wet) finish(no, yes, yes, nullptr, nullptr);
+    else if (!partial) finish(no, yes, no, nullptr, nullptr);
     else
         hipLaunchKernelGGL(ng_assemble_kernel, dim3((unsigned)((n + 1023) / 1024)), dim3(256), 0, s, filled, dist, out, n, seed_add, m.d_cnt);
     MH_HIP(hipGetLastError());
@@ -1673,6 +1725,7 @@
     MH_TRY(g.end(s, &ok, st));
     if (partial) *partial = g.partial;
     if (d8) { d8->done = g.d8_done; d8->deferred = g.out_deferred; }
+    if (ho) ho->wet_pass = g.wet_used;
     if (!ok && st) st->geo_reject = 2;
     return ok ? MHIP_OK : MHIP_ELIMIT;
 }
```

After: 13030 Mcells/s (median of 6 runs). 1.0% higher.
